# olegiy/manuscript-ocr

Hardware: AMD Instinct MI355X
Metric: manuscript pages/sec end-to-end (EAST+TRBA) at 1/2/4/8 MI355X; CER vs CPU ref (higher is better)
Workload: dtype f32 (bf16x3 split operands on the 1x1 / Winograd-domain GEMMs, f32 accumulate)

## Files before the change

### include/msocr.h

```cpp
#ifndef MSOCR_H
#define MSOCR_H
#include <stdint.h>

#ifdef __cplusplus
extern "C" {
#endif

#define MSOCR_F32 0
#define MSOCR_BF16 1

#define MSOCR_OK 0
#define MSOCR_E_ARG (-1)
#define MSOCR_E_LAUNCH (-2)
#define MSOCR_E_NOGPU (-3)

#define MSOCR_CONV_RELU 1u
#define MSOCR_CONV_RESIDUAL 2u
#define MSOCR_CONV_POOL2 4u

typedef struct msocr_conv_desc {
  int32_t dtype;
  int32_t N, H, W, Cin;
  int64_t in_sN, in_sH, in_sW;
  int32_t KH, KW, stride_h, stride_w, pad_h, pad_w;
  int32_t Ho, Wo, Cout;
  int64_t out_ld;
  int64_t res_ld;
  uint32_t flags;
} msocr_conv_desc;

int msocr_conv2d(const msocr_conv_desc* d, const void* in, const void* weight, const float* bias,
                 const void* residual, void* out, void* stream);

#define MSOCR_WINO_2X2 0
#define MSOCR_WINO_4X2 1
#define MSOCR_WINO_4X4 2
#define MSOCR_WINO_4X4_COLTAIL 3
int64_t msocr_winograd_workspace_bytes(const msocr_conv_desc* d, int form);
int msocr_winograd_weights_host(int form, const float* w_khwc_host, int Cout, int Cin, float* u_out_host);
int msocr_conv3x3_winograd(const msocr_conv_desc* d, int form, int split, const void* in, const void* u, const float* bias,
                           const void* residual, void* out, void* workspace, void* stream);
int msocr_winograd_input_transform(const msocr_conv_desc* d, int form, const void* in, void* workspace, void* stream);
int msocr_winograd_gemm(const msocr_conv_desc* d, int form, int split, const void* u, void* workspace, void* stream);
int msocr_winograd_output_transform(const msocr_conv_desc* d, int form, const void* workspace, const float* bias, const void* residual,
                                    void* out, void* stream);

int64_t msocr_winograd_crop_lds_bytes(const msocr_conv_desc* d, int form, int se);
int msocr_winograd_output_chain(const msocr_conv_desc* d, int form, void* workspace, const float* bias, void* stream);
int msocr_winograd_output_se(const msocr_conv_desc* d, int form, const void* workspace, const float* bias, const void* identity,
                             const float* w1, const float* w2, float* gate_ws, void* out, void* stream);

int msocr_split_bf16x3_host(const float* w_host, int64_t n, uint16_t* planes_out_host);
int msocr_split_bf16x3_ktile_host(const float* w_host, int64_t nbatch, int64_t rows, int64_t k, uint16_t* planes_out_host);
int msocr_conv1x1_split(const msocr_conv_desc* d, const void* in, const void* weight_planes, const float* bias,
                        const void* residual, void* out, void* stream);
int msocr_conv2d_split(const msocr_conv_desc* d, const void* in, const void* weight_planes, const float* bias,
                       const void* residual, void* out, void* stream);

int64_t msocr_winograd_fused64_workspace_bytes(const msocr_conv_desc* d);
int msocr_conv3x3_winograd_fused64(const msocr_conv_desc* d, int split, const void* in, const void* u, const float* bias,
                                   const void* residual, void* out, void* workspace, void* stream);
int msocr_winograd_fused64_gemm_output(const msocr_conv_desc* d, int split, const void* u, const void* workspace, const float* bias,
                                       const void* residual, void* out, void* stream);

int msocr_normalize_u8(const uint8_t* src, int N, int H, int W, int pad_t, int pad_l, int Hp, int Wp, int cpad,
                       int mode, int dtype, void* out, void* stream);

int msocr_resize_linear_u8(const uint8_t* src, int N, int sh, int sw, uint8_t* dst, int dh, int dw, void* stream);

int msocr_maxpool2d(const void* in, int N, int H, int W, int C, int64_t in_ld, int k, int s, int p, int dtype,
                    void* out, int Ho, int Wo, int64_t out_ld, void* stream);

int msocr_upsample2x_bilinear(const void* in, int N, int H, int W, int C, int64_t in_ld, int dtype, void* out,
                              int64_t out_ld, void* stream);

int msocr_east_head(const void* h1, int64_t npix, int64_t in_ld, int dtype, const float* w9, const float* b9,
                    float* score_out, float* geo_out, void* stream);

int msocr_east_decode(const float* score, const float* geo, int N, int H, int W, float thresh, float scale,
                      int quant, float* cand_out, int32_t* count_out, int max_cand, void* stream);

int64_t msocr_lanms_workspace_bytes(int N, int max_cand);
int msocr_east_lanms(const float* cand, const int32_t* counts, int N, int max_cand, double iou_thr, float* boxes_out,
                     int32_t* nbox_out, void* workspace, void* stream);

int64_t msocr_east_box_tail_workspace_bytes(int N, int max_cand);
int msocr_east_box_tail(const float* boxes, const int32_t* nbox, int N, int max_cand, double expand_w, double expand_h,
                        double scale_x, double scale_y, int axis_aligned_output, int remove_anomalies, double sigma, int min_count,
                        float* out, int32_t* n_out, void* workspace, void* stream);
int msocr_east_box_tail_host(const float* quads_host, int M, double expand_w, double expand_h, double scale_x, double scale_y,
                             int axis_aligned_output, int remove_anomalies, double sigma, int min_count, float* out_host,
                             int32_t* n_out_host);


int msocr_se_residual(const void* x, const void* identity, int N, int HW, int C, int dtype, const float* w1,
                      const float* w2, float* gate_ws, void* out, void* stream);

int msocr_mean_over_h(const void* in, int N, int H, int W, int C, int dtype, float* out, void* stream);

int msocr_bilstm_recurrent(const float* xproj, const float* w_hh_t, int B, int T, int H, float* hcat_out,
                           void* stream);
int msocr_bilstm_recurrent_split(const float* xproj, const uint16_t* whh_planes, int B, int T, int H, float* hcat_out,
                                 void* stream);

typedef struct msocr_attn_weights {
  const float* h2h_wt;
  const float* h2h_b;
  const float* score_w;
  const float* wih_ctx_t;
  const float* wih_tok;
  const float* whh_t;
  const float* b_gates;
  const float* gen_wt;
  const float* gen_b;
} msocr_attn_weights;

int msocr_attn_greedy(const float* batch_H, const float* proj_H, const msocr_attn_weights* w, int B, int T, int H,
                      int V, int steps, int sos_id, int eos_id, int blank_id, float* logits_out, int32_t* ids_out,
                      void* stream);
int64_t msocr_attn_beam_workspace_bytes(int B, int steps, int beam, int V);
int msocr_attn_beam(const float* batch_H, const float* proj_H, const msocr_attn_weights* w, int B, int T, int H,
                    int V, int steps, int beam, const float* lp_dev, float temperature, int sos_id, int eos_id,
                    int blank_id, int32_t* fin_step_out, void* workspace, const int32_t* chunk_id_dev,
                    const int32_t* chunk_size_dev, int32_t* chunk_state_dev, void* stream);
typedef struct msocr_attn_split_weights {
  const uint16_t* h2h_p;
  const uint16_t* whh_p;
  const uint16_t* gen_p;
} msocr_attn_split_weights;

int msocr_attn_beam_hoisted(const float* batch_H, const float* proj_H, const float* ctx_gates, const msocr_attn_weights* w,
                            const msocr_attn_split_weights* ws, int B, int T, int H, int V, int steps, int beam, const float* lp_dev,
                            float temperature, int sos_id, int eos_id, int blank_id, int32_t* fin_step_out, void* workspace,
                            const int32_t* chunk_id_dev, const int32_t* chunk_size_dev, int32_t* chunk_state_dev, void* stream);
int msocr_attn_greedy_hoisted(const float* batch_H, const float* proj_H, const float* ctx_gates, const msocr_attn_weights* w,
                              const msocr_attn_split_weights* ws, int B, int T, int H, int V, int steps, int sos_id, int eos_id,
                              int blank_id, float* logits_out, int32_t* ids_out, void* stream);
int64_t msocr_attn_pack_split_elems(int N);
int msocr_attn_pack_split_host(const float* wt_host, int N, int gate_interleaved, uint16_t* out_host);
int msocr_attn_beam_finalize(const void* workspace, int B, int V, int steps, int beam, const int32_t* trun_dev,
                             float* logits_out, int32_t* ids_out, void* stream);

int msocr_attn_greedy_alpha(const float* batch_H, const float* proj_H, const msocr_attn_weights* w, int B, int T, int H,
                            int V, int steps, int sos_id, int eos_id, int blank_id, float* logits_out, int32_t* ids_out,
                            float* alpha_out, void* stream);
int msocr_attn_greedy_hoisted_alpha(const float* batch_H, const float* proj_H, const float* ctx_gates, const msocr_attn_weights* w,
                                    const msocr_attn_split_weights* ws, int B, int T, int H, int V, int steps, int sos_id, int eos_id,
                                    int blank_id, float* logits_out, int32_t* ids_out, float* alpha_out, void* stream);
int64_t msocr_attn_beam_alpha_bytes(int B, int steps, int beam, int T);
int msocr_attn_beam_alpha(const float* batch_H, const float* proj_H, const msocr_attn_weights* w, int B, int T, int H,
                          int V, int steps, int beam, const float* lp_dev, float temperature, int sos_id, int eos_id,
                          int blank_id, int32_t* fin_step_out, void* workspace, const int32_t* chunk_id_dev,
                          const int32_t* chunk_size_dev, int32_t* chunk_state_dev, void* alpha_ws, void* stream);
int msocr_attn_beam_hoisted_alpha(const float* batch_H, const float* proj_H, const float* ctx_gates, const msocr_attn_weights* w,
                                  const msocr_attn_split_weights* ws, int B, int T, int H, int V, int steps, int beam,
                                  const float* lp_dev, float temperature, int sos_id, int eos_id, int blank_id, int32_t* fin_step_out,
                                  void* workspace, const int32_t* chunk_id_dev, const int32_t* chunk_size_dev,
                                  int32_t* chunk_state_dev, void* alpha_ws, void* stream);
int msocr_attn_beam_finalize_alpha(const void* workspace, int B, int V, int steps, int beam, const int32_t* trun_dev,
                                   float* logits_out, int32_t* ids_out, const void* alpha_ws, int T, float* alpha_out,
                                   void* stream);

int msocr_seq_confidence(const float* logits, const int32_t* ids, const int32_t* trun_dev, int B, int V, int steps,
                         float* conf_out, void* stream);

int msocr_seq_char_details(const float* logits, const int32_t* ids, const float* alpha, const int32_t* trun_dev, int B, int V,
                           int steps, int T, float* prob_out, float* centre_out, int32_t* peak_out, void* stream);

int msocr_attn_beam_nbest(const void* workspace, int B, int V, int steps, int beam, int n_best, int eos_id, const int32_t* trun_dev,
                          int32_t* ids_out, float* prob_out, float* conf_out, float* logp_out, void* stream);
int msocr_attn_beam_nbest_host(const void* workspace_host, int B, int V, int steps, int beam, int n_best, int eos_id,
                               const int32_t* trun_host, int32_t* ids_out_host, float* prob_out_host, float* conf_out_host,
                               float* logp_out_host);

int msocr_attn_forced(const float* batch_H, const float* proj_H, const msocr_attn_weights* w, int B, int T, int H, int V, int steps,
                      const int32_t* tok_in, int sos_id, int blank_id, float* logits_out, float* alpha_out, void* stream);
int msocr_attn_forced_hoisted(const float* batch_H, const float* proj_H, const float* ctx_gates, const msocr_attn_weights* w,
                              const msocr_attn_split_weights* ws, int B, int T, int H, int V, int steps, const int32_t* tok_in,
                              int sos_id, int blank_id, float* logits_out, float* alpha_out, void* stream);

int msocr_seq_logp(const float* logits, const int32_t* ids, const int32_t* trun_dev, int B, int V, int steps, float temperature,
                   float* logp_steps_out, float* logp_out, void* stream);
int msocr_seq_logp_host(const float* logits_host, const int32_t* ids_host, const int32_t* trun_host, int B, int V, int steps,
                        float temperature, float* logp_steps_out_host, float* logp_out_host);

typedef struct {
  const int32_t *edge_begin, *edge_tok, *edge_child;
  const uint8_t* terminal;
  int n_nodes, n_edges;
} msocr_lexicon;
int64_t msocr_attn_lexicon_nodes_bytes(int B, int steps, int beam);
int msocr_attn_beam_lexicon(const float* batch_H, const float* proj_H, const msocr_attn_weights* w, int B, int T, int H, int V, int steps,
                            int beam, const float* lp_dev, float temperature, int sos_id, int eos_id, int blank_id,
                            int32_t* fin_step_out, void* workspace, const int32_t* chunk_id_dev, const int32_t* chunk_size_dev,
                            int32_t* chunk_state_dev, void* alpha_ws, const msocr_lexicon* lex, int32_t* node_out, void* stream);
int msocr_attn_beam_lexicon_hoisted(const float* batch_H, const float* proj_H, const float* ctx_gates, const msocr_attn_weights* w,
                                    const msocr_attn_split_weights* ws, int B, int T, int H, int V, int steps, int beam,
                                    const float* lp_dev, float temperature, int sos_id, int eos_id, int blank_id, int32_t* fin_step_out,
                                    void* workspace, const int32_t* chunk_id_dev, const int32_t* chunk_size_dev,
                                    int32_t* chunk_state_dev, void* alpha_ws, const msocr_lexicon* lex, int32_t* node_out, void* stream);
int msocr_lexicon_check_host(const int32_t* edge_begin_host, const int32_t* edge_tok_host, const int32_t* edge_child_host,
                             const uint8_t* terminal_host, int n_nodes, int n_edges, int V, int max_depth);

// ... 124 lines not shown
```

### manuscript_ocr_amd/_native.py

```python
import ctypes
import os

import torch

_HERE = os.path.dirname(os.path.abspath(__file__))
LIB_PATH = os.path.join(_HERE, "libmsocr.so")

F32, BF16 = 0, 1
CONV_RELU, CONV_RESIDUAL, CONV_POOL2 = 1, 2, 4
WINO_2X2, WINO_4X2, WINO_4X4, WINO_4X4_COLTAIL = 0, 1, 2, 3

c_i32, c_i64, c_u32 = ctypes.c_int32, ctypes.c_int64, ctypes.c_uint32
c_f32, c_f64, c_vp = ctypes.c_float, ctypes.c_double, ctypes.c_void_p


class ConvDesc(ctypes.Structure):
    _fields_ = [
        ("dtype", c_i32), ("N", c_i32), ("H", c_i32), ("W", c_i32), ("Cin", c_i32),
        ("in_sN", c_i64), ("in_sH", c_i64), ("in_sW", c_i64),
        ("KH", c_i32), ("KW", c_i32), ("stride_h", c_i32), ("stride_w", c_i32), ("pad_h", c_i32), ("pad_w", c_i32),
        ("Ho", c_i32), ("Wo", c_i32), ("Cout", c_i32),
        ("out_ld", c_i64), ("res_ld", c_i64), ("flags", c_u32),
    ]


class JpegInfo(ctypes.Structure):
    _fields_ = [("width", c_i32), ("height", c_i32), ("ncomp", c_i32), ("hs", c_i32 * 3), ("vs", c_i32 * 3),
                ("blocks_w", c_i32 * 3), ("blocks_h", c_i32 * 3), ("supported", c_i32), ("coef_off", c_i64 * 3),
                ("coef_total", c_i64), ("quant", (ctypes.c_uint16 * 64) * 3)]


class AttnWeights(ctypes.Structure):
    _fields_ = [(n, c_vp) for n in ("h2h_wt", "h2h_b", "score_w", "wih_ctx_t", "wih_tok", "whh_t", "b_gates", "gen_wt", "gen_b")]


class AttnSplitWeights(ctypes.Structure):
    _fields_ = [(n, c_vp) for n in ("h2h_p", "whh_p", "gen_p")]


class LexiconArrays(ctypes.Structure):
    _fields_ = [("edge_begin", c_vp), ("edge_tok", c_vp), ("edge_child", c_vp), ("terminal", c_vp), ("n_nodes", c_i32), ("n_edges", c_i32)]


class WordList(ctypes.Structure):
    _fields_ = [("word_begin", c_vp), ("word_tok", c_vp), ("n_words", c_i32), ("n_tok", c_i32), ("by_length", c_vp)]


class CharLMTable(ctypes.Structure):
    _fields_ = [("table", c_vp), ("order", c_i32), ("V", c_i32), ("n_ctx", c_i64)]


_SIGS = {
    "msocr_conv2d": (c_i32, [ctypes.POINTER(ConvDesc), c_vp, c_vp, c_vp, c_vp, c_vp, c_vp]),
    "msocr_winograd_workspace_bytes": (c_i64, [ctypes.POINTER(ConvDesc), c_i32]),
    "msocr_winograd_weights_host": (c_i32, [c_i32, c_vp, c_i32, c_i32, c_vp]),
    "msocr_conv3x3_winograd": (c_i32, [ctypes.POINTER(ConvDesc), c_i32, c_i32, c_vp, c_vp, c_vp, c_vp, c_vp, c_vp, c_vp]),
    "msocr_winograd_input_transform": (c_i32, [ctypes.POINTER(ConvDesc), c_i32, c_vp, c_vp, c_vp]),
    "msocr_winograd_gemm": (c_i32, [ctypes.POINTER(ConvDesc), c_i32, c_i32, c_vp, c_vp, c_vp]),
    "msocr_winograd_output_transform": (c_i32, [ctypes.POINTER(ConvDesc), c_i32, c_vp, c_vp, c_vp, c_vp, c_vp]),
    "msocr_winograd_crop_lds_bytes": (c_i64, [ctypes.POINTER(ConvDesc), c_i32, c_i32]),
    "msocr_winograd_output_chain": (c_i32, [ctypes.POINTER(ConvDesc), c_i32, c_vp, c_vp, c_vp]),
    "msocr_winograd_output_se": (c_i32, [ctypes.POINTER(ConvDesc), c_i32, c_vp, c_vp, c_vp, c_vp, c_vp, c_vp, c_vp, c_vp]),
    "msocr_winograd_fused64_workspace_bytes": (c_i64, [ctypes.POINTER(ConvDesc)]),
    "msocr_conv3x3_winograd_fused64": (c_i32, [ctypes.POINTER(ConvDesc), c_i32, c_vp, c_vp, c_vp, c_vp, c_vp, c_vp, c_vp]),
    "msocr_winograd_fused64_gemm_output": (c_i32, [ctypes.POINTER(ConvDesc), c_i32, c_vp, c_vp, c_vp, c_vp, c_vp, c_vp]),
    "msocr_split_bf16x3_host": (c_i32, [c_vp, c_i64, c_vp]),
    "msocr_split_bf16x3_ktile_host": (c_i32, [c_vp, c_i64, c_i64, c_i64, c_vp]),
    "msocr_conv1x1_split": (c_i32, [ctypes.POINTER(ConvDesc), c_vp, c_vp, c_vp, c_vp, c_vp, c_vp]),
    "msocr_conv2d_split": (c_i32, [ctypes.POINTER(ConvDesc), c_vp, c_vp, c_vp, c_vp, c_vp, c_vp]),
    "msocr_normalize_u8": (c_i32, [c_vp, c_i32, c_i32, c_i32, c_i32, c_i32, c_i32, c_i32, c_i32, c_i32, c_i32, c_vp, c_vp]),
    "msocr_resize_linear_u8": (c_i32, [c_vp, c_i32, c_i32, c_i32, c_vp, c_i32, c_i32, c_vp]),
    "msocr_maxpool2d": (c_i32, [c_vp, c_i32, c_i32, c_i32, c_i32, c_i64, c_i32, c_i32, c_i32, c_i32, c_vp, c_i32, c_i32, c_i64, c_vp]),
    "msocr_upsample2x_bilinear": (c_i32, [c_vp, c_i32, c_i32, c_i32, c_i32, c_i64, c_i32, c_vp, c_i64, c_vp]),
    "msocr_east_head": (c_i32, [c_vp, c_i64, c_i64, c_i32, c_vp, c_vp, c_vp, c_vp, c_vp]),
    "msocr_east_decode": (c_i32, [c_vp, c_vp, c_i32, c_i32, c_i32, c_f32, c_f32, c_i32, c_vp, c_vp, c_i32, c_vp]),
    "msocr_lanms_workspace_bytes": (c_i64, [c_i32, c_i32]),
    "msocr_east_lanms": (c_i32, [c_vp, c_vp, c_i32, c_i32, c_f64, c_vp, c_vp, c_vp, c_vp]),
    "msocr_se_residual": (c_i32, [c_vp, c_vp, c_i32, c_i32, c_i32, c_i32, c_vp, c_vp, c_vp, c_vp, c_vp]),
    "msocr_mean_over_h": (c_i32, [c_vp, c_i32, c_i32, c_i32, c_i32, c_i32, c_vp, c_vp]),
    "msocr_bilstm_recurrent": (c_i32, [c_vp, c_vp, c_i32, c_i32, c_i32, c_vp, c_vp]),
    "msocr_bilstm_recurrent_split": (c_i32, [c_vp, c_vp, c_i32, c_i32, c_i32, c_vp, c_vp]),
    "msocr_attn_greedy": (c_i32, [c_vp, c_vp, ctypes.POINTER(AttnWeights), c_i32, c_i32, c_i32, c_i32, c_i32, c_i32, c_i32, c_i32,
                                  c_vp, c_vp, c_vp]),
    "msocr_attn_greedy_hoisted": (c_i32, [c_vp, c_vp, c_vp, ctypes.POINTER(AttnWeights), ctypes.POINTER(AttnSplitWeights), c_i32, c_i32,
                                          c_i32, c_i32, c_i32, c_i32, c_i32, c_i32, c_vp, c_vp, c_vp]),
    "msocr_attn_beam": (c_i32, [c_vp, c_vp, ctypes.POINTER(AttnWeights), c_i32, c_i32, c_i32, c_i32, c_i32, c_i32, c_vp, c_f32,
                                c_i32, c_i32, c_i32, c_vp, c_vp, c_vp, c_vp, c_vp, c_vp]),
    "msocr_attn_pack_split_elems": (c_i64, [c_i32]),
    "msocr_attn_pack_split_host": (c_i32, [c_vp, c_i32, c_i32, c_vp]),
    "msocr_attn_beam_hoisted": (c_i32, [c_vp, c_vp, c_vp, ctypes.POINTER(AttnWeights), ctypes.POINTER(AttnSplitWeights), c_i32, c_i32, c_i32, c_i32, c_i32, c_i32, c_vp, c_f32,
                                        c_i32, c_i32, c_i32, c_vp, c_vp, c_vp, c_vp, c_vp, c_vp]),
    "msocr_attn_beam_workspace_bytes": (c_i64, [c_i32, c_i32, c_i32, c_i32]),
    "msocr_attn_beam_finalize": (c_i32, [c_vp, c_i32, c_i32, c_i32, c_i32, c_vp, c_vp, c_vp, c_vp]),
    "msocr_seq_confidence": (c_i32, [c_vp, c_vp, c_vp, c_i32, c_i32, c_i32, c_vp, c_vp]),
    "msocr_attn_greedy_alpha": (c_i32, [c_vp, c_vp, ctypes.POINTER(AttnWeights), c_i32, c_i32, c_i32, c_i32, c_i32, c_i32, c_i32, c_i32,
                                        c_vp, c_vp, c_vp, c_vp]),
    "msocr_attn_greedy_hoisted_alpha": (c_i32, [c_vp, c_vp, c_vp, ctypes.POINTER(AttnWeights), ctypes.POINTER(AttnSplitWeights), c_i32,
                                                c_i32, c_i32, c_i32, c_i32, c_i32, c_i32, c_i32, c_vp, c_vp, c_vp, c_vp]),
    "msocr_attn_beam_alpha_bytes": (c_i64, [c_i32, c_i32, c_i32, c_i32]),
    "msocr_attn_beam_alpha": (c_i32, [c_vp, c_vp, ctypes.POINTER(AttnWeights), c_i32, c_i32, c_i32, c_i32, c_i32, c_i32, c_vp, c_f32,
                                      c_i32, c_i32, c_i32, c_vp, c_vp, c_vp, c_vp, c_vp, c_vp, c_vp]),
    "msocr_attn_beam_hoisted_alpha": (c_i32, [c_vp, c_vp, c_vp, ctypes.POINTER(AttnWeights), ctypes.POINTER(AttnSplitWeights), c_i32, c_i32,
                                              c_i32, c_i32, c_i32, c_i32, c_vp, c_f32, c_i32, c_i32, c_i32, c_vp, c_vp, c_vp, c_vp, c_vp,
                                              c_vp, c_vp]),
    "msocr_attn_beam_finalize_alpha": (c_i32, [c_vp, c_i32, c_i32, c_i32, c_i32, c_vp, c_vp, c_vp, c_vp, c_i32, c_vp, c_vp]),
    "msocr_seq_char_details": (c_i32, [c_vp, c_vp, c_vp, c_vp, c_i32, c_i32, c_i32, c_i32, c_vp, c_vp, c_vp, c_vp]),
    "msocr_attn_beam_nbest": (c_i32, [c_vp, c_i32, c_i32, c_i32, c_i32, c_i32, c_i32, c_vp, c_vp, c_vp, c_vp, c_vp, c_vp]),
    "msocr_attn_beam_nbest_host": (c_i32, [c_vp, c_i32, c_i32, c_i32, c_i32, c_i32, c_i32, c_vp, c_vp, c_vp, c_vp, c_vp]),
    "msocr_attn_forced": (c_i32, [c_vp, c_vp, ctypes.POINTER(AttnWeights), c_i32, c_i32, c_i32, c_i32, c_i32, c_vp, c_i32, c_i32,
                                  c_vp, c_vp, c_vp]),
    "msocr_attn_forced_hoisted": (c_i32, [c_vp, c_vp, c_vp, ctypes.POINTER(AttnWeights), ctypes.POINTER(AttnSplitWeights), c_i32, c_i32,
                                          c_i32, c_i32, c_i32, c_vp, c_i32, c_i32, c_vp, c_vp, c_vp]),
    "msocr_seq_logp": (c_i32, [c_vp, c_vp, c_vp, c_i32, c_i32, c_i32, c_f32, c_vp, c_vp, c_vp]),
    "msocr_seq_logp_host": (c_i32, [c_vp, c_vp, c_vp, c_i32, c_i32, c_i32, c_f32, c_vp, c_vp]),
    "msocr_attn_lexicon_nodes_bytes": (c_i64, [c_i32, c_i32, c_i32]),
    "msocr_attn_beam_lexicon": (c_i32, [c_vp, c_vp, ctypes.POINTER(AttnWeights), c_i32, c_i32, c_i32, c_i32, c_i32, c_i32, c_vp, c_f32,
                                        c_i32, c_i32, c_i32, c_vp, c_vp, c_vp, c_vp, c_vp, c_vp, ctypes.POINTER(LexiconArrays), c_vp, c_vp]),
    "msocr_attn_beam_lexicon_hoisted": (c_i32, [c_vp, c_vp, c_vp, ctypes.POINTER(AttnWeights), ctypes.POINTER(AttnSplitWeights), c_i32, c_i32,
                                                c_i32, c_i32, c_i32, c_i32, c_vp, c_f32, c_i32, c_i32, c_i32, c_vp, c_vp, c_vp, c_vp, c_vp,
                                                c_vp, ctypes.POINTER(LexiconArrays), c_vp, c_vp]),
    "msocr_attn_lm_ctx_bytes": (c_i64, [c_i32, c_i32, c_i32]),
    "msocr_attn_beam_lm": (c_i32, [c_vp, c_vp, ctypes.POINTER(AttnWeights), c_i32, c_i32, c_i32, c_i32, c_i32, c_i32, c_vp, c_f32,
                                   c_i32, c_i32, c_i32, c_vp, c_vp, c_vp, c_vp, c_vp, c_vp, ctypes.POINTER(CharLMTable), c_f32, c_vp, c_vp]),
    "msocr_attn_beam_lm_hoisted": (c_i32, [c_vp, c_vp, c_vp, ctypes.POINTER(AttnWeights), ctypes.POINTER(AttnSplitWeights), c_i32, c_i32,
                                           c_i32, c_i32, c_i32, c_i32, c_vp, c_f32, c_i32, c_i32, c_i32, c_vp, c_vp, c_vp, c_vp, c_vp,
                                           c_vp, ctypes.POINTER(CharLMTable), c_f32, c_vp, c_vp]),
    "msocr_lexicon_check_host": (c_i32, [c_vp, c_vp, c_vp, c_vp, c_i32, c_i32, c_i32, c_i32]),
    "msocr_lexicon_nearest_ws_bytes": (c_i64, [c_i32, c_i32, c_i32]),
    "msocr_lexicon_nearest": (c_i32, [c_vp, c_vp, c_i32, c_i32, c_i32, c_i32, c_i32, c_i32, ctypes.POINTER(WordList), c_i32, c_i32,
                                      c_vp, c_vp, c_vp, c_vp]),
    "msocr_lexicon_nearest_host": (c_i32, [c_vp, c_vp, c_i32, c_i32, c_i32, c_i32, c_i32, c_i32, ctypes.POINTER(WordList), c_i32, c_i32,
                                           c_vp, c_vp]),
    "msocr_edit_distance_pairs": (c_i32, [c_vp, c_vp, c_i32, c_vp, c_vp, c_i32, c_i32, c_i32, c_i32, c_i32, c_i32, c_vp, c_vp, c_vp,
                                          c_vp]),
    "msocr_edit_distance_pairs_host": (c_i32, [c_vp, c_vp, c_i32, c_vp, c_vp, c_i32, c_i32, c_i32, c_i32, c_i32, c_i32, c_vp, c_vp,
                                               c_vp]),
    "msocr_wordlist_check_host": (c_i32, [c_vp, c_vp, c_i32, c_i32, c_i32, c_i32]),
    "msocr_crop_resize_pad": (c_i32, [c_vp, c_i32, c_i32, c_i32, c_vp, c_vp, c_i32, c_i32, c_i32, c_vp, c_vp]),
    "msocr_east_box_tail_workspace_bytes": (c_i64, [c_i32, c_i32]),
    "msocr_east_box_tail": (c_i32, [c_vp, c_vp, c_i32, c_i32, c_f64, c_f64, c_f64, c_f64, c_i32, c_i32, c_f64, c_i32, c_vp, c_vp, c_vp, c_vp]),
    "msocr_east_box_tail_host": (c_i32, [c_vp, c_i32, c_f64, c_f64, c_f64, c_f64, c_i32, c_i32, c_f64, c_i32, c_vp, c_vp]),
    "msocr_reading_order_host": (c_i32, [c_vp, c_i32, c_f64, c_f64, c_vp]),
    "msocr_reading_lines_host": (c_i32, [c_vp, c_i32, c_f64, c_f64, c_vp, c_vp, c_vp, c_vp]),
    "msocr_reading_order_workspace_bytes": (c_i64, [c_i32, c_i32]),
    "msocr_reading_order_crops": (c_i32, [c_vp, c_vp, c_i32, c_i32, c_i32, c_i32, c_i32, c_i32, c_i32, c_f64, c_f64, c_i32,
                                          c_vp, c_vp, c_vp, c_vp, c_vp, c_vp]),
    "msocr_reading_order_line_rows": (c_i32, [c_i32]),
    "msocr_reading_order_lines": (c_i32, [c_vp, c_vp, c_i32, c_i32, c_i32, c_i32, c_i32, c_i32, c_i32, c_f64, c_f64, c_i32,
                                          c_vp, c_vp, c_vp, c_vp, c_vp, c_vp, c_vp, c_vp, c_vp]),
    "msocr_quad_crop_descriptors": (c_i32, [c_vp, c_vp, c_i32, c_i32, c_i32, c_i32, c_vp, c_vp, c_vp, c_vp, c_vp, c_vp]),
    "msocr_quad_crop_descriptors_host": (c_i32, [c_vp, c_vp, c_i32, c_i32, c_i32, c_i32, c_vp]),
    "msocr_quad_crop": (c_i32, [c_vp, c_i32, c_i32, c_i32, c_vp, c_vp, c_i32, c_i32, c_i32, c_vp, c_vp]),
    "msocr_quad_crop_host": (c_i32, [c_vp, c_i32, c_i32, c_i32, c_vp, c_i32, c_i32, c_i32, c_vp]),
    "msocr_jpeg_parse_host": (c_i32, [c_vp, c_i64, ctypes.POINTER(JpegInfo)]),
    "msocr_jpeg_parse_oriented_host": (c_i32, [c_vp, c_i64, ctypes.POINTER(JpegInfo), ctypes.POINTER(c_i32)]),
    "msocr_jpeg_entropy_decode_host": (c_i32, [c_vp, c_i64, ctypes.POINTER(JpegInfo), c_vp]),
    "msocr_jpeg_scan_desc_bytes": (c_i64, []),
    "msocr_jpeg_scan_prepare_host": (c_i64, [c_vp, c_i64, ctypes.POINTER(JpegInfo), c_i64, c_vp, c_vp, c_i64]),
    "msocr_jpeg_entropy_decode_device": (c_i32, [c_vp, c_vp, c_i32, c_i32, c_vp, c_vp, c_vp, c_i64, c_vp, c_vp]),
    "msocr_jpeg_entropy_decode_intervals_host": (c_i32, [c_vp, c_vp, c_i32, c_vp, c_vp, c_vp, c_i64, c_vp]),
    "msocr_jpeg_sync_prepare_host": (c_i64, [c_vp, c_i64, ctypes.POINTER(JpegInfo), c_i64, c_vp, c_vp, c_i64]),
    "msocr_jpeg_sync_workspace_bytes": (c_i64, [c_i64, c_i32, c_i32]),
    "msocr_jpeg_entropy_decode_sync_device": (c_i32, [c_vp, c_vp, c_i32, c_vp, c_vp, c_vp, c_i32, c_i64, c_i32, c_i32, c_vp, c_i64,
                                                      c_vp, c_vp, c_vp, c_vp]),
    "msocr_jpeg_entropy_decode_sync_host": (c_i32, [c_vp, c_vp, c_i32, c_vp, c_vp, c_vp, c_i32, c_i32, c_vp, c_i64, c_vp, c_vp]),
    "msocr_jpeg_workspace_bytes": (c_i64, [ctypes.POINTER(JpegInfo)]),
    "msocr_jpeg_reconstruct": (c_i32, [ctypes.POINTER(JpegInfo), c_vp, c_vp, c_vp, c_vp]),
    "msocr_jpeg_reconstruct_host": (c_i32, [ctypes.POINTER(JpegInfo), c_vp, c_vp]),
    "msocr_jpeg_reconstruct_oriented": (c_i32, [ctypes.POINTER(JpegInfo), c_i32, c_vp, c_vp, c_vp, c_vp]),
    "msocr_jpeg_reconstruct_oriented_host": (c_i32, [ctypes.POINTER(JpegInfo), c_i32, c_vp, c_vp]),
    "msocr_nchw_f32_to_nhwc": (c_i32, [c_vp, c_i32, c_i32, c_i32, c_i32, c_i32, c_vp, c_i64, c_vp]),
    "msocr_nhwc_to_nchw_f32": (c_i32, [c_vp, c_i32, c_i32, c_i32, c_i32, c_i64, c_i32, c_vp, c_vp]),
    "msocr_version": (ctypes.c_char_p, []),
}

_lib = None


class NativeError(RuntimeError):
    pass


def lib():
    global _lib
    if _lib is None:
        if not os.path.exists(LIB_PATH) and os.path.exists("/opt/rocm/bin/hipcc"):
            import fcntl
            import subprocess
            try:
                with open(os.path.join(_HERE, "csrc", ".build.lock"), "w") as lock:
                    fcntl.flock(lock, fcntl.LOCK_EX)
                    if not os.path.exists(LIB_PATH):
                        subprocess.check_call(["make", "-s", "-j4", "-C", os.path.join(_HERE, "csrc"), "ARCH=gfx950"])
            except Exception as e:
                print(f"[manuscript_ocr_amd] building libmsocr.so failed: {e}")
        if not os.path.exists(LIB_PATH):
            raise NativeError(
                f"{LIB_PATH} not found: build it with `python -c 'import __graft_entry__ as g; g.build()'` "
                "(or `make -C manuscript_ocr_amd/csrc`). There is no CPU fallback."
            )
        L = ctypes.CDLL(LIB_PATH)
        missing = [name for name in _SIGS if not hasattr(L, name)]
        if missing:
            raise NativeError(f"{LIB_PATH} lacks symbols declared in include/msocr.h: {missing}")
        for name, (res, args) in _SIGS.items():
            fn = getattr(L, name)
            fn.restype, fn.argtypes = res, args
        _lib = L
    return _lib


def exported_symbols():
    return list(_SIGS)


# ... 4 lines not shown
```

### manuscript_ocr_amd/csrc/conv_common.h

```cpp
#ifndef MSOCR_CONV_COMMON_H
#define MSOCR_CONV_COMMON_H
#include <hip/hip_runtime.h>
#include <stdint.h>

#include <type_traits>

#include "internal.h"
#include "msocr.h"
#include "split_mma.h"

typedef uint32_t u32x4 __attribute__((ext_vector_type(4)));
typedef uint32_t u32x2 __attribute__((ext_vector_type(2)));

struct ConvParams {
  const char* in;
  const char* w;
  const float* bias;
  const char* res;
  char* out;
  int N, H, W, Cin;
  long sN, sH, sW;
  int KH, KW, SH, SW, PH, PW;
  int Ho, Wo, Cout;
  long M;
  int ktiles, cin_tiles;
  long Ktot;
  long out_ld, res_ld;
  int relu, has_res;
  int tilesM, tilesN;
  int nbatch;
  long bsA, bsW, bsO;
  long wplane;
  long w_kt_b;
};

__device__ __forceinline__ float bf16_to_f32(uint16_t v) { return __uint_as_float(((uint32_t)v) << 16); }
__device__ __forceinline__ uint16_t f32_to_bf16(float f) {
  __bf16 b = (__bf16)f;
  return *reinterpret_cast<uint16_t*>(&b);
}

template <typename T>
struct Mma;
template <>
struct Mma<float> {
  static __device__ __forceinline__ void run(const u32x4& a, const u32x4& b, f32x16& c) {
#pragma unroll
    for (int j = 0; j < 4; ++j)
      c = __builtin_amdgcn_mfma_f32_32x32x2f32(__uint_as_float(a[j]), __uint_as_float(b[j]), c, 0, 0, 0);
  }
};
template <>
struct Mma<__bf16> {
  static __device__ __forceinline__ void run(const u32x4& a, const u32x4& b, f32x16& c) {
    bf16x8 av = __builtin_bit_cast(bf16x8, a);
    bf16x8 bv = __builtin_bit_cast(bf16x8, b);
    c = __builtin_amdgcn_mfma_f32_32x32x16_bf16(av, bv, c, 0, 0, 0);
  }
};

__attribute__((visibility("hidden"))) bool msocr_internal_split_pp_takes(const ConvParams& p);
__attribute__((visibility("hidden"))) int msocr_internal_split_pp_launch(ConvParams& p, hipStream_t s, bool general);

template <int BKB>
__device__ __forceinline__ int swz(int row) {
  constexpr int CPR = BKB / 16;
  constexpr int RPB = 256 / BKB;
  return (row / RPB) & (CPR - 1);
}
__device__ __forceinline__ int swz16(int row) { return (4 - ((row >> 2) & 3)) & 3; }
template <typename T, int BM_, int BN_, int BKB_, int WM_, int STAGES_>
struct IgemmTile {
  static constexpr int BM = BM_, BN = BN_, BKB = BKB_, THREADS = 256, PERSISTENT = 0;
  static constexpr int BK = BKB / (int)sizeof(T);
  static constexpr int CPR = BKB / 16;
  static constexpr int RPP = 256 / CPR;
  static constexpr int A_IT = BM / RPP, B_IT = (BN + RPP - 1) / RPP;
  static constexpr int A_BYTES = BM * BKB, B_BYTES = BN * BKB, STAGE = A_BYTES + B_BYTES;
  static constexpr int EPI = (BM / WM_) * 32 * BN * 4;
  static constexpr int LDS = STAGES_ * STAGE > EPI ? STAGES_ * STAGE : EPI;
};
template <int BM_, int BN_>
struct SplitStage {
  static constexpr int BM = BM_, BN = BN_, BK = 32;
  static constexpr int ROWB = BK * 2;
  static constexpr int A_PLANE = BM * ROWB, B_PLANE = BN * ROWB;
  static constexpr int STAGE_B = 3 * (A_PLANE + B_PLANE);
  static constexpr int ACH = BK / 4, ARP = 256 / ACH, A_IT = BM / ARP;
  static constexpr int BCH = BK / 8, BRP = 256 / BCH, B_IT = (BN + BRP - 1) / BRP;
};
template <int BN_>
struct SplitTile : SplitStage<128, BN_> {
  static constexpr int WM = 64, WN = BN_ / 2, THREADS = 256, PERSISTENT = 0;
  static constexpr int EPI = (128 / WM) * 32 * BN_ * 4;
  static constexpr int LDS = SplitStage<128, BN_>::STAGE_B > EPI ? SplitStage<128, BN_>::STAGE_B : EPI;
  static __device__ __forceinline__ int swz(int row) { return ::swz<64>(row); }
};
template <int TM, int TN>
struct SplitPPTile : SplitStage<64 * TM, 64 * TN> {
  static constexpr int THREADS = 512, PERSISTENT = 1;
  static constexpr int BIAS_OFF = 2 * SplitStage<64 * TM, 64 * TN>::STAGE_B;
  static constexpr int LDS = BIAS_OFF + 4 * 64 * TN * 4;
  static __device__ __forceinline__ int swz(int row) { return swz16(row); }
};

static __device__ __attribute__((aligned(16))) uint32_t msocr_zero16[4] = {0u, 0u, 0u, 0u};

template <typename I>
__device__ __forceinline__ void xcd_range(I x, I nblk, I& first, I& count) {
  const I q = nblk >> 3, r = nblk & 7;
  first = x < r ? x * (q + 1) : r * (q + 1) + (x - r) * q;
  count = q + (x < r ? 1 : 0);
}
template <typename I>
__device__ __forceinline__ I xcd_tile(I bid, I nblk) {
  I first, count;
  xcd_range<I>(bid & 7, nblk, first, count);
  return first + (bid >> 3);
}
__device__ __forceinline__ void tile_coords(const ConvParams& p, int t, int& batch, int& tile_m, int& tile_n) {
  const int nblk1 = p.tilesM * p.tilesN;
  batch = t / nblk1;
  t -= batch * nblk1;
  tile_n = t % p.tilesN;
  tile_m = t / p.tilesN;
}

template <bool GEN>
struct ATap { int hi0, wi0; };
template <>
struct ATap<false> {};
__device__ __forceinline__ long a_row_origin(const ConvParams& p, long m, ATap<true>& t) {
  const long hw = (long)p.Ho * p.Wo;
  const int n = (int)(m / hw);
  const int rem = (int)(m - (long)n * hw);
  const int ho = rem / p.Wo, wo = rem - ho * p.Wo;
  t.hi0 = ho * p.SH - p.PH;
  t.wi0 = wo * p.SW - p.PW;
  return (long)n * p.sN + (long)t.hi0 * p.sH + (long)t.wi0 * p.sW;
}
template <bool GEN>
__device__ __forceinline__ uint32_t a_row_offset32(const ConvParams& p, long m, int a_chunk, ATap<GEN>& t) {
  if (m >= p.M) m = p.M - 1;
  if constexpr (GEN) return (uint32_t)(int32_t)((a_row_origin(p, m, t) + a_chunk * 4) * 4);
  else return (uint32_t)((m * p.sW + a_chunk * 4) * 4);
}
struct TapCursor {
  int kh, kw, c0;
  __device__ __forceinline__ void reset() { kh = kw = c0 = 0; }
  __device__ __forceinline__ long offset(const ConvParams& p) const { return (long)kh * p.sH + (long)kw * p.sW + c0; }
  __device__ __forceinline__ bool inside(const ConvParams& p, const ATap<true>& t) const {
    const int hi = t.hi0 + kh, wi = t.wi0 + kw;
    return (unsigned)hi < (unsigned)p.H && (unsigned)wi < (unsigned)p.W;
  }
  __device__ __forceinline__ void advance(const ConvParams& p, int bk) {
    c0 += bk;
    if (c0 == p.Cin) {
      c0 = 0;
      if (++kw == p.KW) { kw = 0; ++kh; }
    }
  }
};
template <int A_IT>
__device__ __forceinline__ void load_a_taps32(const ConvParams& p, const char* g_in, const uint32_t (&a_off)[A_IT],
                                              const ATap<true> (&tap)[A_IT], TapCursor& t, int bk, u32x4 (&ra)[A_IT]) {
  const int32_t koff = (int32_t)(t.offset(p) * 4);
#pragma unroll
  for (int i = 0; i < A_IT; ++i) {
    const char* src = g_in + (long)(int32_t)(a_off[i] + (uint32_t)koff);
    ra[i] = *reinterpret_cast<const u32x4*>(t.inside(p, tap[i]) ? src : reinterpret_cast<const char*>(msocr_zero16));
  }
  t.advance(p, bk);
}
template <int A_IT>
__device__ __forceinline__ void load_a_rows32(const char* ga, const uint32_t (&a_off)[A_IT], u32x4 (&ra)[A_IT]) {
#pragma unroll
  for (int i = 0; i < A_IT; ++i) ra[i] = *reinterpret_cast<const u32x4*>(ga + a_off[i]);
}
__device__ __forceinline__ uint32_t b_plane_offset(int co, int cout, int b_chunk) {
  if (co >= cout) co = cout - 1;
  return (uint32_t)(co * 64 + b_chunk * 16);
}
template <class G>
__device__ __forceinline__ void load_b_planes(const ConvParams& p, const char* g_w, long wplane_b, int kt, int b_row0,
                                              const uint32_t (&b_off)[G::B_IT], u32x4 (&rb)[3][G::B_IT]) {
#pragma unroll
  for (int pl = 0; pl < 3; ++pl) {
    const char* const gb = g_w + pl * wplane_b + (long)kt * p.w_kt_b;
#pragma unroll
    for (int j = 0; j < G::B_IT; ++j)
      if (G::BN % G::BRP == 0 || b_row0 + j * G::BRP < G::BN) rb[pl][j] = *reinterpret_cast<const u32x4*>(gb + b_off[j]);
  }
}
template <class G>
__device__ __forceinline__ void split_store_row(unsigned char* sA, int row, int a_chunk, u32x4 r) {
  float x0 = __uint_as_float(r[0]), x1 = __uint_as_float(r[1]), x2 = __uint_as_float(r[2]), x3 = __uint_as_float(r[3]);
  unsigned char* dst = sA + row * G::ROWB + (((a_chunk >> 1) ^ G::swz(row)) << 4) + ((a_chunk & 1) << 3);
#pragma unroll
  for (int pl = 0; pl < 3; ++pl) {
    u32x2 v;
    v[0] = split_step(x0, x1);
    v[1] = split_step(x2, x3);
    *reinterpret_cast<u32x2*>(dst + pl * G::A_PLANE) = v;
  }
}
template <class G>
__device__ __forceinline__ void store_b_row(unsigned char* sB, int pl, int row, int b_chunk, u32x4 v) {
  *reinterpret_cast<u32x4*>(sB + pl * G::B_PLANE + row * G::ROWB + ((b_chunk ^ G::swz(row)) << 4)) = v;
}

template <typename T, int BM, int BN, int WM, int WN, int MT, bool BIAS16, int NCH = 1, typename AccT, int TMA, int TN>
__device__ __forceinline__ void epilogue_lds(const ConvParams& p, unsigned char* smem, const AccT (&acc)[TMA][TN], int tile_m, int tile_n,
                                             char* g_out, int wm, int wn, int r32, int half) {
  constexpr int ES = sizeof(T), EPC = 16 / ES;
  constexpr int AE = MT == 32 ? 16 : 4;
  const int tid = threadIdx.x;
  constexpr int PR = (BM / WM) * 32;
  float* sc = reinterpret_cast<float*>(smem);
  constexpr int VPR = BN / EPC;
  constexpr int ROWS_PP = 256 / VPR;
  const int vcol = (tid % VPR) * EPC;
  const int vrow0 = tid / VPR;
  const int co = tile_n * BN + vcol;
  float bias[EPC];
  if constexpr (BIAS16) {
    static_assert(EPC == 4, "four f32");
    f32x4 b = {0.f, 0.f, 0.f, 0.f};
    if (p.bias) b = *reinterpret_cast<const f32x4*>(p.bias + co);
    bias[0] = b[0]; bias[1] = b[1]; bias[2] = b[2]; bias[3] = b[3];
  } else {
#pragma unroll
    for (int e = 0; e < EPC; ++e) bias[e] = p.bias ? p.bias[co + e] : 0.f;
  }

  constexpr int TPP = 32 / MT;
  constexpr int NR = PR / ROWS_PP;
  static_assert(PR % ROWS_PP == 0 && NR % NCH == 0, "a pass is whole sweeps of 256 threads, a chunk whole rows");
  static_assert(32 % ROWS_PP == 0 || ROWS_PP == 64, "tile_row must be additive in the sweep index (see row_step)");
  const long m0 = (long)tile_m * BM;
  auto tile_row = [&](int i, int lr) { return (lr >> 5) * WM + i * 32 + (lr & 31); };
  auto lds_write = [&](int i) {
#pragma unroll
    for (int ti = 0; ti < TPP; ++ti)
#pragma unroll
      for (int j = 0; j < TN; ++j)
#pragma unroll
        for (int e = 0; e < AE; ++e) {
          const int rit = MT == 32 ? acc_row(e, half) : 4 * half + e;
          sc[(wm * 32 + ti * MT + rit) * BN + wn * WN + j * MT + r32] = acc[i * TPP + ti][j][e];
        }
  };
  auto lds_row = [&](int lr, float (&v)[EPC]) {
#pragma unroll
    for (int e4 = 0; e4 < EPC; e4 += 4) {
      const f32x4 t = *reinterpret_cast<const f32x4*>(&sc[lr * BN + vcol + e4]);
      v[e4] = t[0]; v[e4 + 1] = t[1]; v[e4 + 2] = t[2]; v[e4 + 3] = t[3];
    }
  };
  auto finish_row = [&](float (&v)[EPC], bool res, const u32x4& rv, char* dst) {
#pragma unroll
    for (int e = 0; e < EPC; ++e) v[e] += bias[e];
    if (res) {
      if constexpr (ES == 4) {
#pragma unroll
        for (int e = 0; e < 4; ++e) v[e] += __uint_as_float(rv[e]);
      } else {
#pragma unroll
        for (int e = 0; e < 8; ++e) v[e] += bf16_to_f32((uint16_t)(rv[e >> 1] >> ((e & 1) * 16)));
      }
    }
    if (p.relu) {
#pragma unroll
      for (int e = 0; e < EPC; ++e) v[e] = fmaxf(v[e], 0.f);
    }
    u32x4 o;
    if constexpr (ES == 4) {
#pragma unroll
      for (int e = 0; e < 4; ++e) o[e] = __float_as_uint(v[e]);
    } else {
#pragma unroll
      for (int e = 0; e < 4; ++e) o[e] = (uint32_t)f32_to_bf16(v[2 * e]) | ((uint32_t)f32_to_bf16(v[2 * e + 1]) << 16);
    }
    *reinterpret_cast<u32x4*>(dst) = o;
  };
  auto whole_tile = [&](auto res_c) {
    constexpr bool RES = decltype(res_c)::value;
    constexpr int CR = NR / NCH;
    const long mt = m0 + tile_row(0, vrow0);
    const char* const res_t = RES ? p.res + (mt * p.res_ld + co) * ES : nullptr;
    char* const out_t = g_out + (mt * p.out_ld + co) * ES;
    auto row_step = [&](int i, int r) { return tile_row(i, r * ROWS_PP); };
    auto load_res = [&](int i, int r0, int r1, u32x4 (&rv)[NR]) {
      if constexpr (RES) {
#pragma unroll
        for (int r = r0; r < r1; ++r) rv[r] = *reinterpret_cast<const u32x4*>(res_t + row_step(i, r) * p.res_ld * ES);
      }
    };
#pragma unroll
    for (int i = 0; i < WM / 32; ++i) {
      const int early = (NCH == 1 || i == WM / 32 - 1) ? NR : CR;
      u32x4 rv[NR];
      load_res(i, 0, early, rv);
      if (i) __syncthreads();
      lds_write(i);
      __syncthreads();
#pragma unroll
      for (int c = 0; c < NCH; ++c) {
        float v[CR][EPC];
#pragma unroll
        for (int r = 0; r < CR; ++r) lds_row(vrow0 + (c * CR + r) * ROWS_PP, v[r]);
#pragma unroll
        for (int r = 0; r < CR; ++r) finish_row(v[r], RES, rv[c * CR + r], out_t + row_step(i, c * CR + r) * p.out_ld * ES);
        if (c == 0 && early < NR) load_res(i, early, NR, rv);
      }
    }
  };
  if (m0 + BM <= p.M) {
    if (p.has_res) whole_tile(std::true_type{});
    else whole_tile(std::false_type{});
    return;
  }
#pragma unroll
  for (int i = 0; i < WM / 32; ++i) {
    if (i) __syncthreads();
    lds_write(i);
    __syncthreads();
    for (int lr = vrow0; lr < PR; lr += ROWS_PP) {
      const long m = m0 + tile_row(i, lr);
      if (m >= p.M) continue;
      float v[EPC];
      lds_row(lr, v);
      u32x4 rv = {0u, 0u, 0u, 0u};
      if (p.has_res) rv = *reinterpret_cast<const u32x4*>(p.res + (m * p.res_ld + co) * ES);
      finish_row(v, p.has_res != 0, rv, g_out + (m * p.out_ld + co) * ES);
    }
  }
}

enum ConvStrideRule {
  CONV_STRIDES_TAPS,
  CONV_STRIDES_ALIGNED,
  CONV_STRIDES_DENSE,
};
static inline int conv_desc_check(const msocr_conv_desc* d, const void* in, const void* weight, const void* residual, const void* out, int es,
                                  int cin_mult, int cout_mult, ConvStrideRule rule) {
  if (!d || !in || !weight || !out) return MSOCR_E_ARG;
  const int EPC = 16 / es;
  if (d->N <= 0 || d->H <= 0 || d->W <= 0 || d->Ho <= 0 || d->Wo <= 0) return MSOCR_E_ARG;
  if (d->Cin <= 0 || d->Cin % cin_mult || d->Cout <= 0 || d->Cout % cout_mult) return MSOCR_E_ARG;
  if (d->KH <= 0 || d->KW <= 0 || d->stride_h <= 0 || d->stride_w <= 0) return MSOCR_E_ARG;
  if (d->out_ld % EPC || d->out_ld < d->Cout) return MSOCR_E_ARG;
  if (rule == CONV_STRIDES_TAPS) {
    if (d->in_sN % EPC) return MSOCR_E_ARG;
    if (d->in_sH % EPC) {
      if ((d->stride_h * d->in_sH) % EPC) return MSOCR_E_ARG;
      for (int kh = 0; kh < d->KH; ++kh)
        if (((kh - d->pad_h) * d->in_sH) % EPC) return MSOCR_E_ARG;
    }
    if (d->in_sW % EPC) {
      if ((d->stride_w * d->in_sW) % EPC) return MSOCR_E_ARG;
      for (int kw = 0; kw < d->KW; ++kw)
        if (((kw - d->pad_w) * d->in_sW) % EPC) return MSOCR_E_ARG;
    }
  } else if (rule == CONV_STRIDES_ALIGNED) {
    if (d->pad_h < 0 || d->pad_w < 0 || d->in_sN % EPC || d->in_sH % EPC || d->in_sW % EPC) return MSOCR_E_ARG;
  } else {
    if (d->KH != 1 || d->KW != 1 || d->stride_h != 1 || d->stride_w != 1 || d->pad_h || d->pad_w || d->Ho != d->H || d->Wo != d->W)
      return MSOCR_E_ARG;
    if (d->in_sW % EPC || d->in_sW < d->Cin || (d->H > 1 && d->in_sH != (int64_t)d->W * d->in_sW) ||
        (d->N > 1 && d->in_sN != (int64_t)d->H * d->W * d->in_sW)) return MSOCR_E_ARG;
  }
  if (((uintptr_t)in | (uintptr_t)weight | (uintptr_t)out) & 15) return MSOCR_E_ARG;
  if ((d->flags & MSOCR_CONV_RESIDUAL) && (!residual || d->res_ld % EPC || d->res_ld < d->Cout || ((uintptr_t)residual & 15))) return MSOCR_E_ARG;
  if ((d->H + 2 * d->pad_h - d->KH) / d->stride_h + 1 < d->Ho || (d->W + 2 * d->pad_w - d->KW) / d->stride_w + 1 < d->Wo)
    return MSOCR_E_ARG;
  return MSOCR_OK;
}
static inline ConvParams conv_params(const msocr_conv_desc* d, const void* in, const void* weight, const float* bias, const void* residual,
                                     void* out) {
  ConvParams p = {};
  p.in = (const char*)in; p.w = (const char*)weight; p.bias = bias; p.res = (const char*)residual; p.out = (char*)out;
  p.N = d->N; p.H = d->H; p.W = d->W; p.Cin = d->Cin;
  p.sN = d->in_sN; p.sH = d->in_sH; p.sW = d->in_sW;
  p.KH = d->KH; p.KW = d->KW; p.SH = d->stride_h; p.SW = d->stride_w; p.PH = d->pad_h; p.PW = d->pad_w;
  p.Ho = d->Ho; p.Wo = d->Wo; p.Cout = d->Cout;
  p.M = (long)d->N * d->Ho * d->Wo;
  p.Ktot = (long)d->KH * d->KW * d->Cin;
  p.out_ld = d->out_ld; p.res_ld = d->res_ld;
  p.relu = (d->flags & MSOCR_CONV_RELU) ? 1 : 0;
  p.has_res = (d->flags & MSOCR_CONV_RESIDUAL) ? 1 : 0;
  p.nbatch = 1;
  return p;
}
static inline int gemm_params(const void* A, const void* B, void* C, long M, int N, int K, int nbatch, int n_mult, int k_mult, ConvParams* out) {
  if (!A || !B || !C || M <= 0 || N <= 0 || N % n_mult || K <= 0 || K % k_mult || nbatch <= 0) return MSOCR_E_ARG;
  if (((uintptr_t)A | (uintptr_t)B | (uintptr_t)C) & 15) return MSOCR_E_ARG;
  if (M > 0x7fffffffL) return MSOCR_E_ARG;
  ConvParams p = {};
  p.in = (const char*)A; p.w = (const char*)B; p.out = (char*)C;
  p.N = 1; p.H = (int)M; p.W = 1; p.Cin = K;
  p.sN = M * (long)K; p.sH = K; p.sW = K;
  p.KH = p.KW = 1; p.SH = p.SW = 1;
  p.Ho = (int)M; p.Wo = 1; p.Cout = N;
  p.M = M; p.Ktot = K;
  p.out_ld = N;
  p.nbatch = nbatch; p.bsA = M * (long)K; p.bsW = (long)N * K; p.bsO = M * (long)N;
  *out = p;
  return MSOCR_OK;
}
template <class G, class Kern>
static int conv_launch(Kern kern, ConvParams& p, hipStream_t s) {
  p.tilesM = (int)((p.M + G::BM - 1) / G::BM);
  p.tilesN = p.Cout / G::BN;
  p.cin_tiles = p.Cin / G::BK;
  p.ktiles = (int)(p.Ktot / G::BK);
  if (msocr_internal_lds_limit(reinterpret_cast<const void*>(kern), G::LDS) != MSOCR_OK) return MSOCR_E_LAUNCH;
  const long nblk = (long)p.tilesM * p.tilesN * p.nbatch;
  if (nblk <= 0 || nblk > 0x7fffffffL) return MSOCR_E_ARG;
  long grid = nblk;
  if (G::PERSISTENT) {
    int n_cu = 0;
    if (msocr_internal_cu_count(&n_cu) != MSOCR_OK) return MSOCR_E_LAUNCH;
    n_cu = n_cu > 8 ? n_cu & ~7 : 8;
    grid = (nblk + 7) & ~7L;
    if (grid > n_cu) grid = n_cu;
  }
  MSOCR_LAUNCH(kern, dim3((unsigned)grid), dim3(G::THREADS), G::LDS, s, p);
  return hipGetLastError() == hipSuccess ? MSOCR_OK : MSOCR_E_LAUNCH;
}

#endif
```

### manuscript_ocr_amd/csrc/conv_split.hip

```cpp
#include <hip/hip_runtime.h>
#include <stdint.h>
#include <stdlib.h>
#include <string.h>

#include "conv_common.h"

namespace {

template <int BN, int WPE, bool GEN>
__global__ __launch_bounds__(256, WPE) void conv_split_kernel(ConvParams p) {
  using G = SplitTile<BN>;
  constexpr int BM = G::BM, WM = G::WM, WN = G::WN, BK = G::BK;
  constexpr int TM = WM / 32, TN = WN / 32;
  constexpr int ROWB = G::ROWB, A_PLANE = G::A_PLANE, B_PLANE = G::B_PLANE, STAGE_B = G::STAGE_B;
  constexpr int ACH = G::ACH, ARP = G::ARP, A_IT = G::A_IT;
  constexpr int BCH = G::BCH, B_IT = G::B_IT;

  extern __shared__ __attribute__((aligned(16))) unsigned char smem[];

  const int tid = threadIdx.x;
  const int lane = tid & 63;
  const int wave = tid >> 6;
  const int wm = wave >> 1, wn = wave & 1;

  int batch, tile_m, tile_n;
  tile_coords(p, xcd_tile<int>(blockIdx.x, p.tilesM * p.tilesN * p.nbatch), batch, tile_m, tile_n);
  const char* const g_in = p.in + (long)batch * p.bsA * 4;
  const char* const g_w = p.w + (long)batch * p.bsW * 2;
  char* const g_out = p.out + (long)batch * p.bsO * 4;

  const int a_chunk = tid % ACH, a_row0 = tid / ACH;
  uint32_t a_off[A_IT];
  ATap<GEN> a_tap[A_IT];
#pragma unroll
  for (int i = 0; i < A_IT; ++i) a_off[i] = a_row_offset32<GEN>(p, (long)tile_m * BM + a_row0 + i * ARP, a_chunk, a_tap[i]);
  TapCursor tap;
  tap.reset();
  const int b_chunk = tid % BCH, b_row0 = tid / BCH;
  uint32_t b_off[B_IT];
#pragma unroll
  for (int j = 0; j < B_IT; ++j) b_off[j] = b_plane_offset(tile_n * BN + b_row0 + j * G::BRP, p.Cout, b_chunk);
  const long wplane_b = p.wplane * 2;

  u32x4 ra[A_IT], rb[3][B_IT];
  auto load_tile = [&](int kt) {
    if constexpr (GEN) load_a_taps32(p, g_in, a_off, a_tap, tap, BK, ra);
    else load_a_rows32(g_in + (long)kt * (BK * 4), a_off, ra);
    load_b_planes<G>(p, g_w, wplane_b, kt, b_row0, b_off, rb);
  };
  auto store_tile = [&](int stage) {
    unsigned char* const sA = smem + stage * STAGE_B;
#pragma unroll
    for (int i = 0; i < A_IT; ++i) split_store_row<G>(sA, a_row0 + i * ARP, a_chunk, ra[i]);
    unsigned char* const sB = sA + 3 * A_PLANE;
#pragma unroll
    for (int pl = 0; pl < 3; ++pl)
#pragma unroll
      for (int j = 0; j < B_IT; ++j)
        if (BN % G::BRP == 0 || b_row0 + j * G::BRP < BN) store_b_row<G>(sB, pl, b_row0 + j * G::BRP, b_chunk, rb[pl][j]);
  };

  f32x16 acc[TM][TN];
#pragma unroll
  for (int i = 0; i < TM; ++i)
#pragma unroll
    for (int j = 0; j < TN; ++j)
#pragma unroll
      for (int e = 0; e < 16; ++e) acc[i][j][e] = 0.f;

  const int r32 = lane & 31, half = lane >> 5;

  auto compute = [&](int stage) {
    const unsigned char* const sA = smem + stage * STAGE_B;
    const unsigned char* const sB = sA + 3 * A_PLANE;
#pragma unroll
    for (int q = 0; q < BK / 16; ++q) {
      const int c = 2 * q + half;
      bf16x8 fa[3][TM], fb[3][TN];
#pragma unroll
      for (int pl = 0; pl < 3; ++pl) {
#pragma unroll
        for (int i = 0; i < TM; ++i) {
          const int row = wm * WM + i * 32 + r32;
          fa[pl][i] = *reinterpret_cast<const bf16x8*>(sA + pl * A_PLANE + row * ROWB + ((c ^ swz<ROWB>(row)) << 4));
        }
#pragma unroll
        for (int j = 0; j < TN; ++j) {
          const int row = wn * WN + j * 32 + r32;
          fb[pl][j] = *reinterpret_cast<const bf16x8*>(sB + pl * B_PLANE + row * ROWB + ((c ^ swz<ROWB>(row)) << 4));
        }
      }
#pragma unroll
      for (int t = 0; t < 6; ++t)
#pragma unroll
        for (int i = 0; i < TM; ++i)
#pragma unroll
          for (int j = 0; j < TN; ++j)
            acc[i][j] = __builtin_amdgcn_mfma_f32_32x32x16_bf16(fa[split_pa(t)][i], fb[split_pb(t)][j], acc[i][j], 0, 0, 0);
    }
  };

  load_tile(0);
  store_tile(0);
  __syncthreads();

  for (int kt = 0; kt < p.ktiles; ++kt) {
    if (kt + 1 < p.ktiles) load_tile(kt + 1);
    compute(0);
    __syncthreads();
    if (kt + 1 < p.ktiles) store_tile(0);
    __syncthreads();
  }

  epilogue_lds<float, BM, BN, WM, WN, 32, true>(p, smem, acc, tile_m, tile_n, g_out, wm, wn, r32, half);
}

template <int BN, int WPE, bool GEN>
int launch_split(ConvParams& p, hipStream_t s) {
  return conv_launch<SplitTile<BN>>(conv_split_kernel<BN, WPE, GEN>, p, s);
}

int launch_split_one(ConvParams& p, hipStream_t s, bool general) {
  if (msocr_internal_split_pp_takes(p)) return msocr_internal_split_pp_launch(p, s, general);
  if (general) return p.Cout % 128 == 0 ? launch_split<128, 3, true>(p, s) : launch_split<64, 3, true>(p, s);
  return p.Cout % 128 == 0 ? launch_split<128, 3, false>(p, s) : launch_split<64, 3, false>(p, s);
}

int launch_split_any(ConvParams& p, hipStream_t s, bool general) {
  if (((long)p.Cout * p.Ktot + 32) * 2 >= (1L << 32)) return MSOCR_E_ARG;
  p.w_kt_b = (long)p.Cout * 64;
  if (general) return launch_split_one(p, s, true);
  const long row_b = p.sW * 4;
  const long limit = (1L << 32) - 4096;
  if ((p.M * p.sW + 32) * 4 < limit) return launch_split_one(p, s, false);
  if (p.nbatch != 1 || row_b <= 0 || row_b * 256 >= limit) return MSOCR_E_ARG;
  const long rows_per = (limit / row_b) & ~255L;
  for (long m0 = 0; m0 < p.M; m0 += rows_per) {
    ConvParams q = p;
    q.M = p.M - m0 < rows_per ? p.M - m0 : rows_per;
    q.in = p.in + m0 * row_b;
    q.out = p.out + m0 * p.out_ld * 4;
    if (p.has_res) q.res = p.res + m0 * p.res_ld * 4;
    const int rc = launch_split_one(q, s, false);
    if (rc != MSOCR_OK) return rc;
  }
  return MSOCR_OK;
}

}

extern "C" int msocr_split_bf16x3_host(const float* w_host, int64_t n, uint16_t* planes_out_host) {
  if (!w_host || !planes_out_host || n <= 0) return MSOCR_E_ARG;
  auto rne = [](float f) -> uint16_t {
    uint32_t u = __builtin_bit_cast(uint32_t, f);
    if ((u & 0x7fffffffu) > 0x7f800000u) return (uint16_t)((u >> 16) | 0x40);
    u += 0x7fffu + ((u >> 16) & 1u);
    return (uint16_t)(u >> 16);
  };
  auto up = [](uint16_t h) -> float {
    return __builtin_bit_cast(float, (uint32_t)h << 16);
  };
  for (int64_t i = 0; i < n; ++i) {
    float r = w_host[i];
    for (int pl = 0; pl < 3; ++pl) {
      const uint16_t h = rne(r);
      planes_out_host[pl * n + i] = h;
      r -= up(h);
    }
  }
  return MSOCR_OK;
}

extern "C" int msocr_split_bf16x3_ktile_host(const float* w_host, int64_t nbatch, int64_t rows, int64_t k, uint16_t* planes_out_host) {
  if (!w_host || !planes_out_host || nbatch <= 0 || rows <= 0 || k <= 0 || k % 32) return MSOCR_E_ARG;
  const int64_t n = nbatch * rows * k;
  uint16_t* tmp = (uint16_t*)malloc((size_t)n * 3 * sizeof(uint16_t));
  if (!tmp) return MSOCR_E_ARG;
  const int rc = msocr_split_bf16x3_host(w_host, n, tmp);
  if (rc == MSOCR_OK) {
    const int64_t kt = k / 32;
    for (int pl = 0; pl < 3; ++pl)
      for (int64_t b = 0; b < nbatch; ++b)
        for (int64_t r = 0; r < rows; ++r)
          for (int64_t t = 0; t < kt; ++t)
            memcpy(planes_out_host + pl * n + ((b * kt + t) * rows + r) * 32, tmp + pl * n + (b * rows + r) * k + t * 32, 64);
  }
  free(tmp);
  return rc;
}

extern "C" int msocr_conv1x1_split(const msocr_conv_desc* d, const void* in, const void* weight_planes, const float* bias,
                                   const void* residual, void* out, void* stream) {
  if (!d || d->dtype != MSOCR_F32) return MSOCR_E_ARG;
  if (conv_desc_check(d, in, weight_planes, residual, out, 4, 32, 64, CONV_STRIDES_DENSE) != MSOCR_OK) return MSOCR_E_ARG;
  ConvParams p = conv_params(d, in, weight_planes, bias, residual, out);
  p.wplane = (long)d->Cout * d->Cin;
  return launch_split_any(p, (hipStream_t)stream, false);
}

extern "C" int msocr_conv2d_split(const msocr_conv_desc* d, const void* in, const void* weight_planes, const float* bias,
                                  const void* residual, void* out, void* stream) {
  if (!d || d->dtype != MSOCR_F32) return MSOCR_E_ARG;
  if (conv_desc_check(d, in, weight_planes, residual, out, 4, 32, 64, CONV_STRIDES_ALIGNED) != MSOCR_OK) return MSOCR_E_ARG;
  ConvParams p = conv_params(d, in, weight_planes, bias, residual, out);
  p.wplane = (long)d->Cout * p.Ktot;
  const long img_bytes = (long)d->in_sN * 4;
  if (img_bytes >= (1L << 31)) return MSOCR_E_ARG;
  const int per = (int)(((1L << 31) - 1) / (img_bytes > 0 ? img_bytes : 1));
  if (d->N <= per) return launch_split_any(p, (hipStream_t)stream, true);
  const long out_img = (long)d->Ho * d->Wo * d->out_ld * 4, res_img = (long)d->Ho * d->Wo * d->res_ld * 4;
  for (int n0 = 0; n0 < d->N; n0 += per) {
    ConvParams q = p;
    q.N = d->N - n0 < per ? d->N - n0 : per;
    q.M = (long)q.N * d->Ho * d->Wo;
    q.in = p.in + (long)n0 * img_bytes;
    q.out = p.out + (long)n0 * out_img;
    if (p.has_res) q.res = p.res + (long)n0 * res_img;
    const int rc = launch_split_any(q, (hipStream_t)stream, true);
    if (rc != MSOCR_OK) return rc;
  }
  return MSOCR_OK;
}

int msocr_internal_gemm_split_batched(const float* A, const uint16_t* Bplanes, float* C, long M, int N, int K, int nbatch, hipStream_t s) {
  ConvParams p;
  if (gemm_params(A, Bplanes, C, M, N, K, nbatch, 64, 32, &p) != MSOCR_OK) return MSOCR_E_ARG;
  p.wplane = (long)nbatch * N * K;
  return launch_split_any(p, s, false);
}
```

### manuscript_ocr_amd/csrc/conv_split_pp.hip

```cpp
#include <hip/hip_runtime.h>
#include <stdint.h>

#include <type_traits>

#include "conv_common.h"

namespace {

template <int I>
using ic = std::integral_constant<int, I>;
template <int U, int N, class F>
__device__ __forceinline__ void static_for(F&& f) {
  if constexpr (U < N) {
    f(ic<U>{});
    static_for<U + 1, N>(f);
  }
}

__device__ __forceinline__ void lds_barrier() {
  __builtin_amdgcn_sched_barrier(0);
  asm volatile("s_waitcnt lgkmcnt(0)\n\ts_barrier" ::: "memory");
  __builtin_amdgcn_sched_barrier(0);
}

template <int OFF>
__device__ __forceinline__ void store_f32x4_saddr(const char* sbase, uint32_t voff, f32x4 v) {
  asm volatile("global_store_dwordx4 %0, %1, %2 offset:%3" ::"v"(voff), "v"(v), "s"(sbase), "n"(OFF) : "memory");
}

template <int TM, int TN, bool GEN>
__global__ __launch_bounds__(512, 2) void conv_split_pp_kernel(ConvParams p) {
  using Tile = SplitPPTile<TM, TN>;
  constexpr int BM = Tile::BM, BN = Tile::BN, BK = Tile::BK, ROWB = Tile::ROWB;
  constexpr int A_PLANE = Tile::A_PLANE, B_PLANE = Tile::B_PLANE, STAGE_B = Tile::STAGE_B;
  constexpr int BIAS_OFF = Tile::BIAS_OFF;
  constexpr int RM = 2 * TM, RN = 2 * TN;
  constexpr bool STREAM_B = TN >= TM;
  constexpr int RH = STREAM_B ? RM : RN, RS = STREAM_B ? RN : RM;

  extern __shared__ __attribute__((aligned(16))) unsigned char smem[];

  const int tid = threadIdx.x;
  const int lane = tid & 63;
  const int wave = __builtin_amdgcn_readfirstlane(tid >> 6);

  const int nblk = p.tilesM * p.tilesN * p.nbatch;
  const int xcd = blockIdx.x & 7, slot = blockIdx.x >> 3, per_x = gridDim.x >> 3;
  int x_start, x_cnt;
  xcd_range<int>(xcd, nblk, x_start, x_cnt);
  const int my_tiles = slot < x_cnt ? (x_cnt - slot + per_x - 1) / per_x : 0;
  const int G = my_tiles * p.ktiles;
  if (G == 0) return;

  auto tile_of = [&](int n, int& batch, int& tile_m, int& tile_n) __attribute__((always_inline)) {
    tile_coords(p, x_start + slot + n * per_x, batch, tile_m, tile_n);
  };

  if (wave >= 4) {
    constexpr int D = 2;
    const int ltid = tid & 255;
    constexpr int ACH = Tile::ACH, ARP = Tile::ARP, A_IT = Tile::A_IT;
    constexpr int BCH = Tile::BCH, B_IT = Tile::B_IT;
    const int a_chunk = ltid % ACH, a_row0 = ltid / ACH;
    const int b_chunk = ltid % BCH, b_row0 = ltid / BCH;
    const long wplane_b = p.wplane * 2;
    const int bias_i = ltid < BN ? ltid : BN - 1;

    uint32_t a_off[A_IT], b_off[B_IT];
    ATap<GEN> a_tap[A_IT];
    const char* ga_base = nullptr;
    const char* gb_base = nullptr;
    const float* gbias = nullptr;
    int an = 0, akt = 0, bn = 0, bkt = 0;
    int sn = 0, skt = 0;
    TapCursor tap;
    tap.reset();

    auto set_tile_a = [&](int n) __attribute__((always_inline)) {
      int batch, tile_m, tile_n;
      tile_of(n, batch, tile_m, tile_n);
      ga_base = p.in + (long)batch * p.bsA * 4;
#pragma unroll
      for (int i = 0; i < A_IT; ++i) a_off[i] = a_row_offset32<GEN>(p, (long)tile_m * BM + a_row0 + i * ARP, a_chunk, a_tap[i]);
      tap.reset();
    };
    auto set_tile_b = [&](int n) __attribute__((always_inline)) {
      int batch, tile_m, tile_n;
      tile_of(n, batch, tile_m, tile_n);
      gb_base = p.w + (long)batch * p.bsW * 2;
      gbias = p.bias ? p.bias + tile_n * BN + bias_i : reinterpret_cast<const float*>(msocr_zero16);
#pragma unroll
      for (int j = 0; j < B_IT; ++j) b_off[j] = b_plane_offset(tile_n * BN + b_row0 + j * Tile::BRP, p.Cout, b_chunk);
    };

    u32x4 ra[D][A_IT], rb[D][3][B_IT];
    float rbias[D];
    auto load_a = [&](auto buf_c) __attribute__((always_inline)) {
      constexpr int BUF = decltype(buf_c)::value;
      if constexpr (GEN) load_a_taps32(p, ga_base, a_off, a_tap, tap, BK, ra[BUF]);
      else load_a_rows32(ga_base + (long)akt * (BK * 4), a_off, ra[BUF]);
      if (++akt == p.ktiles) {
        akt = 0;
        if (an + 1 < my_tiles) set_tile_a(++an);
        else tap.reset();
      }
    };
    auto load_b = [&](auto buf_c) __attribute__((always_inline)) {
      constexpr int BUF = decltype(buf_c)::value;
      rbias[BUF] = *gbias;
      load_b_planes<Tile>(p, gb_base, wplane_b, bkt, b_row0, b_off, rb[BUF]);
      if (++bkt == p.ktiles) {
        bkt = 0;
        if (bn + 1 < my_tiles) set_tile_b(++bn);
      }
    };
    auto store = [&](auto buf_c, int stage) __attribute__((always_inline)) {
      constexpr int BUF = decltype(buf_c)::value;
      unsigned char* const sA = smem + stage * STAGE_B;
#pragma unroll
      for (int i = 0; i < A_IT; ++i) split_store_row<Tile>(sA, a_row0 + i * ARP, a_chunk, ra[BUF][i]);
      unsigned char* const sB = sA + 3 * A_PLANE;
#pragma unroll
      for (int pl = 0; pl < 3; ++pl)
#pragma unroll
        for (int j = 0; j < B_IT; ++j) store_b_row<Tile>(sB, pl, b_row0 + j * Tile::BRP, b_chunk, rb[BUF][pl][j]);
      if (BN == 256 || ltid < BN) *reinterpret_cast<float*>(smem + BIAS_OFF + ((sn & 3) * BN + ltid) * 4) = rbias[BUF];
      if (++skt == p.ktiles) { skt = 0; ++sn; }
    };

    set_tile_a(0);
    set_tile_b(0);
    load_b(ic<0>{});
    load_a(ic<0>{});
    load_b(ic<1>{});
    load_a(ic<1>{});
    store(ic<0>{}, 0);
    lds_barrier();
    for (int g = 0;;) {
      load_b(ic<0>{});
      load_a(ic<0>{});
      store(ic<1>{}, 1);
      lds_barrier();
      if (++g >= G) break;
      load_b(ic<1>{});
      load_a(ic<1>{});
      store(ic<0>{}, 0);
      lds_barrier();
      if (++g >= G) break;
    }
    return;
  }

  __builtin_amdgcn_s_setprio(1);
  const int wm = wave >> 1, wn = wave & 1;
  const int r16 = lane & 15, kg = lane >> 4;
  const uint32_t c16 = (uint32_t)((kg ^ swz16(r16)) << 4);
  const uint32_t offA = (uint32_t)((wm * 32 * TM + r16) * ROWB) + c16;
  const uint32_t offB = (uint32_t)(3 * A_PLANE + (wn * 32 * TN + r16) * ROWB) + c16;
  const uint32_t offH = STREAM_B ? offA : offB, offS = STREAM_B ? offB : offA;
  constexpr int PLANE_H = STREAM_B ? A_PLANE : B_PLANE, PLANE_S = STREAM_B ? B_PLANE : A_PLANE;

  bf16x8 fh[3][RH], fs[2][3];
  auto read_held = [&](auto h_c, uint32_t so) __attribute__((always_inline)) {
    constexpr int H = decltype(h_c)::value;
#pragma unroll
    for (int pl = 0; pl < 3; ++pl) fh[pl][H] = *reinterpret_cast<const bf16x8*>(smem + so + offH + pl * PLANE_H + H * 16 * ROWB);
  };
  auto read_stream = [&](auto s_c, uint32_t so) __attribute__((always_inline)) {
    constexpr int S = decltype(s_c)::value;
#pragma unroll
    for (int pl = 0; pl < 3; ++pl) fs[S & 1][pl] = *reinterpret_cast<const bf16x8*>(smem + so + offS + pl * PLANE_S + S * 16 * ROWB);
  };

  f32x4 acc[RM][RN];
  f32x4 part[2][RH];
  auto chain = [&](auto s_c, auto h_c) __attribute__((always_inline)) {
    constexpr int S = decltype(s_c)::value, H = decltype(h_c)::value;
    f32x4 t = {0.f, 0.f, 0.f, 0.f};
#pragma unroll
    for (int k = 0; k < 6; ++k) {
      if constexpr (STREAM_B) t = __builtin_amdgcn_mfma_f32_16x16x32_bf16(fs[S & 1][split_pb(k)], fh[split_pa(k)][H], t, 0, 0, 0);
      else t = __builtin_amdgcn_mfma_f32_16x16x32_bf16(fh[split_pb(k)][H], fs[S & 1][split_pa(k)], t, 0, 0, 0);
    }
    part[S & 1][H] = t;
  };
  auto commit = [&](auto s_c, auto h_c, auto first_c) __attribute__((always_inline)) {
    constexpr int S = decltype(s_c)::value, H = decltype(h_c)::value;
    f32x4& a = STREAM_B ? acc[H][S] : acc[S][H];
    if constexpr (decltype(first_c)::value != 0) a = part[S & 1][H];
    else a += part[S & 1][H];
    asm volatile("" : "+v"(a));
  };

  char* e_ob = nullptr;
  int e_lim = 0;
  bool e_full = true;
  int e_slot = 0;
  const float lo = p.relu ? 0.f : -__builtin_inff();
  const uint32_t vo = (uint32_t)((r16 * p.out_ld + 4 * kg) * 4);
  auto set_epilogue = [&](int n) __attribute__((always_inline)) {
    int batch, tile_m, tile_n;
    tile_of(n, batch, tile_m, tile_n);
    const long row0 = (long)tile_m * BM + wm * 32 * TM;
    const int col0 = tile_n * BN + wn * 32 * TN;
    e_ob = p.out + ((long)batch * p.bsO + row0 * p.out_ld + col0) * 4;
    const long rows = p.M - row0;
    e_full = rows >= 32 * TM;
    e_lim = (int)(rows < 32 * TM ? rows : 32 * TM) - r16;
    e_slot = n & 3;
  };
  auto store_blocks = [&](auto s_c) __attribute__((always_inline)) {
    constexpr int S = decltype(s_c)::value;
    const long ld16 = p.out_ld * 64;
    const float* const sbias = reinterpret_cast<const float*>(smem + BIAS_OFF) + e_slot * BN + wn * 32 * TN + 4 * kg;
    auto body = [&](auto masked_c) __attribute__((always_inline)) {
      constexpr bool MASKED = decltype(masked_c)::value != 0;
      static_for<0, RH>([&](auto h_c) __attribute__((always_inline)) {
        constexpr int H = decltype(h_c)::value;
        constexpr int I = STREAM_B ? H : S, J = STREAM_B ? S : H;
        const f32x4 b4 = *reinterpret_cast<const f32x4*>(sbias + J * 16);
        f32x4 v = acc[I][J] + b4;
        v[0] = fmaxf(v[0], lo); v[1] = fmaxf(v[1], lo); v[2] = fmaxf(v[2], lo); v[3] = fmaxf(v[3], lo);
        const char* const rowp = e_ob + I * ld16;
        if (!MASKED || I * 16 < e_lim) store_f32x4_saddr<J * 64>(rowp, vo, v);
      });
    };
    if (e_full) body(ic<0>{});
    else body(ic<1>{});
  };

  uint32_t so = 0;
  auto ktile = [&](auto first_c, auto pend_first_c, bool prev) __attribute__((always_inline)) {
    constexpr int FIRST = decltype(first_c)::value;
    static_for<0, RS - 1>([&](auto u_c) __attribute__((always_inline)) {
      constexpr int U = decltype(u_c)::value;
      read_stream(ic<U + 1>{}, so);
      __builtin_amdgcn_sched_barrier(0);
      if constexpr (FIRST != 0) {
        if (prev) store_blocks(u_c);
        __builtin_amdgcn_sched_barrier(0);
      }
      static_for<0, RH>([&](auto h_c) __attribute__((always_inline)) {
        chain(u_c, h_c);
        if constexpr (U > 0) commit(ic<U - 1>{}, h_c, first_c);
        else if (FIRST == 0 || prev) commit(ic<RS - 1>{}, h_c, pend_first_c);
      });
      __builtin_amdgcn_sched_barrier(0);
    });
    lds_barrier();
    so ^= (uint32_t)STAGE_B;
    read_stream(ic<0>{}, so);
    __builtin_amdgcn_sched_barrier(0);
    if constexpr (FIRST != 0) {
      if (prev) store_blocks(ic<RS - 1>{});
      __builtin_amdgcn_sched_barrier(0);
    }
    static_for<0, RH>([&](auto h_c) __attribute__((always_inline)) {
      chain(ic<RS - 1>{}, h_c);
      commit(ic<RS - 2>{}, h_c, first_c);
      __builtin_amdgcn_sched_barrier(0);
      read_held(h_c, so);
      __builtin_amdgcn_sched_barrier(0);
    });
  };

  lds_barrier();
  static_for<0, RH>([&](auto h_c) __attribute__((always_inline)) { read_held(h_c, so); });
  read_stream(ic<0>{}, so);
  for (int n = 0; n < my_tiles; ++n) {
    ktile(ic<1>{}, ic<0>{}, n > 0);
    set_epilogue(n);
    ktile(ic<0>{}, ic<1>{}, false);
    for (int kt = 2; kt < p.ktiles; ++kt) ktile(ic<0>{}, ic<0>{}, false);
  }
  static_for<0, RH>([&](auto h_c) __attribute__((always_inline)) { commit(ic<RS - 1>{}, h_c, ic<0>{}); });
  static_for<0, RS>([&](auto s_c) __attribute__((always_inline)) { store_blocks(s_c); });
}

template <int TM, int TN, bool GEN>
int launch_pp(ConvParams& p, hipStream_t s) {
  return conv_launch<SplitPPTile<TM, TN>>(conv_split_pp_kernel<TM, TN, GEN>, p, s);
}

}

bool msocr_internal_split_pp_takes(const ConvParams& p) { return p.Cout % 128 == 0 && !p.has_res && p.Ktot >= 64; }

int msocr_internal_split_pp_launch(ConvParams& p, hipStream_t s, bool general) {
  if (p.Cout % 256 == 0) return general ? launch_pp<2, 4, true>(p, s) : launch_pp<2, 4, false>(p, s);
  if (p.Cout % 128 == 0) return general ? launch_pp<4, 2, true>(p, s) : launch_pp<4, 2, false>(p, s);
  return MSOCR_E_ARG;
}
```

### manuscript_ocr_amd/csrc/internal.h

```cpp
#ifndef MSOCR_INTERNAL_H
#define MSOCR_INTERNAL_H
#include <hip/hip_runtime.h>

#include <map>
#include <mutex>
#include <set>
#include <utility>

#include "msocr.h"

#define MSOCR_LAUNCH(...) do { (void)hipGetLastError(); hipLaunchKernelGGL(__VA_ARGS__); } while (0)
#define LAUNCH_OK() (hipGetLastError() == hipSuccess ? MSOCR_OK : MSOCR_E_LAUNCH)

__attribute__((visibility("hidden"))) int msocr_internal_gemm_f32_batched(const float* A, const float* B, float* C, long M, int N,
                                                                          int K, int nbatch, hipStream_t s);

__attribute__((visibility("hidden"))) int msocr_internal_gemm_split_batched(const float* A, const uint16_t* Bplanes, float* C, long M,
                                                                            int N, int K, int nbatch, hipStream_t s);

__attribute__((visibility("hidden"))) inline int msocr_internal_lds_limit(const void* kernel, int bytes) {
  static std::mutex mu;
  static std::set<std::pair<const void*, int>> raised;
  int dev = 0;
  if (hipGetDevice(&dev) != hipSuccess) return MSOCR_E_LAUNCH;
  std::lock_guard<std::mutex> lock(mu);
  if (raised.count({kernel, dev})) return MSOCR_OK;
  if (hipFuncSetAttribute(kernel, hipFuncAttributeMaxDynamicSharedMemorySize, bytes) != hipSuccess) return MSOCR_E_LAUNCH;
  raised.insert({kernel, dev});
  return MSOCR_OK;
}
__attribute__((visibility("hidden"))) inline int msocr_internal_cu_count(int* n) {
  static std::mutex mu;
  static std::map<int, int> cu_count;
  int dev = 0;
  if (hipGetDevice(&dev) != hipSuccess) return MSOCR_E_LAUNCH;
  std::lock_guard<std::mutex> lock(mu);
  auto it = cu_count.find(dev);
  if (it == cu_count.end()) {
    int cu = 0;
    if (hipDeviceGetAttribute(&cu, hipDeviceAttributeMultiprocessorCount, dev) != hipSuccess) return MSOCR_E_LAUNCH;
    it = cu_count.emplace(dev, cu).first;
  }
  *n = it->second;
  return MSOCR_OK;
}

struct AttnArgs {
  const float* batch_H;
  const float* proj_H;
  const float* ctx_gates;
  msocr_attn_weights w;
  const uint16_t *h2h_p, *whh_p, *gen_p;
  int B, T, V, steps, K;
  int sos_id, eos_id, blank_id;
  float temperature;
  const float* lp;
  float* logits_out;
  int32_t* ids_out;
  int32_t* back;
  int32_t* tokv;
  int32_t* best_at;
  int32_t* fin_step;
  const int32_t* chunk_id;
  const int32_t* chunk_size;
  int32_t* chunk_state;
  float* alpha_out;
  const int32_t* tok_in;
  const int32_t *lex_begin, *lex_tok, *lex_child;
  const uint8_t* lex_terminal;
  int lex_nodes, lex_edges;
  int32_t* node_out;
  const float* lm_table;
  int lm_nctx, lm_ctx0;
  float lm_weight;
  int32_t* ctx_out;
};
__attribute__((visibility("hidden"))) int msocr_internal_attn_beam_mfma(const AttnArgs& a, hipStream_t s);
__attribute__((visibility("hidden"))) int msocr_internal_attn_greedy_mfma(const AttnArgs& a, hipStream_t s);
__attribute__((visibility("hidden"))) int msocr_internal_attn_beam_mfma_alpha(const AttnArgs& a, hipStream_t s);
__attribute__((visibility("hidden"))) int msocr_internal_attn_greedy_mfma_alpha(const AttnArgs& a, hipStream_t s);
__attribute__((visibility("hidden"))) int msocr_internal_attn_forced_mfma(const AttnArgs& a, hipStream_t s);
__attribute__((visibility("hidden"))) int msocr_internal_attn_general(const AttnArgs& a, int H, bool beam, hipStream_t s);
__attribute__((visibility("hidden"))) int msocr_internal_attn_general_forced(const AttnArgs& a, int H, hipStream_t s);
__attribute__((visibility("hidden"))) int msocr_internal_attn_general_lexicon(const AttnArgs& a, int H, hipStream_t s);
__attribute__((visibility("hidden"))) int msocr_internal_attn_lexicon_mfma(const AttnArgs& a, hipStream_t s);
__attribute__((visibility("hidden"))) int msocr_internal_attn_general_lm(const AttnArgs& a, int H, hipStream_t s);
__attribute__((visibility("hidden"))) int msocr_internal_attn_lm_mfma(const AttnArgs& a, hipStream_t s);
#endif
```

### manuscript_ocr_amd/csrc/winograd.hip

```cpp
#include <hip/hip_runtime.h>
#include <stdint.h>

#include "conv_common.h"
#include "se_tail.h"

template <int M> __device__ void wino_bt1(const f32x4 d[M + 2], f32x4 r[M + 2]);
template <int M> __device__ void wino_at1(const f32x4 m[M + 2], f32x4 y[M]);

template <> __device__ __forceinline__ void wino_bt1<2>(const f32x4 d[4], f32x4 r[4]) {
  r[0] = d[0] - d[2];
  r[1] = d[1] + d[2];
  r[2] = d[2] - d[1];
  r[3] = d[1] - d[3];
}
template <> __device__ __forceinline__ void wino_at1<2>(const f32x4 m[4], f32x4 y[2]) {
  y[0] = (m[0] + m[1]) + m[2];
  y[1] = (m[1] - m[2]) - m[3];
}

__device__ __forceinline__ void wino44_bt(const f32x4 d[6], f32x4 r[6]) {
  constexpr float k97_36 = 97.0f / 36.0f, k4_9 = 4.0f / 9.0f, k9_4 = 2.25f, k3_2 = 1.5f, k2_3 = 2.0f / 3.0f;
#pragma unroll
  for (int e = 0; e < 4; ++e) {
    r[0][e] = fmaf(-k97_36, d[2][e], d[0][e]) + d[4][e];
// ... 87 lines not shown
        wino_bt1<MH>(col, hv);
        row[j] = hv[i];
      }
      wino_bt1<MW>(row, v);
#pragma unroll
      for (int j = 0; j < PW; ++j) *reinterpret_cast<f32x4*>(o + (i * PW + j) * plane) = v[j];
    }
  }
}

template <int MH, int MW>
__device__ __forceinline__ void wino_output_body(const float* Mw, int Cout, const WinoGeom& g, long plane_mt, const float* bias, const float* res,
                                                 long res_ld, int relu, float* out, long out_ld, long t, int c) {
  constexpr int PH = MH + 2, PW = MW + 2;
  if (t >= g.Mt) return;
  const int tw = (int)(t % g.TW);
  const long r = t / g.TW;
  const int th = (int)(r % g.TH);
  const int n = (int)(r / g.TH);
  const long plane = plane_mt * (long)Cout;
  const float* mp = Mw + t * (long)Cout + c;
  f32x4 mt[PH][PW];
  if constexpr (MH == 2) {
#pragma unroll
    for (int i = 0; i < PH; ++i)
#pragma unroll
      for (int j = 0; j < PW; ++j) mt[i][j] = *reinterpret_cast<const f32x4*>(mp + (i * PW + j) * plane);
  }
  f32x4 s[MH][PW];
#pragma unroll
  for (int j = 0; j < PW; ++j) {
    f32x4 m[PH], y[MH];
#pragma unroll
    for (int i = 0; i < PH; ++i) m[i] = MH == 2 ? mt[i][j] : *reinterpret_cast<const f32x4*>(mp + (i * PW + j) * plane);
    wino_at1<MH>(m, y);
#pragma unroll
    for (int a = 0; a < MH; ++a) s[a][j] = y[a];
  }
  f32x4 b = {0.f, 0.f, 0.f, 0.f};
  if (bias) b = *reinterpret_cast<const f32x4*>(bias + c);
#pragma unroll
  for (int a = 0; a < MH; ++a) {
    const int ho = MH * th + a;
    if (ho >= g.H) continue;
    f32x4 y[MW];
    wino_at1<MW>(s[a], y);
#pragma unroll
    for (int j = 0; j < MW; ++j) {
      const int wo = g.w0 + MW * tw + j;
      if (wo >= g.W) continue;
      const long pix = ((long)n * g.H + ho) * g.W + wo;
      f32x4 v = y[j] + b;
      if (res) v += *reinterpret_cast<const f32x4*>(res + pix * res_ld + c);
      if (relu) {
        v[0] = fmaxf(v[0], 0.f); v[1] = fmaxf(v[1], 0.f); v[2] = fmaxf(v[2], 0.f); v[3] = fmaxf(v[3], 0.f);
      }
      *reinterpret_cast<f32x4*>(out + pix * out_ld + c) = v;
    }
  }
}

__device__ __forceinline__ long wino_thread_tile(int C, int* c) {
  const int cch = C >> 2;
  const long gid = (long)blockIdx.x * 256 + threadIdx.x;
  const long t = gid / cch;
  *c = (int)(gid - t * cch) << 2;
  return t;
}

#define WINO_TRANSFORM_KERNELS(PREFIX, MH, MW)                                                                                    \
  __global__ __launch_bounds__(256) void PREFIX##_input_kernel(const float* __restrict__ in, long sN, long sH, long sW, int C,   \
                                                               WinoGeom g, float* __restrict__ V) {                            \
    int c;                                                                                                                       \
    const long t = wino_thread_tile(C, &c);                                                                                      \
    wino_input_body<MH, MW>(in, sN, sH, sW, C, g, g.Mt, V, t, c);                                                                \
  }                                                                                                                              \
  __global__ __launch_bounds__(256) void PREFIX##_output_kernel(const float* __restrict__ Mw, int Cout, WinoGeom g,              \
                                                                const float* __restrict__ bias, const float* __restrict__ res,  \
                                                                long res_ld, int relu, float* __restrict__ out, long out_ld) {  \
    int c;                                                                                                                       \
    const long t = wino_thread_tile(Cout, &c);                                                                                   \
    wino_output_body<MH, MW>(Mw, Cout, g, g.Mt, bias, res, res_ld, relu, out, out_ld, t, c);                                     \
  }
WINO_TRANSFORM_KERNELS(wino, 2, 2)
WINO_TRANSFORM_KERNELS(wino42, 4, 2)
WINO_TRANSFORM_KERNELS(wino44, 4, 4)
#undef WINO_TRANSFORM_KERNELS

__global__ __launch_bounds__(256) void wino44_input_kernel_coltail(const float* __restrict__ in, long sN, long sH, long sW, int C,
                                                                   WinoGeom g44, WinoGeom g41, float* __restrict__ V44,
                                                                   float* __restrict__ V41) {
  int c;
  const long t = wino_thread_tile(C, &c);
  if (t < g44.Mt) wino_input_body<4, 4>(in, sN, sH, sW, C, g44, g44.Mt, V44, t, c);
  else wino_input_body<4, 1>(in, sN, sH, sW, C, g41, g41.Mt, V41, t - g44.Mt, c);
}
__global__ __launch_bounds__(256) void wino44_output_kernel_coltail(const float* __restrict__ Mw44, const float* __restrict__ Mw41,
                                                                    int Cout, WinoGeom g44, WinoGeom g41,
                                                                    const float* __restrict__ bias, const float* __restrict__ res,
                                                                    long res_ld, int relu, float* __restrict__ out, long out_ld) {
  int c;
  const long t = wino_thread_tile(Cout, &c);
  if (t < g44.Mt) wino_output_body<4, 4>(Mw44, Cout, g44, g44.Mt, bias, res, res_ld, relu, out, out_ld, t, c);
  else wino_output_body<4, 1>(Mw41, Cout, g41, g41.Mt, bias, res, res_ld, relu, out, out_ld, t - g44.Mt, c);
}

constexpr int kCropThreads = 512;
constexpr int kCropLdsMax = 160 * 1024;

struct WinoCrop {
  WinoGeom a, b;
  long mt44, mt41, row0_44, row0_41;
};
__device__ __forceinline__ WinoCrop wino_crop(const WinoGeom& g44, const WinoGeom& g41, int C) {
  WinoCrop k;
  k.a = g44; k.b = g41;
  k.a.N = k.b.N = 1;
  k.a.Mt = (long)g44.TH * g44.TW;
  k.b.Mt = g41.Mt ? (long)g41.TH * g41.TW : 0;
  k.mt44 = g44.Mt; k.mt41 = g41.Mt;
  k.row0_44 = blockIdx.x * k.a.Mt * C; k.row0_41 = blockIdx.x * k.b.Mt * C;
  return k;
}
template <typename F44, typename F41>
__device__ __forceinline__ void wino_crop_pairs(const WinoCrop& k, int C, F44 f44, F41 f41) {
  const int cch = C >> 2, t44 = (int)k.a.Mt, pairs = (t44 + (int)k.b.Mt) * cch;
  for (int i = threadIdx.x; i < pairs; i += kCropThreads) {
    const int t = i / cch, c = (i - t * cch) << 2;
    if (t < t44) f44(t, c);
    else f41(t - t44, c);
  }
}
__device__ __forceinline__ void wino_crop_output(const WinoCrop& k, const float* Mw44, const float* Mw41, int C, const float* bias, int relu,
                                                 float* crop) {
  wino_crop_pairs(k, C,
                  [&](int t, int c) { wino_output_body<4, 4>(Mw44 + k.row0_44, C, k.a, k.mt44, bias, nullptr, 0, relu, crop, C, t, c); },
                  [&](int t, int c) { wino_output_body<4, 1>(Mw41 + k.row0_41, C, k.b, k.mt41, bias, nullptr, 0, relu, crop, C, t, c); });
  __syncthreads();
}

__global__ __launch_bounds__(kCropThreads) void wino44_output_kernel_chain(const float* __restrict__ Mw44, const float* __restrict__ Mw41,
                                                                            int C, WinoGeom g44, WinoGeom g41,
                                                                            const float* __restrict__ bias, int relu,
                                                                            float* __restrict__ V44, float* __restrict__ V41) {
  extern __shared__ __attribute__((aligned(16))) float crop[];
  const WinoCrop k = wino_crop(g44, g41, C);
  wino_crop_output(k, Mw44, Mw41, C, bias, relu, crop);
  const long sW = C, sH = (long)g44.W * C;
  wino_crop_pairs(k, C,
                  [&](int t, int c) { wino_input_body<4, 4>(crop, 0, sH, sW, C, k.a, k.mt44, V44 + k.row0_44, t, c); },
                  [&](int t, int c) { wino_input_body<4, 1>(crop, 0, sH, sW, C, k.b, k.mt41, V41 + k.row0_41, t, c); });
}

__global__ __launch_bounds__(kCropThreads) void wino44_output_kernel_se(const float* __restrict__ Mw44, const float* __restrict__ Mw41,
                                                                         int C, WinoGeom g44, WinoGeom g41,
                                                                         const float* __restrict__ bias, const float* __restrict__ idt,
                                                                         const float* __restrict__ w1, const float* __restrict__ w2,
                                                                         float* __restrict__ gate_ws, float* __restrict__ out) {
  extern __shared__ __attribute__((aligned(16))) float crop[];
  const int tid = threadIdx.x, HW = g44.H * g44.W;
  const long n = blockIdx.x;
  float* sm = crop + (long)HW * C;
  const WinoCrop k = wino_crop(g44, g41, C);
  wino_crop_output(k, Mw44, Mw41, C, bias, 0, crop);
  const float* is = idt + n * HW * C;
  float* os = out + n * HW * C;
  auto ldx = [&](int p, int c) { return *reinterpret_cast<const f32x4*>(crop + p * C + c); };
  se_partial_sums<1024, kCropThreads>(ldx, HW, C, sm, tid);
  const float* gate = se_gate<1024, kCropThreads>(sm, HW, C, w1, w2, gate_ws + n * C, tid);
  se_scale<1024, kCropThreads>(ldx, [&](int p, int c) { return *reinterpret_cast<const f32x4*>(is + (long)p * C + c); },
                               [&](int p, int c, f32x4 y) { *reinterpret_cast<f32x4*>(os + (long)p * C + c) = y; }, HW, C, gate, tid);
}

struct WinoPart {
  WinoGeom g;
  int P;
  long v, mw;
};
struct WinoPlan {
  int form, nparts;
  WinoPart part[2];
  long tiles, total;
};

static const int kWinoTile[4][2] = {{2, 2}, {4, 2}, {4, 4}, {4, 4}};

static bool wino_plan(const msocr_conv_desc* d, int form, WinoPlan* pl) {
  if (form < MSOCR_WINO_2X2 || form > MSOCR_WINO_4X4_COLTAIL || !d || d->dtype != MSOCR_F32) return false;
  if (d->KH != 3 || d->KW != 3 || d->stride_h != 1 || d->stride_w != 1 || d->pad_h != 1 || d->pad_w != 1) return false;
  if (d->N <= 0 || d->H <= 0 || d->W <= 0 || d->Ho != d->H || d->Wo != d->W) return false;
  if (d->Cin <= 0 || d->Cin % 16 || d->Cout <= 0 || d->Cout % 32) return false;
  if ((long)d->N * ((d->H + 1) / 2) * ((d->W + 1) / 2) > 0x7fffffffL) return false;
  const int mh = kWinoTile[form][0], mw = kWinoTile[form][1];
  WinoGeom g;
  g.N = d->N; g.H = d->H; g.W = d->W;
  g.TH = (d->H + mh - 1) / mh; g.TW = (d->W + mw - 1) / mw;
  g.w0 = 0;
  g.Mt = (long)d->N * g.TH * g.TW;
  const int P = (mh + 2) * (mw + 2);
  if (P * g.Mt * (long)(d->Cin > d->Cout ? d->Cin : d->Cout) > 0x3fffffffffffL) return false;
  pl->form = form;
  pl->nparts = 1;
  pl->part[0].g = g; pl->part[0].P = P;
  if (form == MSOCR_WINO_4X4_COLTAIL) {
    if (d->W < 5 || d->W % 4 != 1) return false;
    if (d->Cin % 32 || d->Cout % 64) return false;
    pl->nparts = 2;
    WinoGeom& g44 = pl->part[0].g;
    g44.TW = d->W / 4; g44.Mt = (long)d->N * g.TH * g44.TW;
    WinoGeom& g41 = pl->part[1].g;
    g41 = g; g41.TW = 1; g41.w0 = d->W - 1; g41.Mt = (long)d->N * g.TH;
    pl->part[1].P = 18;
  }
  pl->tiles = pl->total = 0;
  for (int i = 0; i < pl->nparts; ++i) {
    WinoPart& p = pl->part[i];
    pl->tiles += p.g.Mt;
    p.v = pl->total;
    p.mw = p.v + p.P * p.g.Mt * d->Cin;
    pl->total = p.mw + p.P * p.g.Mt * d->Cout;
  }
  return true;
}

static bool wino_strides_ok(const msocr_conv_desc* d) { return !(d->in_sN % 4 || d->in_sH % 4 || d->in_sW % 4); }

static int wino_check(const msocr_conv_desc* d, int form, WinoPlan* pl) {
  if (!wino_plan(d, form, pl) || !wino_strides_ok(d) || d->out_ld % 4 || d->out_ld < d->Cout) return MSOCR_E_ARG;
  return MSOCR_OK;
}

static bool wino_gemm_ok(int form, int split) {
  if (split != 0 && split != 1) return false;
  return form == MSOCR_WINO_4X2 || (form == MSOCR_WINO_2X2 && !split) || ((form == MSOCR_WINO_4X4 || form == MSOCR_WINO_4X4_COLTAIL) && split);
}

extern "C" int64_t msocr_winograd_workspace_bytes(const msocr_conv_desc* d, int form) {
  WinoPlan pl;
  if (!wino_plan(d, form, &pl)) return -1;
  return pl.total * (int64_t)sizeof(float);
}

static bool wino_grid(const WinoPlan& pl, int C, dim3* grid) {
  const long nb = (pl.tiles * (C / 4) + 255) / 256;
  if (nb > 0x7fffffffL) return false;
  *grid = dim3((unsigned)nb);
  return true;
}

static int wino_launch_input(const msocr_conv_desc* d, const WinoPlan& pl, const void* in, void* workspace, void* stream) {
  if (!in || !workspace || (((uintptr_t)in | (uintptr_t)workspace) & 15)) return MSOCR_E_ARG;
  dim3 grid;
  if (!wino_grid(pl, d->Cin, &grid)) return MSOCR_E_ARG;
  const dim3 blk(256);
  hipStream_t st = (hipStream_t)stream;
  const float* x = (const float*)in;
  float* ws = (float*)workspace;
  const long sN = d->in_sN, sH = d->in_sH, sW = d->in_sW;
  const WinoPart& a = pl.part[0];
  if (pl.nparts == 2) MSOCR_LAUNCH(wino44_input_kernel_coltail, grid, blk, 0, st, x, sN, sH, sW, d->Cin, a.g, pl.part[1].g, ws + a.v, ws + pl.part[1].v);
  else if (pl.form == MSOCR_WINO_2X2) MSOCR_LAUNCH(wino_input_kernel, grid, blk, 0, st, x, sN, sH, sW, d->Cin, a.g, ws + a.v);
  else if (pl.form == MSOCR_WINO_4X2) MSOCR_LAUNCH(wino42_input_kernel, grid, blk, 0, st, x, sN, sH, sW, d->Cin, a.g, ws + a.v);
  else MSOCR_LAUNCH(wino44_input_kernel, grid, blk, 0, st, x, sN, sH, sW, d->Cin, a.g, ws + a.v);
  return hipGetLastError() == hipSuccess ? MSOCR_OK : MSOCR_E_LAUNCH;
}

extern "C" int msocr_winograd_input_transform(const msocr_conv_desc* d, int form, const void* in, void* workspace, void* stream) {
  WinoPlan pl;
  if (wino_check(d, form, &pl) != MSOCR_OK) return MSOCR_E_ARG;
  return wino_launch_input(d, pl, in, workspace, stream);
}

extern "C" int msocr_winograd_gemm(const msocr_conv_desc* d, int form, int split, const void* u, void* workspace, void* stream) {
  WinoPlan pl;
  if (!wino_gemm_ok(form, split) || wino_check(d, form, &pl) != MSOCR_OK || !u || !workspace) return MSOCR_E_ARG;
  if (split && (d->Cin % 32 || d->Cout % 64)) return MSOCR_E_ARG;
  float* ws = (float*)workspace;
  long uoff = 0;
  for (int i = 0; i < pl.nparts; ++i) {
    const WinoPart& p = pl.part[i];
    const int rc = split ? msocr_internal_gemm_split_batched(ws + p.v, (const uint16_t*)u + uoff, ws + p.mw, p.g.Mt, d->Cout, d->Cin, p.P, (hipStream_t)stream)
                         : msocr_internal_gemm_f32_batched(ws + p.v, (const float*)u + uoff, ws + p.mw, p.g.Mt, d->Cout, d->Cin, p.P, (hipStream_t)stream);
    if (rc != MSOCR_OK) return rc;
    uoff += (split ? 3L : 1L) * p.P * d->Cout * d->Cin;
  }
  return MSOCR_OK;
}

extern "C" int msocr_winograd_output_transform(const msocr_conv_desc* d, int form, const void* workspace, const float* bias,
                                               const void* residual, void* out, void* stream) {
  WinoPlan pl;
  if (wino_check(d, form, &pl) != MSOCR_OK || !out || !workspace) return MSOCR_E_ARG;
  if (((uintptr_t)out | (uintptr_t)workspace) & 15) return MSOCR_E_ARG;
  const bool has_res = (d->flags & MSOCR_CONV_RESIDUAL) != 0;
  if (has_res && (!residual || d->res_ld % 4 || d->res_ld < d->Cout || ((uintptr_t)residual & 15))) return MSOCR_E_ARG;
  if (bias && ((uintptr_t)bias & 15)) return MSOCR_E_ARG;
  dim3 grid;
  if (!wino_grid(pl, d->Cout, &grid)) return MSOCR_E_ARG;
  const dim3 blk(256);
  hipStream_t st = (hipStream_t)stream;
  const float* ws = (const float*)workspace;
  const float* rp = has_res ? (const float*)residual : nullptr;
  const long res_ld = d->res_ld, out_ld = d->out_ld;
  const int relu = (d->flags & MSOCR_CONV_RELU) ? 1 : 0;
  float* o = (float*)out;
  const WinoPart& a = pl.part[0];
  if (pl.nparts == 2) MSOCR_LAUNCH(wino44_output_kernel_coltail, grid, blk, 0, st, ws + a.mw, ws + pl.part[1].mw, d->Cout, a.g, pl.part[1].g, bias, rp, res_ld, relu, o, out_ld);
  else if (pl.form == MSOCR_WINO_2X2) MSOCR_LAUNCH(wino_output_kernel, grid, blk, 0, st, ws + a.mw, d->Cout, a.g, bias, rp, res_ld, relu, o, out_ld);
  else if (pl.form == MSOCR_WINO_4X2) MSOCR_LAUNCH(wino42_output_kernel, grid, blk, 0, st, ws + a.mw, d->Cout, a.g, bias, rp, res_ld, relu, o, out_ld);
  else MSOCR_LAUNCH(wino44_output_kernel, grid, blk, 0, st, ws + a.mw, d->Cout, a.g, bias, rp, res_ld, relu, o, out_ld);
  return hipGetLastError() == hipSuccess ? MSOCR_OK : MSOCR_E_LAUNCH;
}

static long wino_crop_lds(const msocr_conv_desc* d, const WinoPlan& pl, bool se) {
  if (pl.form != MSOCR_WINO_4X4 && pl.form != MSOCR_WINO_4X4_COLTAIL) return -1;
  const int C = d->Cout;
  if (se ? (C < 64 || C > 1024 || (C & (C - 1)) || d->out_ld != C) : d->Cin != C) return -1;
  const long bytes = ((long)d->H * d->W * C + (se ? se_scratch_floats(1024, C) : 0)) * (long)sizeof(float);
  return bytes <= kCropLdsMax ? bytes : -1;
}

extern "C" int64_t msocr_winograd_crop_lds_bytes(const msocr_conv_desc* d, int form, int se) {
  WinoPlan pl;
  if (!wino_plan(d, form, &pl)) return -1;
  return wino_crop_lds(d, pl, se != 0);
}

struct WinoCropParts {
  WinoGeom g44, g41;
  long v44, v41, mw44, mw41;
};
static WinoCropParts wino_crop_parts(const WinoPlan& pl) {
  const WinoPart& a = pl.part[0];
  const WinoPart& b = pl.part[pl.nparts - 1];
  WinoCropParts k = {a.g, b.g, a.v, b.v, a.mw, b.mw};
  if (pl.nparts == 1) k.g41.Mt = 0;
  return k;
}

extern "C" int msocr_winograd_output_chain(const msocr_conv_desc* d, int form, void* workspace, const float* bias, void* stream) {
  WinoPlan pl;
  if (!wino_plan(d, form, &pl) || !workspace || ((uintptr_t)workspace & 15) || (bias && ((uintptr_t)bias & 15))) return MSOCR_E_ARG;
  const long lds = wino_crop_lds(d, pl, false);
  if (lds < 0 || (d->flags & MSOCR_CONV_RESIDUAL)) return MSOCR_E_ARG;
  if (msocr_internal_lds_limit(reinterpret_cast<const void*>(wino44_output_kernel_chain), kCropLdsMax) != MSOCR_OK) return MSOCR_E_LAUNCH;
  const WinoCropParts k = wino_crop_parts(pl);
  float* ws = (float*)workspace;
  MSOCR_LAUNCH(wino44_output_kernel_chain, dim3((unsigned)d->N), dim3(kCropThreads), (size_t)lds, (hipStream_t)stream, ws + k.mw44, ws + k.mw41,
               d->Cout, k.g44, k.g41, bias, (d->flags & MSOCR_CONV_RELU) ? 1 : 0, ws + k.v44, ws + k.v41);
  return LAUNCH_OK();
}

extern "C" int msocr_winograd_output_se(const msocr_conv_desc* d, int form, const void* workspace, const float* bias, const void* identity,
                                        const float* w1, const float* w2, float* gate_ws, void* out, void* stream) {
  WinoPlan pl;
  if (!wino_plan(d, form, &pl) || !workspace || !identity || !w1 || !w2 || !gate_ws || !out) return MSOCR_E_ARG;
  if (((uintptr_t)workspace | (uintptr_t)identity | (uintptr_t)out) & 15 || (bias && ((uintptr_t)bias & 15))) return MSOCR_E_ARG;
  const long lds = wino_crop_lds(d, pl, true);
  if (lds < 0 || (d->flags & (MSOCR_CONV_RESIDUAL | MSOCR_CONV_RELU))) return MSOCR_E_ARG;
  if (msocr_internal_lds_limit(reinterpret_cast<const void*>(wino44_output_kernel_se), kCropLdsMax) != MSOCR_OK) return MSOCR_E_LAUNCH;
  const WinoCropParts k = wino_crop_parts(pl);
  const float* ws = (const float*)workspace;
  MSOCR_LAUNCH(wino44_output_kernel_se, dim3((unsigned)d->N), dim3(kCropThreads), (size_t)lds, (hipStream_t)stream, ws + k.mw44, ws + k.mw41,
               d->Cout, k.g44, k.g41, bias, (const float*)identity, w1, w2, gate_ws, (float*)out);
  return LAUNCH_OK();
}

extern "C" int msocr_conv3x3_winograd(const msocr_conv_desc* d, int form, int split, const void* in, const void* u, const float* bias,
                                      const void* residual, void* out, void* workspace, void* stream) {
  if (!u || !wino_gemm_ok(form, split)) return MSOCR_E_ARG;
  int rc = msocr_winograd_input_transform(d, form, in, workspace, stream);
  if (rc != MSOCR_OK) return rc;
  rc = msocr_winograd_gemm(d, form, split, u, workspace, stream);
  if (rc != MSOCR_OK) return rc;
  return msocr_winograd_output_transform(d, form, workspace, bias, residual, out, stream);
}

typedef unsigned int u32x4w __attribute__((ext_vector_type(4)));
#ifndef WINO_FUSED_PFD
#define WINO_FUSED_PFD 3
#endif

typedef __bf16 bf16x8w __attribute__((ext_vector_type(8)));
typedef unsigned int u32x2w __attribute__((ext_vector_type(2)));
template <bool POOL, bool SPLIT = false>
__global__ __launch_bounds__(256, 3) void wino42_fused64_kernel(const float* __restrict__ V, const void* __restrict__ Uv, int Cout,
                                                                 WinoGeom g, const float* __restrict__ bias,
                                                                 const float* __restrict__ res, long res_ld, int relu,
                                                                 float* __restrict__ out, long out_ld) {
  constexpr int K = 64, BM = 32, BN = 32, ROWB = K * 4;
  constexpr int ROWS = 128, PLANE = BM * ROWS;
  constexpr int STAGE_BYTES = SPLIT ? 6 * PLANE : (BM + BN) * ROWB;
  __shared__ __attribute__((aligned(16))) unsigned char smem[2][STAGE_BYTES];
  const int tid = threadIdx.x, lane = tid & 63, wave = tid >> 6;
  const int mi = wave >> 1, nj = wave & 1;
  const int r16 = lane & 15, kg = lane >> 4;
  const int nbn = Cout / BN;
  const long bid = xcd_tile<long>(blockIdx.x, gridDim.x);
  const int nb = (int)(bid % nbn);
  const long m0 = (bid / nbn) * BM;
  const int n0 = nb * BN;
  f32x4 acc[24];

  if constexpr (SPLIT) {
    const unsigned short* U = reinterpret_cast<const unsigned short*>(Uv);
    const int chunk = tid & 15, row0 = tid >> 4;
    const int bchunk = tid & 7, brow = tid >> 3;
    const long planeV = g.Mt * (long)K, planeU = (long)Cout * K, uplane = 24 * planeU;
    const float* pa[2];
#pragma unroll
    for (int i = 0; i < 2; ++i) {
      long m = m0 + row0 + 16 * i;
      if (m >= g.Mt) m = g.Mt - 1;
      pa[i] = V + m * K + chunk * 4;
    }
    const unsigned short* pb = U + (long)(n0 + brow) * K + bchunk * 8;
    constexpr int PFD = 2;
    u32x4w ra[PFD][2], rb[PFD][3];
    auto gload = [&](int p) {
#pragma unroll
      for (int i = 0; i < 2; ++i) ra[p % PFD][i] = *reinterpret_cast<const u32x4w*>(pa[i] + p * planeV);
#pragma unroll
      for (int pl = 0; pl < 3; ++pl) rb[p % PFD][pl] = *reinterpret_cast<const u32x4w*>(pb + pl * uplane + p * planeU);
    };
    auto sstore = [&](int p) {
      unsigned char* st = &smem[p & 1][0];
#pragma unroll
      for (int i = 0; i < 2; ++i) {
        const int row = row0 + 16 * i;
        float x0 = __uint_as_float(ra[p % PFD][i][0]), x1 = __uint_as_float(ra[p % PFD][i][1]);
        float x2 = __uint_as_float(ra[p % PFD][i][2]), x3 = __uint_as_float(ra[p % PFD][i][3]);
        unsigned char* dst = st + row * ROWS + (((chunk >> 1) ^ (row & 7)) << 4) + ((chunk & 1) << 3);
#pragma unroll
        for (int pl = 0; pl < 3; ++pl) {
          u32x2w v;
          v[0] = split_step(x0, x1);
          v[1] = split_step(x2, x3);
          *reinterpret_cast<u32x2w*>(dst + pl * PLANE) = v;
        }
      }
#pragma unroll
      for (int pl = 0; pl < 3; ++pl)
        *reinterpret_cast<u32x4w*>(st + (3 + pl) * PLANE + brow * ROWS + ((bchunk ^ (brow & 7)) << 4)) = rb[p % PFD][pl];
    };
#pragma unroll
    for (int q = 0; q < PFD; ++q) gload(q);
    sstore(0);
    __syncthreads();
#pragma unroll
    for (int p = 0; p < 24; ++p) {
      if (p + PFD < 24) gload(p + PFD);
      const unsigned char* st = &smem[p & 1][0];
      const int rowa = mi * 16 + r16, rowb = nj * 16 + r16;
      f32x4 c4 = {0.f, 0.f, 0.f, 0.f};
#pragma unroll
      for (int ks = 0; ks < 2; ++ks) {
        const int c = 4 * ks + kg;
        bf16x8w fa[3], fb[3];
#pragma unroll
        for (int pl = 0; pl < 3; ++pl) {
          fa[pl] = *reinterpret_cast<const bf16x8w*>(st + pl * PLANE + rowa * ROWS + ((c ^ (rowa & 7)) << 4));
          fb[pl] = *reinterpret_cast<const bf16x8w*>(st + (3 + pl) * PLANE + rowb * ROWS + ((c ^ (rowb & 7)) << 4));
        }
        mma6(fa, fb, c4);
      }
      acc[p] = c4;
      if (p + 1 < 24) sstore(p + 1);
      __syncthreads();
    }
  } else {
  const float* U = reinterpret_cast<const float*>(Uv);
  const int chunk = tid & 15, row0 = tid >> 4;
  const long planeV = g.Mt * (long)K, planeU = (long)Cout * K;
  const float* pa[2];
  const float* pb[2];
#pragma unroll
  for (int i = 0; i < 2; ++i) {
    long m = m0 + row0 + 16 * i;
    if (m >= g.Mt) m = g.Mt - 1;
    pa[i] = V + m * K + chunk * 4;
    pb[i] = U + (long)(n0 + row0 + 16 * i) * K + chunk * 4;
  }
  constexpr int PFD = WINO_FUSED_PFD;
  u32x4w ra[PFD][2], rb[PFD][2];
  auto gload = [&](int p) {
#pragma unroll
    for (int i = 0; i < 2; ++i) {
      ra[p % PFD][i] = *reinterpret_cast<const u32x4w*>(pa[i] + p * planeV);
      rb[p % PFD][i] = *reinterpret_cast<const u32x4w*>(pb[i] + p * planeU);
    }
  };
  auto sstore = [&](int p) {
#pragma unroll
    for (int i = 0; i < 2; ++i) {
      const int row = row0 + 16 * i;
      *reinterpret_cast<u32x4w*>(&smem[p & 1][row * ROWB + ((chunk ^ (row & 15)) << 4)]) = ra[p % PFD][i];
      *reinterpret_cast<u32x4w*>(&smem[p & 1][(BM + row) * ROWB + ((chunk ^ (row & 15)) << 4)]) = rb[p % PFD][i];
    }
  };
#pragma unroll
  for (int q = 0; q < PFD; ++q) gload(q);
  sstore(0);
  __syncthreads();
#pragma unroll
  for (int p = 0; p < 24; ++p) {
    if (p + PFD < 24) gload(p + PFD);
    const unsigned char* sa = &smem[p & 1][0];
    const unsigned char* sb = sa + BM * ROWB;
    const int rowa = mi * 16 + r16, rowb = nj * 16 + r16;
    u32x4w fa[4], fb[4];
#pragma unroll
    for (int q = 0; q < 4; ++q) {
      const int c = kg * 4 + q;
      fa[q] = *reinterpret_cast<const u32x4w*>(sa + rowa * ROWB + ((c ^ (rowa & 15)) << 4));
      fb[q] = *reinterpret_cast<const u32x4w*>(sb + rowb * ROWB + ((c ^ (rowb & 15)) << 4));
    }
    f32x4 c4 = {0.f, 0.f, 0.f, 0.f};
// ... 306 lines not shown
```

### manuscript_ocr_amd/ops.py

```python
import ctypes
import os
from typing import NamedTuple

import numpy as np
import torch

from . import _native as nat


PROFILE = None


def _prof_begin():
    if PROFILE is None:
        return None
    e0 = torch.cuda.Event(enable_timing=True)
    e0.record()
    return e0


def _prof_end(e0, kind, work, tag=None):
    if e0 is None or PROFILE is None:
        return
    e1 = torch.cuda.Event(enable_timing=True)
    e1.record()
    PROFILE.append((e0, e1, kind, work, tag))


def _dt(t):
    if t.dtype == torch.float32:
        return nat.F32
    if t.dtype == torch.bfloat16:
        return nat.BF16
    raise TypeError(f"unsupported dtype {t.dtype}")


def _stream():
    return ctypes.c_void_p(torch.cuda.current_stream().cuda_stream)


def _need_cuda(*ts):
    for t in ts:
        if t is not None and not t.is_cuda:
            raise nat.NativeError("native ops need device tensors (no CPU fallback)")


def _pixel_dense_ld(t):
    N, H, W, C = t.shape
    ld = t.stride(2)
    if t.stride(3) != 1 or t.stride(1) != W * ld or (N > 1 and t.stride(0) != H * W * ld) or ld < C:
        raise ValueError(f"tensor is not pixel-dense NHWC: shape {tuple(t.shape)} strides {t.stride()}")
    return ld


WINOGRAD_MIN_CIN = int(os.environ.get("MSOCR_WINOGRAD_MIN_CIN", "128"))


WINO_WS_LIMIT = int(os.environ.get("MSOCR_WINO_WS_LIMIT", str(1 << 30)))
_WINO_ARENA = {}


def _wino_workspace(nbytes, device):
    if torch.cuda.is_current_stream_capturing():
        return torch.empty((nbytes,), dtype=torch.uint8, device=device)
    key = (device.index, torch.cuda.current_stream().cuda_stream)
    buf = _WINO_ARENA.get(key)
    if buf is None or buf.numel() < nbytes:
        buf = None
        _WINO_ARENA.pop(key, None)
        buf = torch.empty((nbytes,), dtype=torch.uint8, device=device)
        _WINO_ARENA[key] = buf
    return buf


WINOGRAD_TALL = int(os.environ.get("MSOCR_WINO_TALL", "1"))


def _tall_pays(H):
    return 24 * (-(-H // 4)) < 16 * (-(-H // 2))


WINOGRAD_SQUARE = int(os.environ.get("MSOCR_WINO_SQUARE", "1"))
WINOGRAD_SQUARE_MIN_CIN = int(os.environ.get("MSOCR_WINO_SQUARE_MIN_CIN", "512"))


WINOGRAD_COLTAIL = int(os.environ.get("MSOCR_WINO_COLTAIL", "1"))


def _coltail(W):
    return bool(WINOGRAD_COLTAIL) and W % 4 == 1 and W >= 5


def _square_pays(W):
    points = 36 * (W // 4) + 18 if _coltail(W) else 36 * (-(-W // 4))
    return points < 24 * (-(-W // 2))


WINO_FORMS = {nat.WINO_2X2: ("winograd", 16, (2, 2)), nat.WINO_4X2: ("winograd42", 24, (4, 2)), nat.WINO_4X4: ("winograd44", 36, (4, 4)),
              nat.WINO_4X4_COLTAIL: ("winograd44", 36 + 18, (4, 4))}


def _wino_rows(form, nn, H, W):
    _, npts, (mh, mw) = WINO_FORMS[form]
    TH = -(-H // mh)
    if form == nat.WINO_4X4_COLTAIL:
        mt44, mt41 = nn * TH * (W // 4), nn * TH
        return 36 * mt44 + 18 * mt41, mt44 + mt41
    mt = nn * TH * -(-W // mw)
    return npts * mt, mt


def _wino_weights(wh, form):
    Cout, _, _, Cin = wh.shape
    u = torch.empty((WINO_FORMS[form][1], Cout, Cin), dtype=torch.float32)
    calls = [(nat.WINO_4X4, u[:36]), (form, u[36:])] if form == nat.WINO_4X4_COLTAIL else [(form, u)]
    for f, planes in calls:
        nat.check(nat.lib().msocr_winograd_weights_host(f, wh.data_ptr(), Cout, Cin, planes.data_ptr()), "winograd_weights_host")
    return u


WINOGRAD_FUSED64 = int(os.environ.get("MSOCR_WINO_FUSED64", "1"))


SPLIT_BF16X3 = int(os.environ.get("MSOCR_SPLIT", "1"))


def split_planes(t):
    th = t.detach().float().cpu().contiguous()
    planes = torch.empty((3,) + tuple(th.shape), dtype=torch.int16)
    nat.check(nat.lib().msocr_split_bf16x3_host(th.data_ptr(), th.numel(), planes.data_ptr()), "split_bf16x3_host")
    return planes.view(torch.bfloat16).to(t.device)


def split_planes_ktile(t, nbatch, rows):
    th = t.detach().float().cpu().contiguous()
    k = th.numel() // (nbatch * rows)
    assert k % 32 == 0 and nbatch * rows * k == th.numel()
    planes = torch.empty((3, nbatch, k // 32, rows, 32), dtype=torch.int16)
    nat.check(nat.lib().msocr_split_bf16x3_ktile_host(th.data_ptr(), nbatch, rows, k, planes.data_ptr()), "split_bf16x3_ktile_host")
    return planes.view(torch.bfloat16).to(t.device)


def unsplit_planes_ktile(planes):
    nb, kt, rows = planes.shape[1:4]
    return planes.float().sum(0).permute(0, 2, 1, 3).reshape(nb, rows, kt * 32)


SPLIT_MIN_K = int(os.environ.get("MSOCR_SPLIT_MIN_K", "128"))


def _split_eligible(w):
    Cout, KH, KW, Cin = w.shape
    return w.dtype == torch.float32 and Cin % 32 == 0 and Cout % 64 == 0 and KH * KW * Cin >= SPLIT_MIN_K


def attach_split(w, split=None):
    if split is False:
        w._msocr_nosplit = True
        return w
    Cout, KH, KW, Cin = w.shape
    if (SPLIT_BF16X3 if split is None else split) and KH == 1 and KW == 1 and _split_eligible(w):
        w._msocr_split = split_planes_ktile(w, 1, Cout)
    return w


def attach_winograd(w, split=None, square=True):
    Cout, KH, KW, Cin = w.shape
    if (WINOGRAD_MIN_CIN and WINOGRAD_FUSED64 and WINOGRAD_TALL and w.dtype == torch.float32 and KH == 3 and KW == 3 and Cin == 64
            and Cin < WINOGRAD_MIN_CIN and Cout % 32 == 0):
        u42 = _wino_weights(w.detach().cpu().contiguous(), nat.WINO_4X2)
        w._msocr_wino42_fused = u42.to(w.device)
        if (SPLIT_BF16X3 if split is None else split) and (Cout % 64 == 0 or Cout >= 128):
            w._msocr_wino42_fused_split = split_planes(u42).to(w.device)
        return w
    if not (WINOGRAD_MIN_CIN and w.dtype == torch.float32 and KH == 3 and KW == 3 and Cin >= WINOGRAD_MIN_CIN and Cin % 16 == 0
            and Cout % 32 == 0):
        return w
    wh = w.detach().cpu().contiguous()
    w._msocr_wino = _wino_weights(wh, nat.WINO_2X2).to(w.device)
    u42 = _wino_weights(wh, nat.WINO_4X2)
    w._msocr_wino42 = u42.to(w.device)
    if (SPLIT_BF16X3 if split is None else split) and Cin % 32 == 0 and Cout % 64 == 0:
        w._msocr_wino42_split = split_planes_ktile(u42, 24, Cout).to(w.device)
        if WINOGRAD_SQUARE and square and Cin >= WINOGRAD_SQUARE_MIN_CIN:
            u54 = _wino_weights(wh, nat.WINO_4X4_COLTAIL)
            p44, p41 = split_planes_ktile(u54[:36], 36, Cout), split_planes_ktile(u54[36:], 18, Cout)
            w._msocr_wino44ct_split = torch.cat([p44.reshape(-1), p41.reshape(-1)]).to(w.device)
            w._msocr_wino44_split = w._msocr_wino44ct_split[:p44.numel()].view(p44.shape)
            w._msocr_wino41_split = w._msocr_wino44ct_split[p44.numel():].view(p41.shape)
    return w


def _wino_stage_in(d, form, xp, ws, what):
    rows, mt = _wino_rows(form, d.N, d.H, d.W)
    e = _prof_begin()
    nat.check(nat.lib().msocr_winograd_input_transform(ctypes.byref(d), form, xp, ws.data_ptr(), _stream()), what)
    _prof_end(e, "wino_in", 4.0 * (d.N * d.H * d.W * d.Cin + rows * d.Cin), (mt, d.Cin))


def _wino_stage_gemm(d, form, split, u, ws, what, alg, name, out_px, res_io, fused_tail=None):
    rows, _ = _wino_rows(form, d.N, d.H, d.W)
    e = _prof_begin()
    if fused_tail is not None:
        rc = nat.lib().msocr_winograd_fused64_gemm_output(ctypes.byref(d), int(split), u.data_ptr(), ws.data_ptr(), *fused_tail, _stream())
    else:
        rc = nat.lib().msocr_winograd_gemm(ctypes.byref(d), form, int(split), u.data_ptr(), ws.data_ptr(), _stream())
    nat.check(rc, what)
    io = 4 * (d.N * d.H * d.W * d.Cin + d.N * out_px * d.Cout * res_io + d.Cout * 9 * d.Cin)
    _prof_end(e, "conv_gemm", (alg, 2.0 * rows * d.Cin * d.Cout, io), (d.N * d.H * d.W, d.Cout, 9 * d.Cin, name))


def _winograd(d, x, w, u, form, split, bias, residual, out, alg, fused=False, pool2=False):
    N, H, W, Cin = x.shape
    Cout = w.shape[0]
    name = WINO_FORMS[form][0] + ("_fused" if fused else "") + ("_split" if split else "")
    L = nat.lib()
    nbytes = L.msocr_winograd_fused64_workspace_bytes(ctypes.byref(d)) if fused else L.msocr_winograd_workspace_bytes(ctypes.byref(d), form)
    if nbytes < 0:
        raise nat.NativeError(f"{name}: unsupported shape {tuple(x.shape)} * {tuple(w.shape)} pool2={pool2}")
    parts = min(N, -(-nbytes // WINO_WS_LIMIT))
    per = -(-N // parts)
    ws = _wino_workspace(nbytes if parts == 1 else (nbytes // N) * per, x.device)
    bp = bias.data_ptr() if bias is not None else None
    what = f"msocr_conv3x3_{name} {tuple(x.shape)} * {tuple(w.shape)}"
    out_px = H * W // (4 if pool2 else 1)
    res_io = 2 if residual is not None else 1
    for n0 in range(0, N, per):
        n1 = min(N, n0 + per)
        d.N = n1 - n0
        xp, rp, op = x[n0:n1].data_ptr(), (residual[n0:n1].data_ptr() if residual is not None else None), out[n0:n1].data_ptr()
        if PROFILE is None:
            if fused:
                rc = L.msocr_conv3x3_winograd_fused64(ctypes.byref(d), int(split), xp, u.data_ptr(), bp, rp, op, ws.data_ptr(), _stream())
            else:
                rc = L.msocr_conv3x3_winograd(ctypes.byref(d), form, int(split), xp, u.data_ptr(), bp, rp, op, ws.data_ptr(), _stream())
            nat.check(rc, what)
            continue
        nn = n1 - n0
        rows, mt = _wino_rows(form, nn, H, W)
        _wino_stage_in(d, form, xp, ws, what)
        _wino_stage_gemm(d, form, split, u, ws, what, alg * nn / N, name, out_px, res_io, (bp, rp, op) if fused else None)
        if not fused:
            e = _prof_begin()
            nat.check(L.msocr_winograd_output_transform(ctypes.byref(d), form, ws.data_ptr(), bp, rp, op, _stream()), what)
            _prof_end(e, "wino_out", 4.0 * (rows * Cout + nn * H * W * Cout * res_io), (mt, Cout))
    d.N = N


def _wino_form(w, H, W):
    form, u, split = nat.WINO_2X2, w._msocr_wino, False
    if WINOGRAD_TALL and _tall_pays(H) and getattr(w, "_msocr_wino42", None) is not None:
        form, u = nat.WINO_4X2, w._msocr_wino42
        up = getattr(w, "_msocr_wino42_split", None)
        if up is not None and SPLIT_BF16X3:
            u, split = up, True
        up44 = getattr(w, "_msocr_wino44ct_split", None)
        if up44 is not None and SPLIT_BF16X3 and WINOGRAD_SQUARE and _square_pays(W):
            form, u, split = nat.WINO_4X4_COLTAIL if _coltail(W) else nat.WINO_4X4, up44, True
    return form, u, split


def conv2d(x, w, bias, stride=(1, 1), pad=(0, 0), relu=False, residual=None, out=None, out_hw=None, alg_k=None, pool2=False):
    _need_cuda(x, w, bias, residual, out)
    N, H, W, Cin = x.shape
    Cout, KH, KW, Cw = w.shape
    assert Cw == Cin and w.is_contiguous() and w.dtype == x.dtype and x.stride(3) == 1
    sh, sw = stride
    ph, pw = pad
    Ho, Wo = out_hw if out_hw else ((H + 2 * ph - KH) // sh + 1, (W + 2 * pw - KW) // sw + 1)
    wino = (sh, sw, ph, pw) == (1, 1, 1, 1) and (Ho, Wo) == (H, W)
    fused = (getattr(w, "_msocr_wino42_fused", None) is not None and WINOGRAD_FUSED64 and WINOGRAD_TALL and wino and _tall_pays(H)
             and (not pool2 or (H % 2 == 0 and W % 2 == 0 and residual is None)))
    if pool2 and not fused:
        return maxpool2d(conv2d(x, w, bias, stride, pad, relu, residual, None, out_hw, alg_k), 2, 2, 0, out=out)
    u = getattr(w, "_msocr_wino", None)
    use_wino = u is not None and wino
    oh, ow = (Ho // 2, Wo // 2) if pool2 else (Ho, Wo)
    if out is None:
        out = torch.empty((N, oh, ow, Cout), dtype=x.dtype, device=x.device)
    assert out.shape == (N, oh, ow, Cout) and out.dtype == x.dtype
    d = nat.ConvDesc()
    d.dtype = _dt(x)
    d.N, d.H, d.W, d.Cin = N, H, W, Cin
    d.in_sN, d.in_sH, d.in_sW = x.stride(0), x.stride(1), x.stride(2)
    d.KH, d.KW, d.stride_h, d.stride_w, d.pad_h, d.pad_w = KH, KW, sh, sw, ph, pw
    d.Ho, d.Wo, d.Cout = Ho, Wo, Cout
    d.out_ld = _pixel_dense_ld(out)
    flags = (nat.CONV_RELU if relu else 0) | (nat.CONV_POOL2 if pool2 else 0)
    rp = None
    if residual is not None:
        assert residual.shape == out.shape and residual.dtype == x.dtype
        d.res_ld = _pixel_dense_ld(residual)
        flags |= nat.CONV_RESIDUAL
        rp = residual.data_ptr()
    d.flags = flags
    if bias is not None:
        assert bias.dtype == torch.float32 and bias.numel() == Cout and bias.is_contiguous()
    bp = bias.data_ptr() if bias is not None else None
    alg = 2.0 * N * Ho * Wo * Cout * (alg_k if alg_k else KH * KW * Cin)
    if fused:
        up = getattr(w, "_msocr_wino42_fused_split", None) if SPLIT_BF16X3 else None
        u = w._msocr_wino42_fused if up is None else up
        _winograd(d, x, w, u, nat.WINO_4X2, up is not None, bias, residual, out, alg, fused=True, pool2=pool2)
    elif use_wino:
        form, u, split = _wino_form(w, H, W)
        _winograd(d, x, w, u, form, split, bias, residual, out, alg)
    else:
        wp = getattr(w, "_msocr_split", None)
        if (wp is None and SPLIT_BF16X3 and not getattr(w, "_msocr_nosplit", False) and _split_eligible(w)
                and not torch.cuda.is_current_stream_capturing()):
            wp = w._msocr_split = split_planes_ktile(w, 1, Cout)
        split = wp is not None and SPLIT_BF16X3 and KH * KW * Cin >= SPLIT_MIN_K and all(v % 4 == 0 for v in x.stride()[:3])
        lean = (split and (KH, KW, sh, sw, ph, pw) == (1, 1, 1, 1, 0, 0) and (Ho, Wo) == (H, W)
                and (H == 1 or x.stride(1) == W * x.stride(2)) and (N == 1 or x.stride(0) == H * W * x.stride(2)))
        e = _prof_begin()
        if split:
            fn = nat.lib().msocr_conv1x1_split if lean else nat.lib().msocr_conv2d_split
            rc = fn(ctypes.byref(d), x.data_ptr(), wp.data_ptr(), bp, rp, out.data_ptr(), _stream())
            nat.check(rc, f"msocr_conv{'1x1' if lean else '2d'}_split {tuple(x.shape)} * {tuple(w.shape)}")
        else:
            rc = nat.lib().msocr_conv2d(ctypes.byref(d), x.data_ptr(), w.data_ptr(), bp, rp, out.data_ptr(), _stream())
            nat.check(rc, f"msocr_conv2d {tuple(x.shape)} * {tuple(w.shape)}")
        io = x.element_size() * (N * H * W * Cin + N * Ho * Wo * Cout * (2 if residual is not None else 1) + Cout * KH * KW * Cin)
        _prof_end(e, "conv_gemm", (alg, 2.0 * N * Ho * Wo * Cout * KH * KW * Cin, io),
                  (N * Ho * Wo, Cout, KH * KW * Cin, "direct_split" if split else "direct"))
    return out


def normalize_u8(imgs_u8, pad_t, pad_l, Hp, Wp, mode, dtype, cpad=4):
    _need_cuda(imgs_u8)
    N, H, W, C = imgs_u8.shape
    assert C == 3 and imgs_u8.dtype == torch.uint8 and imgs_u8.is_contiguous()
    out = torch.empty((N, Hp, Wp, cpad), dtype=dtype, device=imgs_u8.device)
    nat.check(nat.lib().msocr_normalize_u8(imgs_u8.data_ptr(), N, H, W, pad_t, pad_l, Hp, Wp, cpad, mode, _dt(out), out.data_ptr(),
                                           _stream()),
              "normalize_u8")
    return out


def resize_linear_u8(src, dh, dw):
    _need_cuda(src)
    N, sh, sw, C = src.shape
    assert C == 3 and src.dtype == torch.uint8 and src.is_contiguous()
    dst = torch.empty((N, dh, dw, 3), dtype=torch.uint8, device=src.device)
    nat.check(nat.lib().msocr_resize_linear_u8(src.data_ptr(), N, sh, sw, dst.data_ptr(), dh, dw, _stream()), "resize_linear_u8")
    return dst


def maxpool2d(x, k, s, p, out=None):
    _need_cuda(x, out)
    N, H, W, C = x.shape
    Ho, Wo = (H + 2 * p - k) // s + 1, (W + 2 * p - k) // s + 1
    if out is None:
        out = torch.empty((N, Ho, Wo, C), dtype=x.dtype, device=x.device)
    e = _prof_begin()
    nat.check(nat.lib().msocr_maxpool2d(x.data_ptr(), N, H, W, C, _pixel_dense_ld(x), k, s, p, _dt(x), out.data_ptr(), Ho, Wo,
                                        _pixel_dense_ld(out), _stream()), "maxpool2d")
    _prof_end(e, "maxpool", float(x.element_size()) * N * C * (H * W + Ho * Wo))
    return out


def upsample2x_into(x, out):
    _need_cuda(x, out)
    N, H, W, C = x.shape
    assert out.shape[0] == N and out.shape[1] == 2 * H and out.shape[2] == 2 * W and out.dtype == x.dtype
    nat.check(nat.lib().msocr_upsample2x_bilinear(x.data_ptr(), N, H, W, C, _pixel_dense_ld(x), _dt(x), out.data_ptr(),
                                                  _pixel_dense_ld(out), _stream()), "upsample2x")
    return out


def east_head(h1, w9, b9, score=None, geo=None):
    _need_cuda(h1, w9, b9)
    N, H, W, C = h1.shape
    assert C == 32 and w9.shape == (9, 32) and w9.dtype == torch.float32
    if score is None:
        score = torch.empty((N, H, W), dtype=torch.float32, device=h1.device)
    if geo is None:
        geo = torch.empty((N, H, W, 8), dtype=torch.float32, device=h1.device)
    nat.check(nat.lib().msocr_east_head(h1.data_ptr(), N * H * W, _pixel_dense_ld(h1), _dt(h1), w9.data_ptr(), b9.data_ptr(),
# ... 9 lines not shown
    counts = torch.empty((N,), dtype=torch.int32, device=score.device)
    nat.check(nat.lib().msocr_east_decode(score.data_ptr(), geo.data_ptr(), N, H, W, float(thresh), float(scale), int(quant),
                                          cand.data_ptr(), counts.data_ptr(), max_cand, _stream()), "east_decode")
    return cand, counts


def east_lanms(cand, counts, iou_thr, workspace=None):
    _need_cuda(cand, counts)
    N, max_cand, _ = cand.shape
    if workspace is None:
        nbytes = nat.lib().msocr_lanms_workspace_bytes(N, max_cand)
        workspace = torch.empty((nbytes,), dtype=torch.uint8, device=cand.device)
    boxes = torch.empty_like(cand)
    nbox = torch.empty((N,), dtype=torch.int32, device=cand.device)
    nat.check(nat.lib().msocr_east_lanms(cand.data_ptr(), counts.data_ptr(), N, max_cand, float(iou_thr), boxes.data_ptr(),
                                         nbox.data_ptr(), workspace.data_ptr(), _stream()), "east_lanms")
    return boxes, nbox


def east_box_tail(boxes, nbox, expand_w, expand_h, scale_x, scale_y, axis_aligned, remove_anomalies, sigma, min_count, workspace=None):
    _need_cuda(boxes, nbox)
    N, max_cand, _ = boxes.shape
    ws = workspace
    if ws is None:
        ws = torch.empty((nat.lib().msocr_east_box_tail_workspace_bytes(N, max_cand),), dtype=torch.uint8, device=boxes.device)
    out = torch.empty_like(boxes)
    n_out = torch.empty((N,), dtype=torch.int32, device=boxes.device)
    nat.check(nat.lib().msocr_east_box_tail(boxes.data_ptr(), nbox.data_ptr(), N, max_cand, float(expand_w), float(expand_h),
                                            float(scale_x), float(scale_y), int(bool(axis_aligned)), int(bool(remove_anomalies)),
                                            float(sigma), int(min_count), out.data_ptr(), n_out.data_ptr(), ws.data_ptr(), _stream()),
              "east_box_tail")
    return out, n_out


class ReadingOrder(NamedTuple):
    order: torch.Tensor
    keep: torch.Tensor
    desc: torch.Tensor
    ncrop: torch.Tensor


def reading_order_crops(boxes, nbox, page_hw, min_text_size, img_h, img_w, page_base=0, y_tol_ratio=0.6, x_gap_ratio=float("inf"),
                        workspace=None):
    _need_cuda(boxes, nbox)
    N, max_cand, _ = boxes.shape
    dev = boxes.device
    ws = workspace
    if ws is None:
        ws = torch.empty((nat.lib().msocr_reading_order_workspace_bytes(N, max_cand),), dtype=torch.uint8, device=dev)
    order = torch.empty((N, max_cand), dtype=torch.int32, device=dev)
    keep = torch.empty((N, max_cand), dtype=torch.int32, device=dev)
    desc = torch.empty((N, max_cand, 8), dtype=torch.int32, device=dev)
    ncrop = torch.empty((N,), dtype=torch.int32, device=dev)
    nat.check(nat.lib().msocr_reading_order_crops(boxes.data_ptr(), nbox.data_ptr(), N, max_cand, int(page_hw[0]), int(page_hw[1]),
                                                  int(min_text_size), int(img_h), int(img_w), float(y_tol_ratio), float(x_gap_ratio),
                                                  int(page_base), order.data_ptr(), keep.data_ptr(), desc.data_ptr(), ncrop.data_ptr(),
                                                  ws.data_ptr(), _stream()), "reading_order_crops")
    return ReadingOrder(order, keep, desc, ncrop)


class ReadingLines(NamedTuple):
    line: torch.Tensor
    lines: torch.Tensor
    nlines: torch.Tensor


def reading_order_lines(boxes, nbox, page_hw, min_text_size, img_h, img_w, page_base=0, y_tol_ratio=0.6, x_gap_ratio=float("inf"),
                        workspace=None):
    _need_cuda(boxes, nbox)
    N, max_cand, _ = boxes.shape
    dev = boxes.device
    ws = workspace
    if ws is None:
        ws = torch.empty((nat.lib().msocr_reading_order_workspace_bytes(N, max_cand),), dtype=torch.uint8, device=dev)
    i32 = lambda *shape: torch.empty(shape, dtype=torch.int32, device=dev)
    ro = ReadingOrder(i32(N, max_cand), i32(N, max_cand), i32(N, max_cand, 8), i32(N))
    rl = ReadingLines(i32(N, max_cand), i32(N, nat.lib().msocr_reading_order_line_rows(max_cand), 6), i32(N))
    nat.check(nat.lib().msocr_reading_order_lines(boxes.data_ptr(), nbox.data_ptr(), N, max_cand, int(page_hw[0]), int(page_hw[1]),
                                                  int(min_text_size), int(img_h), int(img_w), float(y_tol_ratio), float(x_gap_ratio),
                                                  int(page_base), *[t.data_ptr() for t in ro + rl], ws.data_ptr(), _stream()),
              "reading_order_lines")
    return ro, rl


def reading_lines_host(aabbs_i32, y_tol_ratio=0.6, x_gap_ratio=float("inf")):
    boxes = np.ascontiguousarray(aabbs_i32, dtype=np.int32).reshape(-1, 4)
    n = len(boxes)
    order, line, lines = np.empty(n, dtype=np.int32), np.empty(n, dtype=np.int32), np.empty((n, 6), dtype=np.int32)
    nlines = np.zeros(1, dtype=np.int32)
    nat.check(nat.lib().msocr_reading_lines_host(boxes.ctypes.data, n, float(y_tol_ratio), float(x_gap_ratio), order.ctypes.data,
                                                 line.ctypes.data, lines.ctypes.data, nlines.ctypes.data), "reading_lines_host")
    return order, line, lines[:int(nlines[0])].copy()


def nchw_to_nhwc(x_f32, dtype, out=None):
    _need_cuda(x_f32)
    N, C, H, W = x_f32.shape
    assert x_f32.dtype == torch.float32 and x_f32.is_contiguous()
    if out is None:
        out = torch.empty((N, H, W, C), dtype=dtype, device=x_f32.device)
    nat.check(nat.lib().msocr_nchw_f32_to_nhwc(x_f32.data_ptr(), N, C, H, W, _dt(out), out.data_ptr(), _pixel_dense_ld(out), _stream()),
              "nchw_to_nhwc")
    return out


def nhwc_to_nchw_f32(x):
    _need_cuda(x)
    N, H, W, C = x.shape
    out = torch.empty((N, C, H, W), dtype=torch.float32, device=x.device)
    nat.check(nat.lib().msocr_nhwc_to_nchw_f32(x.data_ptr(), N, C, H, W, _pixel_dense_ld(x), _dt(x), out.data_ptr(), _stream()),
              "nhwc_to_nchw")
    return out


def se_residual(x, identity, w1, w2, out=None, gate=None):
    _need_cuda(x, identity, w1, w2)
    N, H, W, C = x.shape
    assert x.is_contiguous() and identity.is_contiguous() and identity.shape == x.shape and identity.dtype == x.dtype
    assert w1.shape == (C // 16, C) and w2.shape == (C, C // 16) and w1.dtype == torch.float32
    if out is None:
        out = torch.empty_like(x)
    if gate is None:
        gate = torch.empty((N, C), dtype=torch.float32, device=x.device)
    assert gate.shape == (N, C) and gate.dtype == torch.float32 and gate.is_contiguous()
    e = _prof_begin()
    nat.check(nat.lib().msocr_se_residual(x.data_ptr(), identity.data_ptr(), N, H * W, C, _dt(x), w1.data_ptr(), w2.data_ptr(),
                                          gate.data_ptr(), out.data_ptr(), _stream()), "se_residual")
    _prof_end(e, "se_residual", 3.0 * x.element_size() * N * H * W * C, (N, H * W, C))
    return out


SE_BLOCK_FUSED = int(os.environ.get("MSOCR_SE_BLOCK_FUSED", "1"))


def _square_desc(dtype, N, H, W, w, stride, relu):
    Cout, KH, KW, Cin = w.shape
    if (dtype != torch.float32 or (KH, KW) != (3, 3) or tuple(stride) != (1, 1) or getattr(w, "_msocr_wino", None) is None
            or getattr(w, "_msocr_wino42_fused", None) is not None):
        return None
    form, u, split = _wino_form(w, H, W)
    if form not in (nat.WINO_4X4, nat.WINO_4X4_COLTAIL) or not split:
        return None
    d = nat.ConvDesc()
    d.dtype = nat.F32
    d.N, d.H, d.W, d.Cin = N, H, W, Cin
    d.in_sN, d.in_sH, d.in_sW = H * W * Cin, W * Cin, Cin
    d.KH, d.KW, d.stride_h, d.stride_w, d.pad_h, d.pad_w = 3, 3, 1, 1, 1, 1
    d.Ho, d.Wo, d.Cout = H, W, Cout
    d.out_ld = Cout
    d.flags = nat.CONV_RELU if relu else 0
    return d, form, u


def se_block(x, conv1, conv2, identity, se, stride=(1, 1), gate=None):
    (w1, b1), (w2, b2), (s1, s2) = conv1, conv2, se
    _need_cuda(x, w1, b1, w2, b2, identity, s1, s2, gate)
    N, H, W, _ = x.shape
    Ho, Wo = (H - 1) // stride[0] + 1, (W - 1) // stride[1] + 1
    C = w2.shape[0]
    L = nat.lib()
    q2 = _square_desc(x.dtype, N, Ho, Wo, w2, (1, 1), False) if SE_BLOCK_FUSED and SPLIT_BF16X3 else None
    if q2 is None or L.msocr_winograd_crop_lds_bytes(ctypes.byref(q2[0]), q2[1], 1) < 0:
        o = conv2d(x, w1, b1, stride=stride, pad=(1, 1), relu=True)
        o = conv2d(o, w2, b2, pad=(1, 1))
        return se_residual(o, identity, s1, s2, gate=gate)
    d2, form, u2 = q2
    assert identity.shape == (N, Ho, Wo, C) and identity.dtype == x.dtype and identity.is_contiguous()
    assert s1.shape == (C // 16, C) and s2.shape == (C, C // 16) and s1.dtype == torch.float32
    assert b1.dtype == b2.dtype == torch.float32 and b1.is_contiguous() and b2.is_contiguous() and b2.numel() == C
    assert w2.shape[3] == w1.shape[0] == b1.numel() and w1.shape[3] == x.shape[3]
    q1 = _square_desc(x.dtype, N, H, W, w1, stride, True) if x.stride(3) == 1 else None
    if q1 is not None and (q1[1] != form or L.msocr_winograd_crop_lds_bytes(ctypes.byref(q1[0]), form, 0) < 0):
        q1 = None
    if q1 is not None:
        d1, _, u1 = q1
        d1.in_sN, d1.in_sH, d1.in_sW = x.stride(0), x.stride(1), x.stride(2)
        o1 = None
    else:
        o1 = conv2d(x, w1, b1, stride=stride, pad=(1, 1), relu=True)
    out = torch.empty((N, Ho, Wo, C), dtype=x.dtype, device=x.device)
    if gate is None:
        gate = torch.empty((N, C), dtype=torch.float32, device=x.device)
    assert gate.shape == (N, C) and gate.dtype == torch.float32 and gate.is_contiguous()
    nbytes = L.msocr_winograd_workspace_bytes(ctypes.byref(d2), form)
    parts = min(N, -(-nbytes // WINO_WS_LIMIT))
    per = -(-N // parts)
    ws = _wino_workspace(nbytes if parts == 1 else (nbytes // N) * per, x.device)
    name = WINO_FORMS[form][0] + "_split"
    what = f"se_block {tuple(x.shape)} * {tuple(w1.shape)} * {tuple(w2.shape)}"
    alg = 2.0 * Ho * Wo * C * 9
    for n0 in range(0, N, per):
        n1 = min(N, n0 + per)
        nn = d2.N = n1 - n0
        rows, mt = _wino_rows(form, nn, Ho, Wo)
        if q1 is not None:
            d1.N = nn
            _wino_stage_in(d1, form, x[n0:n1].data_ptr(), ws, what)
            _wino_stage_gemm(d1, form, True, u1, ws, what, alg * d1.Cin * nn, name, Ho * Wo, 1)
            e = _prof_begin()
            nat.check(L.msocr_winograd_output_chain(ctypes.byref(d1), form, ws.data_ptr(), b1.data_ptr(), _stream()), what)
            _prof_end(e, "wino_out", 4.0 * 2 * rows * C, (mt, C, "chain"))
        else:
            _wino_stage_in(d2, form, o1[n0:n1].data_ptr(), ws, what)
        _wino_stage_gemm(d2, form, True, u2, ws, what, alg * d2.Cin * nn, name, Ho * Wo, 1)
        e = _prof_begin()
        nat.check(L.msocr_winograd_output_se(ctypes.byref(d2), form, ws.data_ptr(), b2.data_ptr(), identity[n0:n1].data_ptr(), s1.data_ptr(),
                                             s2.data_ptr(), gate[n0:n1].data_ptr(), out[n0:n1].data_ptr(), _stream()), what)
        _prof_end(e, "wino_out", 4.0 * (rows * C + 2 * nn * Ho * Wo * C), (mt, C, "se"))
    return out


def mean_over_h(x):
    _need_cuda(x)
    N, H, W, C = x.shape
    assert x.is_contiguous()
    out = torch.empty((N, W, C), dtype=torch.float32, device=x.device)
    nat.check(nat.lib().msocr_mean_over_h(x.data_ptr(), N, H, W, C, _dt(x), out.data_ptr(), _stream()), "mean_over_h")
    return out


def bilstm_recurrent(xproj, whh_t, B, T, H, whh_planes=None):
    _need_cuda(xproj, whh_t)
    assert xproj.is_contiguous() and xproj.numel() == B * T * 8 * H and whh_t.shape == (2, H, H, 4) and whh_t.is_contiguous()
    out = torch.empty((B, T, 2 * H), dtype=torch.float32, device=xproj.device)
    e = _prof_begin()
    if whh_planes is not None and H == 256 and SPLIT_BF16X3 and B * T * 8 * H < 2 ** 32:
        nat.check(nat.lib().msocr_bilstm_recurrent_split(xproj.data_ptr(), whh_planes.data_ptr(), B, T, H, out.data_ptr(), _stream()),
                  "bilstm_recurrent_split")
    else:
        nat.check(nat.lib().msocr_bilstm_recurrent(xproj.data_ptr(), whh_t.data_ptr(), B, T, H, out.data_ptr(), _stream()), "bilstm_recurrent")
    _prof_end(e, "bilstm", (2.0 * T * (4.0 * H * H * 4 + B * (H + H + 4 * H) * 4 * 2), T), (B, T, H))
    return out


def crop_descriptors(boxes, page_ids, page_hw, img_h, img_w):
    H, W = page_hw
    b = np.asarray(boxes, dtype=np.int64).reshape(-1, 4)
    pg = np.asarray(page_ids, dtype=np.int64).reshape(-1)
    a_, b_ = np.maximum(0, b[:, 0]), np.maximum(0, b[:, 1])
    c_, d_ = np.minimum(W, b[:, 2]), np.minimum(H, b[:, 3])
    c_ = np.where(c_ < 0, np.maximum(W + c_, 0), c_)
    d_ = np.where(d_ < 0, np.maximum(H + d_, 0), d_)
    keep = (c_ > a_) & (d_ > b_)
    a_, b_, c_, d_, pg = a_[keep], b_[keep], c_[keep], d_[keep], pg[keep]
    h, w = d_ - b_, c_ - a_
    scale = np.minimum(img_h / np.maximum(h, 1), img_w / np.maximum(w, 1))
    nw = np.maximum(1, np.rint(w * scale).astype(np.int64))
    nh = np.maximum(1, np.rint(h * scale).astype(np.int64))
    yy = np.maximum(0, np.minimum((img_h - nh) // 2, img_h - nh))
    desc = np.stack([pg, a_, b_, c_, d_, nw, nh, yy], axis=1).astype(np.int32) if len(pg) else np.zeros((0, 8), dtype=np.int32)
    return desc, keep


def _crop_descriptors_loop(boxes, page_ids, page_hw, img_h, img_w):
    H, W = page_hw
    desc, keep = [], []
    for (x0, y0, x1, y1), pg in zip(boxes, page_ids):
        a, b = max(0, int(x0)), max(0, int(y0))
        c, d = min(W, int(x1)), min(H, int(y1))
        if c < 0:
            c = max(W + c, 0)
        if d < 0:
            d = max(H + d, 0)
        if c <= a or d <= b:
            keep.append(False)
            continue
        h, w = d - b, c - a
        scale = min(img_h / max(h, 1), img_w / max(w, 1))
        nw, nh = max(1, int(round(w * scale))), max(1, int(round(h * scale)))
        yy = max(0, min((img_h - nh) // 2, img_h - nh))
        desc.append((pg, a, b, c, d, nw, nh, yy))
        keep.append(True)
    return np.asarray(desc, dtype=np.int32).reshape(-1, 8), np.asarray(keep, dtype=bool)


def _crop(symbol, width, pages_u8, desc_host, img_h, img_w, desc_dev):
    _need_cuda(pages_u8, desc_dev)
    N, H, W, C = pages_u8.shape
    assert C == 3 and pages_u8.dtype == torch.uint8 and pages_u8.is_contiguous()
    hp = None
    if desc_host is not None:
        desc_host = desc_host.astype("int32", copy=False)
        hp = desc_host.ctypes.data
    M = len(desc_host) if desc_host is not None else int(desc_dev.shape[0])
    if desc_dev is None:
        desc_dev = torch.from_numpy(desc_host).to(pages_u8.device)
    else:
        assert desc_dev.dtype == torch.int32 and desc_dev.is_contiguous() and desc_dev.shape == (M, width)
        desc_dev.record_stream(torch.cuda.current_stream())
    out = torch.empty((M, img_h, img_w, 3), dtype=torch.uint8, device=pages_u8.device)
    nat.check(getattr(nat.lib(), symbol)(pages_u8.data_ptr(), N, H, W, desc_dev.data_ptr(), hp, M, img_h, img_w, out.data_ptr(), _stream()),
              symbol[len("msocr_"):])
    return out


def crop_resize_pad(pages_u8, desc_host, img_h, img_w, desc_dev=None):
    return _crop("msocr_crop_resize_pad", 8, pages_u8, desc_host, img_h, img_w, desc_dev)


def quad_crop_descriptors(boxes, nbox, ro, img_h, img_w, out=None):
    ro = ReadingOrder(*ro)
    _need_cuda(boxes, nbox, *ro)
    N, max_cand, _ = boxes.shape
    assert boxes.dtype == torch.float32 and boxes.is_contiguous() and ro.desc.shape == (N, max_cand, 8) and ro.desc.is_contiguous()
    qdesc = out if out is not None else torch.zeros((N, max_cand, 12), dtype=torch.int32, device=boxes.device)
    assert qdesc.shape == (N, max_cand, 12) and qdesc.dtype == torch.int32 and qdesc.is_contiguous() and qdesc.is_cuda
    nat.check(nat.lib().msocr_quad_crop_descriptors(boxes.data_ptr(), nbox.data_ptr(), N, max_cand, int(img_h), int(img_w),
                                                    ro.order.data_ptr(), ro.keep.data_ptr(), ro.desc.data_ptr(), ro.ncrop.data_ptr(),
                                                    qdesc.data_ptr(), _stream()), "quad_crop_descriptors")
    return qdesc


def quad_descriptors(polygons, desc, img_h=0, img_w=0, natural=False):
    desc = np.ascontiguousarray(desc, dtype=np.int32).reshape(-1, 8)
    M = len(desc)
    quads = np.ascontiguousarray(np.asarray(polygons, dtype=np.float32).reshape(M, 8))
    out = np.zeros((M, 12), dtype=np.int32)
    nat.check(nat.lib().msocr_quad_crop_descriptors_host(quads.ctypes.data, desc.ctypes.data, M, int(img_h), int(img_w), int(bool(natural)),
                                                         out.ctypes.data), "quad_crop_descriptors_host")
    return out


def quad_crop_host(pages_u8, qdesc, img_h, img_w):
    pages_u8 = np.ascontiguousarray(pages_u8, dtype=np.uint8)
    qdesc = np.ascontiguousarray(qdesc, dtype=np.int32).reshape(-1, 12)
    N, H, W, C = pages_u8.shape
    assert C == 3
    out = np.empty((len(qdesc), img_h, img_w, 3), dtype=np.uint8)
    nat.check(nat.lib().msocr_quad_crop_host(pages_u8.ctypes.data, N, H, W, qdesc.ctypes.data, len(qdesc), int(img_h), int(img_w),
                                             out.ctypes.data), "quad_crop_host")
    return out


def quad_crop(pages_u8, qdesc_host, img_h, img_w, qdesc_dev=None):
    return _crop("msocr_quad_crop", 12, pages_u8, qdesc_host, img_h, img_w, qdesc_dev)
```

### manuscript_ocr_amd/recognizers/_trba/net.py

```python
import ctypes

import numpy as np

import torch

from ... import _native as nat
from ... import ops
from ...detectors._east.net import BN_EPS, pack_stem_weight, stem_view, to_khwc


def _fold(sd, conv_key, bn_key):
    w = sd[conv_key + ".weight"].float()
    gamma, beta = sd[bn_key + ".weight"].float(), sd[bn_key + ".bias"].float()
    mean, var = sd[bn_key + ".running_mean"].float(), sd[bn_key + ".running_var"].float()
    s = gamma / torch.sqrt(var + BN_EPS)
    return w * s.view(-1, 1, 1, 1), beta - mean * s


def _gate_interleave(w_t, H):
    K = w_t.shape[0]
    return w_t.reshape(K, 4, H).permute(0, 2, 1).contiguous()


HOIST_CTX = True

LAYER_SPEC = (("layer1", 1, 2), ("layer2", 2, 1), ("layer3", 5, 2), ("layer4", 3, 1))


class TrbaNet:
    def __init__(self, state_dict, num_classes, hidden=256, dtype=torch.float32, device="cuda", split=None):
        check_decoder_shape(hidden, num_classes)
        self.dtype, self.device = dtype, torch.device(device)
        self.V, self.Hd = num_classes, hidden
        dev, sd = self.device, state_dict
        P = {}
        self.cpad = 4 if dtype == torch.float32 else 8
        self.cin_pad = 16 if dtype == torch.float32 else 32
        w, b = _fold(sd, "cnn.conv0.0", "cnn.conv0.1")
        P["stem"] = (pack_stem_weight(w, self.cin_pad, self.cpad).to(dtype).to(dev), b.to(dev))
        w, b = _fold(sd, "cnn.conv0.3", "cnn.conv0.4")
        P["conv0b"] = (to_khwc(w, dtype, dev, split), b.to(dev))
        for lname, blocks, stride in LAYER_SPEC:
            for i in range(blocks):
                p = f"cnn.{lname}.{i}."
                for j in (1, 2):
                    w, b = _fold(sd, p + f"conv{j}", p + f"bn{j}")
                    P[f"{lname}.{i}.conv{j}"] = (to_khwc(w, dtype, dev, split), b.to(dev))
                P[f"{lname}.{i}.se"] = (sd[p + "se.fc.0.weight"].float().contiguous().to(dev),
                                        sd[p + "se.fc.2.weight"].float().contiguous().to(dev))
                if p + "downsample.0.weight" in sd:
                    w, b = _fold(sd, p + "downsample.0", p + "downsample.1")
                    P[f"{lname}.{i}.down"] = (to_khwc(w, dtype, dev, split), b.to(dev))
        w, b = _fold(sd, "cnn.conv_out.0", "cnn.conv_out.1")
        P["out0"] = (to_khwc(w, dtype, dev, split), b.to(dev))
        w, b = _fold(sd, "cnn.conv_out.3", "cnn.conv_out.4")
        P["out1"] = (to_khwc(w, dtype, dev, split), b.to(dev))
        self.P = P
        H = hidden
        self.rnn = []
        for l in (0, 1):
            p = f"enc_rnn.{l}."
            w_ih = torch.cat([sd[p + "rnn.weight_ih_l0"], sd[p + "rnn.weight_ih_l0_reverse"]]).float()
            b = torch.cat([sd[p + "rnn.bias_ih_l0"] + sd[p + "rnn.bias_hh_l0"],
                           sd[p + "rnn.bias_ih_l0_reverse"] + sd[p + "rnn.bias_hh_l0_reverse"]]).float()
            whh_t = torch.stack([_gate_interleave(sd[p + "rnn.weight_hh_l0"].float().t(), H),
                                 _gate_interleave(sd[p + "rnn.weight_hh_l0_reverse"].float().t(), H)])
            whh_p = None
            if (ops.SPLIT_BF16X3 if split is None else split) and dtype == torch.float32 and H == 256:
                n = nat.lib().msocr_attn_pack_split_elems(4 * H)
                packed = torch.empty((2, n), dtype=torch.int16)
                wt = whh_t.contiguous()
                for d in (0, 1):
                    nat.check(nat.lib().msocr_attn_pack_split_host(wt[d].data_ptr(), 4 * H, 1, packed[d].data_ptr()), "attn_pack_split_host")
                whh_p = packed.to(dev)
            self.rnn.append({
                "w_ih": w_ih.view(8 * H, 1, 1, -1).contiguous().to(dev), "b": b.contiguous().to(dev),
                "whh_t": whh_t.contiguous().to(dev), "whh_p": whh_p,
                "lin_w": sd[p + "linear.weight"].float().view(H, 1, 1, 2 * H).contiguous().to(dev),
                "lin_b": sd[p + "linear.bias"].float().contiguous().to(dev),
            })
        self.dec = AttnDecoder(state_dict, num_classes, hidden, split, device,
                               step_split=bool((ops.SPLIT_BF16X3 if split is None else split) and dtype == torch.float32))
        self.att, self._aw, self._asw = self.dec.att, self.dec._aw, self.dec._asw

    def _se_block(self, x, lname, i, stride):
        P = self.P
        w1, b1 = P[f"{lname}.{i}.conv1"]
        w2, b2 = P[f"{lname}.{i}.conv2"]
        key = f"{lname}.{i}.down"
        idt = ops.conv2d(x, *P[key], stride=(stride, stride)) if key in P else x
        return ops.se_block(x, (w1, b1), (w2, b2), idt, P[f"{lname}.{i}.se"], stride=(stride, stride))

    def cnn(self, canvases_u8):
        B, h, w, _ = canvases_u8.shape
        x = ops.normalize_u8(canvases_u8, 1, 1, h + 2, w + 4, 1, self.dtype, cpad=self.cpad)
        ws, bs = self.P["stem"]
        x = ops.conv2d(stem_view(x, self.cin_pad), ws, bs, (1, 1), (0, 0), True, out_hw=(h, w), alg_k=27)
        x = ops.conv2d(x, *self.P["conv0b"], pad=(1, 1), relu=True, pool2=True)
        for lname, blocks, stride in LAYER_SPEC:
            for i in range(blocks):
                x = self._se_block(x, lname, i, stride if i == 0 else 1)
        x = ops.conv2d(x, *self.P["out0"], stride=(2, 1), pad=(0, 1), relu=True)
        return ops.conv2d(x, *self.P["out1"], relu=True)

    def encode(self, canvases_u8):
        f = self.cnn(canvases_u8)
        B, Hf, T, C = f.shape
        seq = ops.mean_over_h(f)
        H = self.Hd
        for l in (0, 1):
            r = self.rnn[l]
            xproj = _gemm(seq.view(B * T, -1), r["w_ih"], r["b"])
            hcat = ops.bilstm_recurrent(xproj, r["whh_t"], B, T, H, r["whh_p"])
            seq = _gemm(hcat.view(B * T, 2 * H), r["lin_w"], r["lin_b"]).view(B, T, H)
        proj = _gemm(seq.view(B * T, H), self.att["i2h_w"], None).view(B, T, H)
        return seq, proj

    def greedy(self, batch_H, proj_H, max_len, sos_id, eos_id, blank_id, want_alpha=False):
        return self.dec.greedy(batch_H, proj_H, max_len, sos_id, eos_id, blank_id, want_alpha=want_alpha)

    def forced(self, batch_H, proj_H, tok_in, sos_id, blank_id, ctx_gates=None):
        return self.dec.forced(batch_H, proj_H, tok_in, sos_id, blank_id, ctx_gates=ctx_gates)

    def beam(self, batch_H, proj_H, max_len, beam_size, alpha, temperature, sos_id, eos_id, blank_id, chunks=None, want_alpha=False,
             lexicon=None, lm=None, lm_weight=0.0):
        return self.dec.beam(batch_H, proj_H, max_len, beam_size, alpha, temperature, sos_id, eos_id, blank_id, chunks,
                             want_alpha=want_alpha, lexicon=lexicon, lm=lm, lm_weight=lm_weight)

    def beam_finalize(self, ws, B, steps, beam_size, trun_dev, alpha_ws=None):
        return self.dec.beam_finalize(ws, B, steps, beam_size, trun_dev, alpha_ws=alpha_ws)

    def beam_nbest(self, ws, B, steps, beam_size, trun_dev, n_best, eos_id):
        return self.dec.beam_nbest(ws, B, steps, beam_size, trun_dev, n_best, eos_id)


def check_decoder_shape(hidden, num_classes):
    if hidden % 64 or not 64 <= hidden <= 512:
        raise ValueError(f"hidden_size must be a multiple of 64 between 64 and 512 for the HIP recurrent / attention kernels, got {hidden}")
    if num_classes > 512:
        raise ValueError(f"charsets above 512 tokens are not supported by the decoder kernels, got {num_classes}")


def _gemm(x2d, w, b):
    M, K = x2d.shape
    return ops.conv2d(x2d.view(1, M, 1, K), w, b).view(M, w.shape[0])


class AttnDecoder:

    def __init__(self, state_dict, num_classes, hidden=256, split=None, device="cuda", step_split=None):
        check_decoder_shape(hidden, num_classes)
        if step_split is None:
            step_split = bool(ops.SPLIT_BF16X3 if split is None else split)
        self.device = torch.device(device)
        self.V, self.Hd = num_classes, hidden
        dev, sd, H = self.device, state_dict, hidden
        a = "attn.attention_cell."
        w_ih = sd[a + "rnn.weight_ih"].float()
        self.att = {
            "i2h_w": sd[a + "i2h.weight"].float().view(H, 1, 1, H).contiguous().to(dev),
            "h2h_wt": sd[a + "h2h.weight"].float().t().contiguous().to(dev),
            "h2h_b": sd[a + "h2h.bias"].float().contiguous().to(dev),
            "score_w": sd[a + "score.weight"].float().view(H).contiguous().to(dev),
            "wih_ctx_t": _gate_interleave(w_ih[:, :H].t(), H).to(dev),
            "wih_tok": _gate_interleave(w_ih[:, H:].t(), H).to(dev),
            "whh_t": _gate_interleave(sd[a + "rnn.weight_hh"].float().t(), H).to(dev),
            "b_gates": _gate_interleave((sd[a + "rnn.bias_ih"] + sd[a + "rnn.bias_hh"]).float().view(1, 4 * H), H).view(H, 4).contiguous().to(dev),
            "gen_wt": sd["attn.generator.weight"].float().t().contiguous().to(dev),
            "gen_b": sd["attn.generator.bias"].float().contiguous().to(dev),
        }
        self.att["wih_ctx_rows"] = ops.attach_split(w_ih[:, :H].reshape(4, H, H).permute(1, 0, 2).reshape(4 * H, 1, 1, H).contiguous().to(dev),
                                                    split)
        aw = nat.AttnWeights()
        for k in ("h2h_wt", "h2h_b", "score_w", "wih_ctx_t", "wih_tok", "whh_t", "b_gates", "gen_wt", "gen_b"):
            setattr(aw, k, self.att[k].data_ptr())
        self._aw = aw
        self._asw = None
        self._lp_cache = {}
        if step_split and H == 256 and self.V <= 256:
            asw = nat.AttnSplitWeights()
            for src, dst, n, gi in (("h2h_wt", "h2h_p", H, 0), ("whh_t", "whh_p", 4 * H, 1), ("gen_wt", "gen_p", self.V, 0)):
                wt = self.att[src].cpu().contiguous()
                packed = torch.empty((nat.lib().msocr_attn_pack_split_elems(n),), dtype=torch.int16)
                nat.check(nat.lib().msocr_attn_pack_split_host(wt.data_ptr(), n, gi, packed.data_ptr()), "attn_pack_split_host")
                self.att[dst] = packed.to(dev)
                setattr(asw, dst, self.att[dst].data_ptr())
            self._asw = asw

    def _matrix_core(self, T, beam_size=None):
        if not HOIST_CTX or self.Hd != 256 or self.V > 256 or T > 48:
            return False
        return self._asw is not None if beam_size is None else beam_size <= 8

    def ctx_gates(self, batch_H):
        B, T, H = batch_H.shape
        return _gemm(batch_H.reshape(B * T, H), self.att["wih_ctx_rows"], None)

    def greedy(self, batch_H, proj_H, max_len, sos_id, eos_id, blank_id, ctx_gates=None, want_alpha=False, alpha_out=None):
        B, T, H = batch_H.shape
        steps = max_len + 1
        logits = torch.empty((B, steps, self.V), dtype=torch.float32, device=self.device)
        ids = torch.empty((B, steps), dtype=torch.int32, device=self.device)
        blank = -1 if blank_id is None else blank_id
        al = None
        if want_alpha:
            al = alpha_out if alpha_out is not None else torch.empty((B, steps, T), dtype=torch.float32, device=self.device)
            assert al.shape == (B, steps, T) and al.dtype == torch.float32 and al.is_contiguous() and al.is_cuda
        if self._matrix_core(T):
            ctxg = self.ctx_gates(batch_H) if ctx_gates is None else ctx_gates
            head = (batch_H.data_ptr(), proj_H.data_ptr(), ctxg.data_ptr(), ctypes.byref(self._aw), ctypes.byref(self._asw), B, T, H, self.V,
                    steps, sos_id, eos_id, blank, logits.data_ptr(), ids.data_ptr())
            if al is None:
                nat.check(nat.lib().msocr_attn_greedy_hoisted(*head, ops._stream()), "attn_greedy_hoisted")
            else:
                nat.check(nat.lib().msocr_attn_greedy_hoisted_alpha(*head, al.data_ptr(), ops._stream()), "attn_greedy_hoisted_alpha")
        else:
            head = (batch_H.data_ptr(), proj_H.data_ptr(), ctypes.byref(self._aw), B, T, H, self.V, steps, sos_id, eos_id, blank,
                    logits.data_ptr(), ids.data_ptr())
            if al is None:
                nat.check(nat.lib().msocr_attn_greedy(*head, ops._stream()), "attn_greedy")
            else:
                nat.check(nat.lib().msocr_attn_greedy_alpha(*head, al.data_ptr(), ops._stream()), "attn_greedy_alpha")
        return (logits, ids, al) if want_alpha else (logits, ids)

    def forced(self, batch_H, proj_H, tok_in, sos_id, blank_id, ctx_gates=None):
        B, T, H = batch_H.shape
        assert tok_in.dim() == 2 and tok_in.shape[0] == B and tok_in.dtype == torch.int32 and tok_in.is_contiguous() and tok_in.is_cuda
        steps = tok_in.shape[1]
        logits = torch.empty((B, steps, self.V), dtype=torch.float32, device=self.device)
        al = torch.empty((B, steps, T), dtype=torch.float32, device=self.device)
        blank = -1 if blank_id is None else blank_id
        if self._matrix_core(T):
            ctxg = self.ctx_gates(batch_H) if ctx_gates is None else ctx_gates
            nat.check(nat.lib().msocr_attn_forced_hoisted(batch_H.data_ptr(), proj_H.data_ptr(), ctxg.data_ptr(), ctypes.byref(self._aw),
                                                          ctypes.byref(self._asw), B, T, H, self.V, steps, tok_in.data_ptr(), sos_id, blank,
                                                          logits.data_ptr(), al.data_ptr(), ops._stream()), "attn_forced_hoisted")
        else:
            nat.check(nat.lib().msocr_attn_forced(batch_H.data_ptr(), proj_H.data_ptr(), ctypes.byref(self._aw), B, T, H, self.V, steps,
                                                  tok_in.data_ptr(), sos_id, blank, logits.data_ptr(), al.data_ptr(), ops._stream()),
                      "attn_forced")
        return logits, al

    def seq_logp(self, logits, ids, trun_dev, temperature=1.0):
        B, steps, V = logits.shape
        lps = torch.empty((B, steps), dtype=torch.float32, device=self.device)
        lp = torch.empty((B,), dtype=torch.float32, device=self.device)
        nat.check(nat.lib().msocr_seq_logp(logits.data_ptr(), ids.data_ptr(), trun_dev.data_ptr(), B, V, steps, float(temperature),
                                           lps.data_ptr(), lp.data_ptr(), ops._stream()), "seq_logp")
        return lps, lp

    def beam(self, batch_H, proj_H, max_len, beam_size, alpha, temperature, sos_id, eos_id, blank_id, chunks=None, ctx_gates=None,
             want_alpha=False, alpha_ws=None, lexicon=None, lm=None, lm_weight=0.0):
        B, T, H = batch_H.shape
        steps = max_len
# ... 116 lines not shown
```

Baseline: 83.09.

## Merge two-part Winograd GEMMs into one launch and fuse next block's input transform

Winograd convolutions split into two parts (4x4 and 4x1 tile regions) now run both GEMMs in one persistent split-bf16 launch using a second segment descriptor, instead of two launches. The SE-block output kernel can also write the next block's Winograd input transform straight from LDS. The next se_block then reuses that workspace and skips its own input-transform pass. This cuts kernel launches and a global read of the activation, at the cost of token and epoch bookkeeping that must stay correct across workspace arenas and graph capture.

```diff
diff --git a/include/msocr.h b/include/msocr.h
--- a/include/msocr.h
+++ b/include/msocr.h
@@ -17,6 +17,7 @@
 #define MSOCR_CONV_RELU 1u
 #define MSOCR_CONV_RESIDUAL 2u
 #define MSOCR_CONV_POOL2 4u
+#define MSOCR_CONV_WINO_GEMM_PER_PART 8u
 
 typedef struct msocr_conv_desc {
   int32_t dtype;
@@ -49,6 +50,8 @@
 int msocr_winograd_output_chain(const msocr_conv_desc* d, int form, void* workspace, const float* bias, void* stream);
 int msocr_winograd_output_se(const msocr_conv_desc* d, int form, const void* workspace, const float* bias, const void* identity,
                              const float* w1, const float* w2, float* gate_ws, void* out, void* stream);
+int msocr_winograd_output_se_next(const msocr_conv_desc* d, int form, void* workspace, const float* bias, const void* identity,
+                                  const float* w1, const float* w2, float* gate_ws, void* out, void* stream);
 
 int msocr_split_bf16x3_host(const float* w_host, int64_t n, uint16_t* planes_out_host);
 int msocr_split_bf16x3_ktile_host(const float* w_host, int64_t nbatch, int64_t rows, int64_t k, uint16_t* planes_out_host);
diff --git a/manuscript_ocr_amd/_native.py b/manuscript_ocr_amd/_native.py
--- a/manuscript_ocr_amd/_native.py
+++ b/manuscript_ocr_amd/_native.py
@@ -7,7 +7,7 @@
 LIB_PATH = os.path.join(_HERE, "libmsocr.so")
 
 F32, BF16 = 0, 1
-CONV_RELU, CONV_RESIDUAL, CONV_POOL2 = 1, 2, 4
+CONV_RELU, CONV_RESIDUAL, CONV_POOL2, CONV_WINO_GEMM_PER_PART = 1, 2, 4, 8
 WINO_2X2, WINO_4X2, WINO_4X4, WINO_4X4_COLTAIL = 0, 1, 2, 3
 
 c_i32, c_i64, c_u32 = ctypes.c_int32, ctypes.c_int64, ctypes.c_uint32
@@ -61,6 +61,7 @@
     "msocr_winograd_crop_lds_bytes": (c_i64, [ctypes.POINTER(ConvDesc), c_i32, c_i32]),
     "msocr_winograd_output_chain": (c_i32, [ctypes.POINTER(ConvDesc), c_i32, c_vp, c_vp, c_vp]),
     "msocr_winograd_output_se": (c_i32, [ctypes.POINTER(ConvDesc), c_i32, c_vp, c_vp, c_vp, c_vp, c_vp, c_vp, c_vp, c_vp]),
+    "msocr_winograd_output_se_next": (c_i32, [ctypes.POINTER(ConvDesc), c_i32, c_vp, c_vp, c_vp, c_vp, c_vp, c_vp, c_vp, c_vp]),
     "msocr_winograd_fused64_workspace_bytes": (c_i64, [ctypes.POINTER(ConvDesc)]),
     "msocr_conv3x3_winograd_fused64": (c_i32, [ctypes.POINTER(ConvDesc), c_i32, c_vp, c_vp, c_vp, c_vp, c_vp, c_vp, c_vp]),
     "msocr_winograd_fused64_gemm_output": (c_i32, [ctypes.POINTER(ConvDesc), c_i32, c_vp, c_vp, c_vp, c_vp, c_vp, c_vp]),
diff --git a/manuscript_ocr_amd/csrc/conv_common.h b/manuscript_ocr_amd/csrc/conv_common.h
--- a/manuscript_ocr_amd/csrc/conv_common.h
+++ b/manuscript_ocr_amd/csrc/conv_common.h
@@ -11,6 +11,15 @@
 
 typedef uint32_t u32x4 __attribute__((ext_vector_type(4)));
 typedef uint32_t u32x2 __attribute__((ext_vector_type(2)));
+
+struct ConvSeg {
+  const char* in;
+  const char* w;
+  char* out;
+  long M;
+  int tilesM, nbatch;
+  long bsA, bsW, bsO, wplane;
+};
 
 struct ConvParams {
   const char* in;
@@ -32,6 +41,7 @@
   long bsA, bsW, bsO;
   long wplane;
   long w_kt_b;
+  ConvSeg seg1;
 };
 
 __device__ __forceinline__ float bf16_to_f32(uint16_t v) { return __uint_as_float(((uint32_t)v) << 16); }
@@ -124,6 +134,28 @@
   t -= batch * nblk1;
   tile_n = t % p.tilesN;
   tile_m = t / p.tilesN;
+}
+__device__ __forceinline__ ConvSeg tile_coords_seg(const ConvParams& p, int t, int& batch, int& tile_m, int& tile_n) {
+  const int n0 = p.tilesM * p.tilesN * p.nbatch;
+  const bool second = t >= n0;
+  ConvSeg s;
+  s.in = second ? p.seg1.in : p.in;
+  s.w = second ? p.seg1.w : p.w;
+  s.out = second ? p.seg1.out : p.out;
+  s.M = second ? p.seg1.M : p.M;
+  s.tilesM = second ? p.seg1.tilesM : p.tilesM;
+  s.nbatch = second ? p.seg1.nbatch : p.nbatch;
+  s.bsA = second ? p.seg1.bsA : p.bsA;
+  s.bsW = second ? p.seg1.bsW : p.bsW;
+  s.bsO = second ? p.seg1.bsO : p.bsO;
+  s.wplane = second ? p.seg1.wplane : p.wplane;
+  if (second) t -= n0;
+  const int nblk1 = s.tilesM * p.tilesN;
+  batch = t / nblk1;
+  t -= batch * nblk1;
+  tile_n = t % p.tilesN;
+  tile_m = t / p.tilesN;
+  return s;
 }
 
 template <bool GEN>
@@ -140,8 +172,8 @@
   return (long)n * p.sN + (long)t.hi0 * p.sH + (long)t.wi0 * p.sW;
 }
 template <bool GEN>
-__device__ __forceinline__ uint32_t a_row_offset32(const ConvParams& p, long m, int a_chunk, ATap<GEN>& t) {
-  if (m >= p.M) m = p.M - 1;
+__device__ __forceinline__ uint32_t a_row_offset32(const ConvParams& p, long M, long m, int a_chunk, ATap<GEN>& t) {
+  if (m >= M) m = M - 1;
   if constexpr (GEN) return (uint32_t)(int32_t)((a_row_origin(p, m, t) + a_chunk * 4) * 4);
   else return (uint32_t)((m * p.sW + a_chunk * 4) * 4);
 }
@@ -415,8 +447,14 @@
   p.cin_tiles = p.Cin / G::BK;
   p.ktiles = (int)(p.Ktot / G::BK);
   if (msocr_internal_lds_limit(reinterpret_cast<const void*>(kern), G::LDS) != MSOCR_OK) return MSOCR_E_LAUNCH;
-  const long nblk = (long)p.tilesM * p.tilesN * p.nbatch;
-  if (nblk <= 0 || nblk > 0x7fffffffL) return MSOCR_E_ARG;
+  long nblk = (long)p.tilesM * p.tilesN * p.nbatch;
+  if (nblk <= 0) return MSOCR_E_ARG;
+  if (p.seg1.nbatch) {
+    if (!G::PERSISTENT || p.seg1.nbatch < 0 || p.seg1.M <= 0) return MSOCR_E_ARG;
+    p.seg1.tilesM = (int)((p.seg1.M + G::BM - 1) / G::BM);
+    nblk += (long)p.seg1.tilesM * p.tilesN * p.seg1.nbatch;
+  }
+  if (nblk > 0x7fffffffL) return MSOCR_E_ARG;
   long grid = nblk;
   if (G::PERSISTENT) {
     int n_cu = 0;
diff --git a/manuscript_ocr_amd/csrc/conv_split.hip b/manuscript_ocr_amd/csrc/conv_split.hip
--- a/manuscript_ocr_amd/csrc/conv_split.hip
+++ b/manuscript_ocr_amd/csrc/conv_split.hip
@@ -33,7 +33,7 @@
   uint32_t a_off[A_IT];
   ATap<GEN> a_tap[A_IT];
 #pragma unroll
-  for (int i = 0; i < A_IT; ++i) a_off[i] = a_row_offset32<GEN>(p, (long)tile_m * BM + a_row0 + i * ARP, a_chunk, a_tap[i]);
+  for (int i = 0; i < A_IT; ++i) a_off[i] = a_row_offset32<GEN>(p, p.M, (long)tile_m * BM + a_row0 + i * ARP, a_chunk, a_tap[i]);
   TapCursor tap;
   tap.reset();
   const int b_chunk = tid % BCH, b_row0 = tid / BCH;
@@ -228,3 +228,23 @@
   p.wplane = (long)nbatch * N * K;
   return launch_split_any(p, s, false);
 }
+
+int msocr_internal_gemm_split_batched2(const float* A0, const uint16_t* B0, float* C0, long M0, int nbatch0, const float* A1,
+                                       const uint16_t* B1, float* C1, long M1, int nbatch1, int N, int K, hipStream_t s) {
+  ConvParams p, q;
+  if (gemm_params(A0, B0, C0, M0, N, K, nbatch0, 64, 32, &p) != MSOCR_OK || gemm_params(A1, B1, C1, M1, N, K, nbatch1, 64, 32, &q) != MSOCR_OK)
+    return MSOCR_E_ARG;
+  p.wplane = (long)nbatch0 * N * K;
+  q.wplane = (long)nbatch1 * N * K;
+  const long limit = (1L << 32) - 4096;
+  const bool lean_ok = (p.M * p.sW + 32) * 4 < limit && (q.M * q.sW + 32) * 4 < limit && ((long)N * K + 32) * 2 < (1L << 32);
+  if (!lean_ok || !msocr_internal_split_pp_takes(p)) {
+    const int rc = launch_split_any(p, s, false);
+    return rc != MSOCR_OK ? rc : launch_split_any(q, s, false);
+  }
+  p.w_kt_b = (long)N * 64;
+  p.seg1.in = q.in; p.seg1.w = q.w; p.seg1.out = q.out;
+  p.seg1.M = q.M; p.seg1.nbatch = q.nbatch;
+  p.seg1.bsA = q.bsA; p.seg1.bsW = q.bsW; p.seg1.bsO = q.bsO; p.seg1.wplane = q.wplane;
+  return msocr_internal_split_pp_launch(p, s, false);
+}
diff --git a/manuscript_ocr_amd/csrc/conv_split_pp.hip b/manuscript_ocr_amd/csrc/conv_split_pp.hip
--- a/manuscript_ocr_amd/csrc/conv_split_pp.hip
+++ b/manuscript_ocr_amd/csrc/conv_split_pp.hip
@@ -44,7 +44,7 @@
   const int lane = tid & 63;
   const int wave = __builtin_amdgcn_readfirstlane(tid >> 6);
 
-  const int nblk = p.tilesM * p.tilesN * p.nbatch;
+  const int nblk = p.tilesM * p.tilesN * p.nbatch + (GEN ? 0 : p.seg1.tilesM * p.tilesN * p.seg1.nbatch);
   const int xcd = blockIdx.x & 7, slot = blockIdx.x >> 3, per_x = gridDim.x >> 3;
   int x_start, x_cnt;
   xcd_range<int>(xcd, nblk, x_start, x_cnt);
@@ -53,7 +53,14 @@
   if (G == 0) return;
 
   auto tile_of = [&](int n, int& batch, int& tile_m, int& tile_n) __attribute__((always_inline)) {
-    tile_coords(p, x_start + slot + n * per_x, batch, tile_m, tile_n);
+    const int t = x_start + slot + n * per_x;
+    if constexpr (GEN) {
+      tile_coords(p, t, batch, tile_m, tile_n);
+      ConvSeg s = {p.in, p.w, p.out, p.M, p.tilesM, p.nbatch, p.bsA, p.bsW, p.bsO, p.wplane};
+      return s;
+    } else {
+      return tile_coords_seg(p, t, batch, tile_m, tile_n);
+    }
   };
 
   if (wave >= 4) {
@@ -63,7 +70,7 @@
     constexpr int BCH = Tile::BCH, B_IT = Tile::B_IT;
     const int a_chunk = ltid % ACH, a_row0 = ltid / ACH;
     const int b_chunk = ltid % BCH, b_row0 = ltid / BCH;
-    const long wplane_b = p.wplane * 2;
+    long wplane_b = p.wplane * 2;
     const int bias_i = ltid < BN ? ltid : BN - 1;
 
     uint32_t a_off[A_IT], b_off[B_IT];
@@ -78,16 +85,17 @@
 
     auto set_tile_a = [&](int n) __attribute__((always_inline)) {
       int batch, tile_m, tile_n;
-      tile_of(n, batch, tile_m, tile_n);
-      ga_base = p.in + (long)batch * p.bsA * 4;
-#pragma unroll
-      for (int i = 0; i < A_IT; ++i) a_off[i] = a_row_offset32<GEN>(p, (long)tile_m * BM + a_row0 + i * ARP, a_chunk, a_tap[i]);
+      const ConvSeg sg = tile_of(n, batch, tile_m, tile_n);
+      ga_base = sg.in + (long)batch * sg.bsA * 4;
+#pragma unroll
+      for (int i = 0; i < A_IT; ++i) a_off[i] = a_row_offset32<GEN>(p, sg.M, (long)tile_m * BM + a_row0 + i * ARP, a_chunk, a_tap[i]);
       tap.reset();
     };
     auto set_tile_b = [&](int n) __attribute__((always_inline)) {
       int batch, tile_m, tile_n;
-      tile_of(n, batch, tile_m, tile_n);
-      gb_base = p.w + (long)batch * p.bsW * 2;
+      const ConvSeg sg = tile_of(n, batch, tile_m, tile_n);
+      gb_base = sg.w + (long)batch * sg.bsW * 2;
+      if constexpr (!GEN) wplane_b = sg.wplane * 2;
       gbias = p.bias ? p.bias + tile_n * BN + bias_i : reinterpret_cast<const float*>(msocr_zero16);
 #pragma unroll
       for (int j = 0; j < B_IT; ++j) b_off[j] = b_plane_offset(tile_n * BN + b_row0 + j * Tile::BRP, p.Cout, b_chunk);
@@ -200,11 +208,11 @@
   const uint32_t vo = (uint32_t)((r16 * p.out_ld + 4 * kg) * 4);
   auto set_epilogue = [&](int n) __attribute__((always_inline)) {
     int batch, tile_m, tile_n;
-    tile_of(n, batch, tile_m, tile_n);
+    const ConvSeg sg = tile_of(n, batch, tile_m, tile_n);
     const long row0 = (long)tile_m * BM + wm * 32 * TM;
     const int col0 = tile_n * BN + wn * 32 * TN;
-    e_ob = p.out + ((long)batch * p.bsO + row0 * p.out_ld + col0) * 4;
-    const long rows = p.M - row0;
+    e_ob = sg.out + ((long)batch * sg.bsO + row0 * p.out_ld + col0) * 4;
+    const long rows = sg.M - row0;
     e_full = rows >= 32 * TM;
     e_lim = (int)(rows < 32 * TM ? rows : 32 * TM) - r16;
     e_slot = n & 3;
@@ -287,6 +295,7 @@
 bool msocr_internal_split_pp_takes(const ConvParams& p) { return p.Cout % 128 == 0 && !p.has_res && p.Ktot >= 64; }
 
 int msocr_internal_split_pp_launch(ConvParams& p, hipStream_t s, bool general) {
+  if (general && p.seg1.nbatch) return MSOCR_E_ARG;
   if (p.Cout % 256 == 0) return general ? launch_pp<2, 4, true>(p, s) : launch_pp<2, 4, false>(p, s);
   if (p.Cout % 128 == 0) return general ? launch_pp<4, 2, true>(p, s) : launch_pp<4, 2, false>(p, s);
   return MSOCR_E_ARG;
diff --git a/manuscript_ocr_amd/csrc/internal.h b/manuscript_ocr_amd/csrc/internal.h
--- a/manuscript_ocr_amd/csrc/internal.h
+++ b/manuscript_ocr_amd/csrc/internal.h
@@ -17,6 +17,9 @@
 
 __attribute__((visibility("hidden"))) int msocr_internal_gemm_split_batched(const float* A, const uint16_t* Bplanes, float* C, long M,
                                                                             int N, int K, int nbatch, hipStream_t s);
+__attribute__((visibility("hidden"))) int msocr_internal_gemm_split_batched2(const float* A0, const uint16_t* B0, float* C0, long M0,
+                                                                             int nbatch0, const float* A1, const uint16_t* B1, float* C1,
+                                                                             long M1, int nbatch1, int N, int K, hipStream_t s);
 
 __attribute__((visibility("hidden"))) inline int msocr_internal_lds_limit(const void* kernel, int bytes) {
   static std::mutex mu;
diff --git a/manuscript_ocr_amd/csrc/winograd.hip b/manuscript_ocr_amd/csrc/winograd.hip
--- a/manuscript_ocr_amd/csrc/winograd.hip
+++ b/manuscript_ocr_amd/csrc/winograd.hip
@@ -263,12 +263,12 @@
                   [&](int t, int c) { wino_input_body<4, 1>(crop, 0, sH, sW, C, k.b, k.mt41, V41 + k.row0_41, t, c); });
 }
 
-__global__ __launch_bounds__(kCropThreads) void wino44_output_kernel_se(const float* __restrict__ Mw44, const float* __restrict__ Mw41,
-                                                                         int C, WinoGeom g44, WinoGeom g41,
-                                                                         const float* __restrict__ bias, const float* __restrict__ idt,
-                                                                         const float* __restrict__ w1, const float* __restrict__ w2,
-                                                                         float* __restrict__ gate_ws, float* __restrict__ out) {
-  extern __shared__ __attribute__((aligned(16))) float crop[];
+template <bool NEXT_V>
+__device__ __forceinline__ void wino_crop_se(float* crop, const float* __restrict__ Mw44, const float* __restrict__ Mw41, int C,
+                                             const WinoGeom& g44, const WinoGeom& g41, const float* __restrict__ bias,
+                                             const float* __restrict__ idt, const float* __restrict__ w1, const float* __restrict__ w2,
+                                             float* __restrict__ gate_ws, float* __restrict__ out, float* __restrict__ V44,
+                                             float* __restrict__ V41) {
   const int tid = threadIdx.x, HW = g44.H * g44.W;
   const long n = blockIdx.x;
   float* sm = crop + (long)HW * C;
@@ -280,7 +280,35 @@
   se_partial_sums<1024, kCropThreads>(ldx, HW, C, sm, tid);
   const float* gate = se_gate<1024, kCropThreads>(sm, HW, C, w1, w2, gate_ws + n * C, tid);
   se_scale<1024, kCropThreads>(ldx, [&](int p, int c) { return *reinterpret_cast<const f32x4*>(is + (long)p * C + c); },
-                               [&](int p, int c, f32x4 y) { *reinterpret_cast<f32x4*>(os + (long)p * C + c) = y; }, HW, C, gate, tid);
+                               [&](int p, int c, f32x4 y) {
+                                 *reinterpret_cast<f32x4*>(os + (long)p * C + c) = y;
+                                 if constexpr (NEXT_V) *reinterpret_cast<f32x4*>(crop + p * C + c) = y;
+                               }, HW, C, gate, tid);
+  if constexpr (NEXT_V) {
+    __syncthreads();
+    const long sW = C, sH = (long)g44.W * C;
+    wino_crop_pairs(k, C,
+                    [&](int t, int c) { wino_input_body<4, 4>(crop, 0, sH, sW, C, k.a, k.mt44, V44 + k.row0_44, t, c); },
+                    [&](int t, int c) { wino_input_body<4, 1>(crop, 0, sH, sW, C, k.b, k.mt41, V41 + k.row0_41, t, c); });
+  }
+}
+
+__global__ __launch_bounds__(kCropThreads) void wino44_output_kernel_se(const float* __restrict__ Mw44, const float* __restrict__ Mw41,
+                                                                         int C, WinoGeom g44, WinoGeom g41,
+                                                                         const float* __restrict__ bias, const float* __restrict__ idt,
+                                                                         const float* __restrict__ w1, const float* __restrict__ w2,
+                                                                         float* __restrict__ gate_ws, float* __restrict__ out) {
+  extern __shared__ __attribute__((aligned(16))) float crop[];
+  wino_crop_se<false>(crop, Mw44, Mw41, C, g44, g41, bias, idt, w1, w2, gate_ws, out, nullptr, nullptr);
+}
+__global__ __launch_bounds__(kCropThreads) void wino44_output_kernel_se_next(const float* __restrict__ Mw44, const float* __restrict__ Mw41,
+                                                                              int C, WinoGeom g44, WinoGeom g41,
+                                                                              const float* __restrict__ bias, const float* __restrict__ idt,
+                                                                              const float* __restrict__ w1, const float* __restrict__ w2,
+                                                                              float* __restrict__ gate_ws, float* __restrict__ out,
+                                                                              float* __restrict__ V44, float* __restrict__ V41) {
+  extern __shared__ __attribute__((aligned(16))) float crop[];
+  wino_crop_se<true>(crop, Mw44, Mw41, C, g44, g41, bias, idt, w1, w2, gate_ws, out, V44, V41);
 }
 
 struct WinoPart {
@@ -387,6 +415,12 @@
   if (!wino_gemm_ok(form, split) || wino_check(d, form, &pl) != MSOCR_OK || !u || !workspace) return MSOCR_E_ARG;
   if (split && (d->Cin % 32 || d->Cout % 64)) return MSOCR_E_ARG;
   float* ws = (float*)workspace;
+  if (split && pl.nparts == 2 && !(d->flags & MSOCR_CONV_WINO_GEMM_PER_PART)) {
+    const WinoPart &a = pl.part[0], &b = pl.part[1];
+    const uint16_t* ua = (const uint16_t*)u;
+    return msocr_internal_gemm_split_batched2(ws + a.v, ua, ws + a.mw, a.g.Mt, a.P, ws + b.v, ua + 3L * a.P * d->Cout * d->Cin, ws + b.mw,
+                                              b.g.Mt, b.P, d->Cout, d->Cin, (hipStream_t)stream);
+  }
   long uoff = 0;
   for (int i = 0; i < pl.nparts; ++i) {
     const WinoPart& p = pl.part[i];
@@ -474,6 +508,21 @@
   const float* ws = (const float*)workspace;
   MSOCR_LAUNCH(wino44_output_kernel_se, dim3((unsigned)d->N), dim3(kCropThreads), (size_t)lds, (hipStream_t)stream, ws + k.mw44, ws + k.mw41,
                d->Cout, k.g44, k.g41, bias, (const float*)identity, w1, w2, gate_ws, (float*)out);
+  return LAUNCH_OK();
+}
+
+extern "C" int msocr_winograd_output_se_next(const msocr_conv_desc* d, int form, void* workspace, const float* bias, const void* identity,
+                                             const float* w1, const float* w2, float* gate_ws, void* out, void* stream) {
+  WinoPlan pl;
+  if (!wino_plan(d, form, &pl) || !workspace || !identity || !w1 || !w2 || !gate_ws || !out) return MSOCR_E_ARG;
+  if (((uintptr_t)workspace | (uintptr_t)identity | (uintptr_t)out) & 15 || (bias && ((uintptr_t)bias & 15))) return MSOCR_E_ARG;
+  const long lds = wino_crop_lds(d, pl, true);
+  if (lds < 0 || wino_crop_lds(d, pl, false) < 0 || (d->flags & (MSOCR_CONV_RESIDUAL | MSOCR_CONV_RELU))) return MSOCR_E_ARG;
+  if (msocr_internal_lds_limit(reinterpret_cast<const void*>(wino44_output_kernel_se_next), kCropLdsMax) != MSOCR_OK) return MSOCR_E_LAUNCH;
+  const WinoCropParts k = wino_crop_parts(pl);
+  float* ws = (float*)workspace;
+  MSOCR_LAUNCH(wino44_output_kernel_se_next, dim3((unsigned)d->N), dim3(kCropThreads), (size_t)lds, (hipStream_t)stream, ws + k.mw44,
+               ws + k.mw41, d->Cout, k.g44, k.g41, bias, (const float*)identity, w1, w2, gate_ws, (float*)out, ws + k.v44, ws + k.v41);
   return LAUNCH_OK();
 }
 
diff --git a/manuscript_ocr_amd/ops.py b/manuscript_ocr_amd/ops.py
--- a/manuscript_ocr_amd/ops.py
+++ b/manuscript_ocr_amd/ops.py
@@ -58,12 +58,21 @@
 
 WINO_WS_LIMIT = int(os.environ.get("MSOCR_WINO_WS_LIMIT", str(1 << 30)))
 _WINO_ARENA = {}
+_WINO_EPOCH = {}
+
+
+def _wino_epoch(device, stream, bump=False):
+    key = (device.index, stream)
+    if bump:
+        _WINO_EPOCH[key] = _WINO_EPOCH.get(key, 0) + 1
+    return _WINO_EPOCH.get(key, 0)
 
 
 def _wino_workspace(nbytes, device):
+    key = (device.index, torch.cuda.current_stream().cuda_stream)
+    _wino_epoch(device, key[1], bump=True)
     if torch.cuda.is_current_stream_capturing():
         return torch.empty((nbytes,), dtype=torch.uint8, device=device)
-    key = (device.index, torch.cuda.current_stream().cuda_stream)
     buf = _WINO_ARENA.get(key)
     if buf is None or buf.numel() < nbytes:
         buf = None
@@ -198,8 +207,17 @@
     _prof_end(e, "wino_in", 4.0 * (d.N * d.H * d.W * d.Cin + rows * d.Cin), (mt, d.Cin))
 
 
+WINO_GEMM_MERGED = 1
+
+
+def _gemm_launch_flag(d):
+    d.flags = (d.flags & ~nat.CONV_WINO_GEMM_PER_PART) | (0 if WINO_GEMM_MERGED else nat.CONV_WINO_GEMM_PER_PART)
+    return d
+
+
 def _wino_stage_gemm(d, form, split, u, ws, what, alg, name, out_px, res_io, fused_tail=None):
     rows, _ = _wino_rows(form, d.N, d.H, d.W)
+    _gemm_launch_flag(d)
     e = _prof_begin()
     if fused_tail is not None:
         rc = nat.lib().msocr_winograd_fused64_gemm_output(ctypes.byref(d), int(split), u.data_ptr(), ws.data_ptr(), *fused_tail, _stream())
@@ -225,6 +243,7 @@
     what = f"msocr_conv3x3_{name} {tuple(x.shape)} * {tuple(w.shape)}"
     out_px = H * W // (4 if pool2 else 1)
     res_io = 2 if residual is not None else 1
+    _gemm_launch_flag(d)
     for n0 in range(0, N, per):
         n1 = min(N, n0 + per)
         d.N = n1 - n0
@@ -540,7 +559,36 @@
     return d, form, u
 
 
-def se_block(x, conv1, conv2, identity, se, stride=(1, 1), gate=None):
+SE_BLOCK_NEXT_V = 1
+
+
+class NextV:
+    __slots__ = ("ws", "plan", "stream", "epoch", "out", "version", "capturing")
+
+    def __init__(self, ws, plan, stream, epoch, out, capturing=False):
+        self.ws, self.plan, self.stream, self.epoch, self.out, self.capturing = ws, tuple(plan), stream, epoch, out, capturing
+        self.version = out._version
+
+    def usable(self, x, plan, stream, ws_now, epoch_now):
+        return (self.ws is ws_now and self.plan == tuple(plan) and self.stream == stream and self.epoch == epoch_now
+                and self.out is x and self.version == x._version)
+
+
+def _next_v_workspace(tok, nbytes, device, stream):
+    if torch.cuda.is_current_stream_capturing():
+        return tok.ws if tok.capturing and tok.ws.numel() >= nbytes else None
+    buf = _WINO_ARENA.get((device.index, stream))
+    return buf if buf is not None and buf.numel() >= nbytes and not tok.capturing else None
+
+
+def se_block(x, conv1, conv2, identity, se, stride=(1, 1), gate=None, v_in=None, next_conv1=None):
+    if next_conv1 is not None:
+        out, tok = _se_block(x, conv1, conv2, identity, se, stride, gate, v_in, next_conv1)
+        return out, tok
+    return _se_block(x, conv1, conv2, identity, se, stride, gate, v_in, None)[0]
+
+
+def _se_block(x, conv1, conv2, identity, se, stride, gate, v_in, next_conv1):
     (w1, b1), (w2, b2), (s1, s2) = conv1, conv2, se
     _need_cuda(x, w1, b1, w2, b2, identity, s1, s2, gate)
     N, H, W, _ = x.shape
@@ -551,7 +599,7 @@
     if q2 is None or L.msocr_winograd_crop_lds_bytes(ctypes.byref(q2[0]), q2[1], 1) < 0:
         o = conv2d(x, w1, b1, stride=stride, pad=(1, 1), relu=True)
         o = conv2d(o, w2, b2, pad=(1, 1))
-        return se_residual(o, identity, s1, s2, gate=gate)
+        return se_residual(o, identity, s1, s2, gate=gate), None
     d2, form, u2 = q2
     assert identity.shape == (N, Ho, Wo, C) and identity.dtype == x.dtype and identity.is_contiguous()
     assert s1.shape == (C // 16, C) and s2.shape == (C, C // 16) and s1.dtype == torch.float32
@@ -573,7 +621,18 @@
     nbytes = L.msocr_winograd_workspace_bytes(ctypes.byref(d2), form)
     parts = min(N, -(-nbytes // WINO_WS_LIMIT))
     per = -(-N // parts)
-    ws = _wino_workspace(nbytes if parts == 1 else (nbytes // N) * per, x.device)
+    plan, stream = (form, N, Ho, Wo, C), torch.cuda.current_stream().cuda_stream
+    have_v = (v_in is not None and SE_BLOCK_NEXT_V and q1 is not None and parts == 1
+              and v_in.usable(x, plan, stream, _next_v_workspace(v_in, nbytes, x.device, stream), _wino_epoch(x.device, stream)))
+    if have_v:
+        ws = v_in.ws
+        _wino_epoch(x.device, stream, bump=True)
+    else:
+        ws = _wino_workspace(nbytes if parts == 1 else (nbytes // N) * per, x.device)
+    give_v = bool(next_conv1 is not None and SE_BLOCK_NEXT_V and parts == 1 and next_conv1.shape == (C, 3, 3, C))
+    if give_v:
+        qn = _square_desc(x.dtype, N, Ho, Wo, next_conv1, (1, 1), True)
+        give_v = qn is not None and qn[1] == form and L.msocr_winograd_crop_lds_bytes(ctypes.byref(qn[0]), form, 0) >= 0
     name = WINO_FORMS[form][0] + "_split"
     what = f"se_block {tuple(x.shape)} * {tuple(w1.shape)} * {tuple(w2.shape)}"
     alg = 2.0 * Ho * Wo * C * 9
@@ -583,7 +642,8 @@
         rows, mt = _wino_rows(form, nn, Ho, Wo)
         if q1 is not None:
             d1.N = nn
-            _wino_stage_in(d1, form, x[n0:n1].data_ptr(), ws, what)
+            if not have_v:
+                _wino_stage_in(d1, form, x[n0:n1].data_ptr(), ws, what)
             _wino_stage_gemm(d1, form, True, u1, ws, what, alg * d1.Cin * nn, name, Ho * Wo, 1)
             e = _prof_begin()
             nat.check(L.msocr_winograd_output_chain(ctypes.byref(d1), form, ws.data_ptr(), b1.data_ptr(), _stream()), what)
@@ -592,10 +652,15 @@
             _wino_stage_in(d2, form, o1[n0:n1].data_ptr(), ws, what)
         _wino_stage_gemm(d2, form, True, u2, ws, what, alg * d2.Cin * nn, name, Ho * Wo, 1)
         e = _prof_begin()
-        nat.check(L.msocr_winograd_output_se(ctypes.byref(d2), form, ws.data_ptr(), b2.data_ptr(), identity[n0:n1].data_ptr(), s1.data_ptr(),
-                                             s2.data_ptr(), gate[n0:n1].data_ptr(), out[n0:n1].data_ptr(), _stream()), what)
-        _prof_end(e, "wino_out", 4.0 * (rows * C + 2 * nn * Ho * Wo * C), (mt, C, "se"))
-    return out
+        se_call = L.msocr_winograd_output_se_next if give_v else L.msocr_winograd_output_se
+        nat.check(se_call(ctypes.byref(d2), form, ws.data_ptr(), b2.data_ptr(), identity[n0:n1].data_ptr(), s1.data_ptr(),
+                          s2.data_ptr(), gate[n0:n1].data_ptr(), out[n0:n1].data_ptr(), _stream()), what)
+        if give_v:
+            _prof_end(e, "wino_out", 4.0 * (2 * rows * C + 2 * nn * Ho * Wo * C), (mt, C, "se", "next_v"))
+        else:
+            _prof_end(e, "wino_out", 4.0 * (rows * C + 2 * nn * Ho * Wo * C), (mt, C, "se"))
+    tok = NextV(ws, plan, stream, _wino_epoch(x.device, stream), out, torch.cuda.is_current_stream_capturing()) if give_v else None
+    return out, tok
 
 
 def mean_over_h(x):
diff --git a/manuscript_ocr_amd/recognizers/_trba/net.py b/manuscript_ocr_amd/recognizers/_trba/net.py
--- a/manuscript_ocr_amd/recognizers/_trba/net.py
+++ b/manuscript_ocr_amd/recognizers/_trba/net.py
@@ -83,13 +83,16 @@
                                step_split=bool((ops.SPLIT_BF16X3 if split is None else split) and dtype == torch.float32))
         self.att, self._aw, self._asw = self.dec.att, self.dec._aw, self.dec._asw
 
-    def _se_block(self, x, lname, i, stride):
+    def _se_block(self, x, lname, i, stride, v_in=None, nxt=None):
         P = self.P
         w1, b1 = P[f"{lname}.{i}.conv1"]
         w2, b2 = P[f"{lname}.{i}.conv2"]
         key = f"{lname}.{i}.down"
         idt = ops.conv2d(x, *P[key], stride=(stride, stride)) if key in P else x
-        return ops.se_block(x, (w1, b1), (w2, b2), idt, P[f"{lname}.{i}.se"], stride=(stride, stride))
+        if nxt is None:
+            return ops.se_block(x, (w1, b1), (w2, b2), idt, P[f"{lname}.{i}.se"], stride=(stride, stride), v_in=v_in), None
+        return ops.se_block(x, (w1, b1), (w2, b2), idt, P[f"{lname}.{i}.se"], stride=(stride, stride), v_in=v_in,
+                            next_conv1=P[f"{nxt[0]}.{nxt[1]}.conv1"][0])
 
     def cnn(self, canvases_u8):
         B, h, w, _ = canvases_u8.shape
@@ -97,9 +100,13 @@
         ws, bs = self.P["stem"]
         x = ops.conv2d(stem_view(x, self.cin_pad), ws, bs, (1, 1), (0, 0), True, out_hw=(h, w), alg_k=27)
         x = ops.conv2d(x, *self.P["conv0b"], pad=(1, 1), relu=True, pool2=True)
-        for lname, blocks, stride in LAYER_SPEC:
-            for i in range(blocks):
-                x = self._se_block(x, lname, i, stride if i == 0 else 1)
+        seq = [(lname, i, stride if i == 0 else 1) for lname, blocks, stride in LAYER_SPEC for i in range(blocks)]
+        tok = None
+        for j, (lname, i, stride) in enumerate(seq):
+            nxt = seq[j + 1] if j + 1 < len(seq) else None
+            if nxt is not None and nxt[2] != 1:
+                nxt = None
+            x, tok = self._se_block(x, lname, i, stride, tok, nxt)
         x = ops.conv2d(x, *self.P["out0"], stride=(2, 1), pad=(0, 1), relu=True)
         return ops.conv2d(x, *self.P["out1"], relu=True)
 
```

Result: no change. 83.97 (median of 6 runs) (+1.1%).
